# Pasqui1010/DART-Planner

Hardware: AMD Instinct MI355X
Metric: SE(3) rollouts/sec (N=30, batch=8192) + p95 solve ms, at 1/2/4/8 MI355X (higher is better)
Workload: dtype f32

## Files before the change

### dart_planner_amd/capi.py

```python
from __future__ import annotations

import ctypes as C
import math
import os
from typing import Optional

_HERE = os.path.dirname(os.path.abspath(__file__))
DEFAULT_LIBRARY = os.path.join(_HERE, "libse3mpc.so")

SE3MPC_MAX_HORIZON = 64
SE3MPC_MAX_CORRECTIONS = 10
SE3MPC_MAX_SPHERES = 256

STATUS_NAMES = {0: "SE3MPC_OK", -1: "SE3MPC_ERR_NULL", -2: "SE3MPC_ERR_HORIZON", -3: "SE3MPC_ERR_SHAPE",
                -4: "SE3MPC_ERR_PARAM", -5: "SE3MPC_ERR_WORKSPACE", -6: "SE3MPC_ERR_LAUNCH",
                -7: "SE3MPC_ERR_NO_DEVICE"}
TASK_MESSAGES = {1: "CONVERGENCE: NORM OF PROJECTED GRADIENT <= PGTOL",
                 2: "CONVERGENCE: RELATIVE REDUCTION OF F <= FACTR*EPSMCH",
                 3: "STOP: TOTAL NO. OF ITERATIONS REACHED LIMIT",
                 4: "STOP: TOTAL NO. OF F,G EVALUATIONS EXCEEDS LIMIT",
                 5: "ABNORMAL: "}


class Se3mpcLibraryError(RuntimeError):
    """libse3mpc.so is missing or does not export the ABI of include/se3mpc.h."""


class Se3mpcError(RuntimeError):

    def __init__(self, fn: str, status: int, detail: str = ""):
        self.status = status
        super().__init__(f"{fn} -> {STATUS_NAMES.get(status, status)}" + (f": {detail}" if detail else ""))


class Params(C.Structure):
    _fields_ = [("horizon", C.c_int32), ("has_goal", C.c_int32), ("dt", C.c_double), ("mass", C.c_double),
                ("gravity", C.c_double), ("position_weight", C.c_double), ("velocity_weight", C.c_double),
                ("acceleration_weight", C.c_double), ("thrust_weight", C.c_double), ("terminal_factor", C.c_double),
                ("position_bound", C.c_double), ("max_velocity", C.c_double), ("max_acceleration", C.c_double),
                ("max_thrust", C.c_double), ("min_thrust", C.c_double), ("max_tilt_angle", C.c_double),
                ("safety_margin", C.c_double), ("max_iterations", C.c_int32), ("max_corrections", C.c_int32),
                ("max_linesearch", C.c_int32), ("max_fun", C.c_int32), ("pgtol", C.c_double), ("ftol", C.c_double)]

    @classmethod
    def reference_defaults(cls, **overrides) -> "Params":
        p = cls(horizon=6, has_goal=1, dt=1.0 / 400.0, mass=1.5, gravity=9.81, position_weight=100.0,
                velocity_weight=10.0, acceleration_weight=1.0, thrust_weight=0.1, terminal_factor=10.0,
                position_bound=100.0, max_velocity=10.0, max_acceleration=15.0, max_thrust=25.0, min_thrust=2.0,
                max_tilt_angle=math.pi / 4, safety_margin=1.5, max_iterations=15, max_corrections=10,
                max_linesearch=20, max_fun=15000, pgtol=0.05, ftol=0.5)
        names = cls._field_names()
        for k, v in overrides.items():
            if k not in names:
                raise AttributeError(f"se3mpc_params has no field {k!r}")
            setattr(p, k, v)
        return p

    @classmethod
    def _field_names(cls) -> frozenset:
        names = cls.__dict__.get("_names")
        if names is None:
            names = cls._names = frozenset(n for n, _ in cls._fields_)
        return names

    def copy(self, **overrides) -> "Params":
        q = Params()
        C.memmove(C.byref(q), C.byref(self), C.sizeof(Params))
        for k, v in overrides.items():
            setattr(q, k, v)
        return q

    def as_dict(self) -> dict:
        return {n: getattr(self, n) for n, _ in self._fields_}


class SolveInfo(C.Structure):
    _fields_ = [("fun", C.c_double), ("nit", C.c_int32), ("nfev", C.c_int32), ("status", C.c_int32),
                ("task", C.c_int32)]


class VoxelMapDesc(C.Structure):
    _fields_ = [("keys", C.c_void_p), ("prob", C.c_void_p), ("count", C.c_void_p), ("capacity", C.c_int32),
                ("reserved", C.c_int32), ("resolution", C.c_double), ("prior", C.c_double)]


class ControllerParams(C.Structure):
    _fields_ = [("kp_pos", C.c_double * 3), ("ki_pos", C.c_double * 3), ("kd_pos", C.c_double * 3), ("kp_att", C.c_double * 3),
                ("kd_att", C.c_double * 3), ("inertia", C.c_double * 3), ("max_torque_xyz", C.c_double * 3),
                ("max_integral_per_axis", C.c_double * 3), ("max_integral_pos", C.c_double), ("max_tilt_angle", C.c_double),
                ("mass", C.c_double), ("gravity", C.c_double), ("max_thrust", C.c_double), ("min_thrust", C.c_double),
                ("tracking_error_threshold", C.c_double), ("velocity_error_threshold", C.c_double),
                ("back_calculation_gain", C.c_double), ("integral_decay_factor", C.c_double), ("saturation_threshold", C.c_double),
                ("yaw_singularity_threshold", C.c_double), ("default_heading_yaw", C.c_double),
                ("anti_windup_method", C.c_int32), ("yaw_fallback_method", C.c_int32)]
    ANTI_WINDUP = {"clamping": 0, "back_calculation": 1}
    YAW_FALLBACK = {"skip_yaw": 0, "default_heading": 1, "maintain_current": 2}

    @classmethod
    def from_config(cls, cfg) -> "ControllerParams":
        p = cls()
        for name, ctype in cls._fields_:
            if name == "anti_windup_method":
                p.anti_windup_method = cls.ANTI_WINDUP.get(cfg.anti_windup_method, 2)
            elif name == "yaw_fallback_method":
                p.yaw_fallback_method = cls.YAW_FALLBACK.get(cfg.yaw_singularity_fallback_method, 3)
            elif ctype is C.c_double:
                setattr(p, name, float(getattr(cfg, name)))
            else:
                setattr(p, name, (C.c_double * 3)(*[float(v) for v in getattr(cfg, name)]))
        return p


class SimulatorParams(C.Structure):
    _fields_ = [("mass", C.c_double), ("gravity", C.c_double), ("inertia", C.c_double * 3), ("max_thrust", C.c_double),
                ("max_torque", C.c_double)]

    @classmethod
    def reference_defaults(cls, **overrides) -> "SimulatorParams":
        p = cls(mass=1.5, gravity=9.81, inertia=(C.c_double * 3)(0.1, 0.1, 0.2), max_thrust=20.0, max_torque=10.0)
        for k, v in overrides.items():
            setattr(p, k, v)
        return p


class SmootherParams(C.Structure):
    _fields_ = [("transition_time", C.c_double), ("velocity_limit", C.c_double), ("acceleration_limit", C.c_double),
                ("jerk_limit", C.c_double), ("update_dt", C.c_double), ("smoothing_window", C.c_double),
                ("pos_diff_threshold", C.c_double), ("vel_diff_threshold", C.c_double), ("timeout", C.c_double),
                ("decay_rate", C.c_double), ("decay_cap", C.c_double)]

    @classmethod
    def reference_defaults(cls, **overrides) -> "SmootherParams":
        p = cls(transition_time=0.5, velocity_limit=5.0, acceleration_limit=3.0, jerk_limit=10.0, update_dt=0.01, smoothing_window=0.1,
                pos_diff_threshold=0.5, vel_diff_threshold=1.0, timeout=2.0, decay_rate=2.0, decay_cap=5.0)
        for k, v in overrides.items():
            if k not in dict(cls._fields_):
                raise AttributeError(f"se3mpc_smoother_params has no field {k!r}")
            setattr(p, k, float(v))
        return p

    def copy(self, **overrides) -> "SmootherParams":
        return type(self).reference_defaults(**{**{k: getattr(self, k) for k, _ in self._fields_}, **overrides})


CONTROLLER_STATE_WORDS = 12
SMOOTHER_STATE_WORDS = 25

_P = C.c_void_p
_I = C.c_int
_D = C.c_double
_PP = C.POINTER(Params)
_VP = C.POINTER(VoxelMapDesc)

_TYPED_API = {
    "init": (True, [_I, _I, _P, _P, _P, _I, _P, _P]),
    "cost_grad": (True, [_I, _I, _P, _P, _P, _P, _P]),
    "dynamics_residual": (True, [_I, _I, _P, _P, _P, _P, _P]),
    "obstacle_residual": (True, [_I, _I, _P, _P, _I, _P, _P, _P, _P]),
    "physical_constraints": (True, [_I, _I, _P, _P, _P]),
    "extract": (True, [_I, _I, _P, _P, _P, _P, _P, _P]),
    "rollout_cost_grad": (True, [_I, _I, _P, _P, _P, _P, _P, _P, _P, _P, _P, C.c_uint32, _P]),
    "rollout_cost_grad_batched": (True, [_I, _I, _I, _P, _P, _P, _P, _P, _P, _P, C.c_uint32, _P]),
    "rollout_obstacles": (True, [_I, _I, _P, _P, _P, _P, _P, _P, _P, _I, _P, _P, _P, C.c_uint32, _P]),
    "rollout_obstacles_batched": (True, [_I, _I, _I, _P, _P, _P, _P, _P, _P, _P, _I, _P, _P, _P, C.c_uint32, _P]),
    "rollout_iterate": (True, [_I, _I, _I, _I, _D, _P, _P, _P, _P, _P, _P, _P, _P, _P, C.c_uint32, _P]),
    "rollout_iterate_obstacles": (True, [_I, _I, _I, _I, _D, _P, _P, _P, _P, _P, _P, _P, _P, _P, _I, _D, _P, _P, C.c_uint32, _P]),
    "shooting_finish": (True, [_I, _I, _P, _P, _I, C.c_uint32, _P, _P, _I, _D, _P, _P, _P]),
    "projected_step": (True, [_I, _I, _D, _P, _P, _P, _P]),
    "is_plan_valid": (True, [_I, _I, _P, _P, _P, _P]),
    "argmin": (False, [_I, _P, C.c_uint32, _P, _P]),
    "spheres_from_grid": (False, [_P, _P, _I, C.c_double, _I, C.c_double, _P, _I, _P, _P]),
    "transpose": (False, [_I, _I, _P, _I, _P, _I, _P]),
    "population_sums": (False, [_I, _I, _I, _P, _P, _D, _P, _D, _P, _P, _P]),
    "mppi": (True, [_I, _I, _I, _I, _D, _D, C.c_uint64, C.c_uint32, _P, C.c_uint32, _P, _P, _P, _P, _P, _P, _I, _D, _P, _P, _P, _P]),
    "mppi_split": (True, [_I, _I, _I, _I, _D, _D, C.c_uint64, C.c_uint32, _P, C.c_uint32, _P, _P, _P, _P, _P, _P, _I, _D, _P, _P, _P, _I, _P, C.c_size_t,
                          _P]),
    "mppi_samples": (True, [_I, _I, _I, _D, C.c_uint64, C.c_uint32, C.c_uint32, _P, _P, _I, _P, _P, _P]),
    "solve": (True, [_I, _P, _P, _P, _P, _P, _P, _P, _P, _P, _P, _P]),
    "plan_host": (True, [_I, _P, _P, _P, _P, _P, _P, _P, _P, _P, _P, _P, C.c_uint64, C.c_double, _P]),
}
_VOXEL_TYPED_API = {
    "query": [_P, _I, _P, _P],
    "trajectory_safe": [_P, _I, _I, C.c_longlong, _D, _D, _P, _P, _P],
    "local_spheres": [C.POINTER(C.c_double * 3), _D, _D, _I, _D, _P, _I, _P, _P, _P],
}
_VOXEL_PLAIN_API = {
    "se3mpc_voxel_clear": (C.c_int, [_VP, _P]),
    "se3mpc_voxel_insert": (C.c_int, [_VP, _P, _P, _D, _P, _I, _P, _P]),
    "se3mpc_voxel_update_rays": (C.c_int, [_VP, _P, _P, _P, _P, _I, _D, _D, _P, _P, _I, _P, _P, _P, _P]),
    "se3mpc_voxel_update_row_words": (C.c_longlong, [_I, _I]),
    "se3mpc_voxel_trace_rays": (C.c_int, [_VP, _P, _P, _P, _I, _P, _P, _I, _P, _P]),
    "se3mpc_voxel_export": (C.c_int, [_VP, _P, _P, _P, _P, _P]),
    "se3mpc_voxel_local_workspace": (C.c_int, [_I]),
}
_CP = C.POINTER(ControllerParams)
_SP = C.POINTER(SimulatorParams)
_MP = C.POINTER(SmootherParams)
_LL = C.c_longlong
_PLAN = [_I, _P, _LL, _P, _LL, _P, _LL, _P, _LL]
_LOOP_TYPED_API = {
    "control": [_CP, _I, _P, _P, _P, _P, _P, _P, _P, _P, _P, _P, _P, _P, _P, _P, _P, _P, _P],
    "control_fast": [_CP, _D, _D, _I, _D, _P, _P, _P, _P, _P, _P, _P, _P, _P, _P, _P, _P, _P, _P],
    "controller_integral_update": [_CP, _I, _P, _D, _P, _P, _P],
    "controller_attitude_torque": [_CP, _I, _P, _P, _P, _P, _P, C.POINTER(C.c_double * 9), _P, _P, _P, _P],
    "controller_desired_frame": [_CP, _I, _I, _P, _P, _P, _P, _P, _P, _P],
    "control_plan": [_CP, _I, _P, _P, _P, _P, _P, _P, _I, _P, _LL, _P, _LL, _P, _LL, _P, _LL, _P, _P, _P, _P, _P, _P, _P, _P],
    "simulator_step": [_SP, _I, _D, _P, _P, _P, _LL, _P, _P, _P, _P, _P, _P],
    "closed_loop": [_CP, _SP, _I, _I, _D, _I, _P, _LL, _P, _LL, _P, _LL, _P, _LL, _P, _P, _P, _P, _P, _P, _P, _LL, _I,
                    C.POINTER(C.c_double * 3), _I, _P, _P, _P, _P, _P],
    "smoother_update": [_MP, _I, _P] + _PLAN + _PLAN + [_P, _P],
    "smoother_desired": [_MP, _I, _P, _P, _P] + _PLAN + [_P, _P, _P, _P],
    "closed_loop_smoothed": [_MP, _CP, _SP, _I, _I, _D] + _PLAN + [_P, _P, _P, _P, _P, _P, _P, _P, _LL, _I, C.POINTER(C.c_double * 3),
                             _P, _P, _P, _P, _P],
    "monte_carlo": [_PP, _CP, _SP, _I, _I, _I, _D, _P, _P, _LL, _P, _P, _P, _P, _P, _P, _P, _P, _P, _P, _P],
    "mppi_closed_loop": [_PP, _CP, _SP, _I, _I, _I, _D, C.c_uint32, _I, _I, _I, _D, _D, C.c_uint64, C.c_uint32, C.c_uint32, _P, _P, _I, _D, _P, _LL,
                         _P, _P, _P, _P, _P, _P, _P, _P, _P, _P, _P, _P],
}
_PLAIN_API = {
    "se3mpc_controller_default_params": (C.c_int, [_CP]),
    "se3mpc_simulator_default_params": (C.c_int, [_SP]),
    "se3mpc_controller_reset": (C.c_int, [_CP, _I, _P, _P]),
    "se3mpc_smoother_default_params": (C.c_int, [_MP]),
    "se3mpc_smoother_reset": (C.c_int, [_I, _P, _P]),
    "se3mpc_abi_version": (C.c_int, []),
    "se3mpc_last_error": (C.c_char_p, []),
    "se3mpc_device_count": (C.c_int, []),
    "se3mpc_default_params": (C.c_int, [_PP]),
    "se3mpc_check_params": (C.c_int, [_PP]),
    "se3mpc_set_rollout_variant": (C.c_int, [_I]),
    "se3mpc_set_solver_variant": (C.c_int, [_I]),
    "se3mpc_reduce_keys": (C.c_int, [_P, _I, _I, _P, _P]),
    "se3mpc_key_index": (C.c_uint32, [C.c_uint64]),
    "se3mpc_key_cost": (C.c_float, [C.c_uint64]),
    "se3mpc_population_workspace": (C.c_int, [_I, _I]),
    "se3mpc_mppi_split_workspace_bytes": (C.c_size_t, [_I, _I, _I]),
}


def exported_symbols() -> list:
    names = list(_PLAIN_API)
    for base in _TYPED_API:
        names += [f"se3mpc_{base}_f32", f"se3mpc_{base}_f64"]
    for base in _LOOP_TYPED_API:
        names += [f"se3mpc_{base}_f32", f"se3mpc_{base}_f64"]
    names += list(_VOXEL_PLAIN_API)
    for base in _VOXEL_TYPED_API:
        names += [f"se3mpc_voxel_{base}_f32", f"se3mpc_voxel_{base}_f64"]
    return names


class Library:

    def __init__(self, path: Optional[str] = None):
        self.path = path or os.environ.get("SE3MPC_LIBRARY", DEFAULT_LIBRARY)
        if not os.path.exists(self.path):
            raise Se3mpcLibraryError(
                f"{self.path} not found: the HIP extension has not been built.  Run "
                "`python -c 'import __graft_entry__ as g; g.build()'` (or `make -C dart_planner_amd/csrc`). "
                "There is no CPU fallback.")
        try:
            self._dll = C.CDLL(self.path)
        except OSError as e:
            raise Se3mpcLibraryError(f"cannot load {self.path}: {e}") from e
        missing = [s for s in exported_symbols() if not hasattr(self._dll, s)]
        if missing:
            raise Se3mpcLibraryError(f"{self.path} does not export {missing}")
        for name, (res, args) in _PLAIN_API.items():
            fn = getattr(self._dll, name)
            fn.restype, fn.argtypes = res, args
        for base, (has_params, args) in _TYPED_API.items():
            for suf in ("f32", "f64"):
                fn = getattr(self._dll, f"se3mpc_{base}_{suf}")
                fn.restype = C.c_int
                fn.argtypes = ([_PP] if has_params else []) + args
        for base, args in _LOOP_TYPED_API.items():
            for suf in ("f32", "f64"):
                fn = getattr(self._dll, f"se3mpc_{base}_{suf}")
                fn.restype, fn.argtypes = C.c_int, args
        for name, (res, args) in _VOXEL_PLAIN_API.items():
            fn = getattr(self._dll, name)
            fn.restype, fn.argtypes = res, args
        for base, args in _VOXEL_TYPED_API.items():
            for suf in ("f32", "f64"):
                fn = getattr(self._dll, f"se3mpc_voxel_{base}_{suf}")
                fn.restype = C.c_int
                fn.argtypes = [_VP] + args
        if self._dll.se3mpc_abi_version() != 1:
            raise Se3mpcLibraryError(f"{self.path}: ABI version {self._dll.se3mpc_abi_version()} != 1")

    def abi_version(self) -> int:
        return self._dll.se3mpc_abi_version()

    def last_error(self) -> str:
        return (self._dll.se3mpc_last_error() or b"").decode()

    def device_count(self) -> int:
        return self._dll.se3mpc_device_count()

    def default_params(self) -> Params:
        p = Params()
        self._check("se3mpc_default_params", self._dll.se3mpc_default_params(C.byref(p)))
        return p

    def check_params(self, p: Params) -> int:
        return self._dll.se3mpc_check_params(C.byref(p))

    def set_rollout_variant(self, variant: int) -> None:
        self._check("se3mpc_set_rollout_variant", self._dll.se3mpc_set_rollout_variant(variant))

    def set_solver_variant(self, variant: int) -> None:
        self._check("se3mpc_set_solver_variant", self._dll.se3mpc_set_solver_variant(variant))

    def reduce_keys(self, wave_keys: int, per_batch: int, nbatch: int, keys_out: int, stream: int) -> None:
        self._check("se3mpc_reduce_keys", self._dll.se3mpc_reduce_keys(wave_keys, per_batch, nbatch, keys_out, stream))

    def population_workspace(self, rows: int, B: int) -> int:
        return self._dll.se3mpc_population_workspace(rows, B)

    def mppi_split_workspace_bytes(self, horizon: int, nprob: int, splits: int) -> int:
        return self._dll.se3mpc_mppi_split_workspace_bytes(horizon, nprob, splits)

    def key_index(self, key: int) -> int:
        return self._dll.se3mpc_key_index(C.c_uint64(key))

    def key_cost(self, key: int) -> float:
        return self._dll.se3mpc_key_cost(C.c_uint64(key))

    def call(self, base: str, suffix: str, *args, params: Optional[Params] = None) -> None:
        fn = getattr(self._dll, f"se3mpc_{base}_{suffix}")
        has_params = _TYPED_API[base][0]
        if has_params:
            if params is None:
                raise TypeError(f"se3mpc_{base} needs params")
            rc = fn(C.byref(params), *args)
        else:
            rc = fn(*args)
        self._check(f"se3mpc_{base}_{suffix}", rc)

    def call_status(self, base: str, suffix: str, *args, params: Optional[Params] = None) -> int:
        fn = getattr(self._dll, f"se3mpc_{base}_{suffix}")
        if _TYPED_API[base][0]:
            return fn(C.byref(params) if params is not None else None, *args)
        return fn(*args)

    def controller_default_params(self) -> ControllerParams:
        p = ControllerParams()
        self._check("se3mpc_controller_default_params", self._dll.se3mpc_controller_default_params(C.byref(p)))
        return p

    def simulator_default_params(self) -> SimulatorParams:
        p = SimulatorParams()
        self._check("se3mpc_simulator_default_params", self._dll.se3mpc_simulator_default_params(C.byref(p)))
        return p

    def controller_reset(self, cp: ControllerParams, B: int, state: int, stream: int) -> None:
        self._check("se3mpc_controller_reset", self._dll.se3mpc_controller_reset(C.byref(cp), B, state, stream))

    def smoother_default_params(self) -> SmootherParams:
        p = SmootherParams()
        self._check("se3mpc_smoother_default_params", self._dll.se3mpc_smoother_default_params(C.byref(p)))
        return p

    def smoother_reset(self, B: int, state: int, stream: int) -> None:
        self._check("se3mpc_smoother_reset", self._dll.se3mpc_smoother_reset(B, state, stream))

    def loop_call(self, base: str, suffix: str, *args) -> None:
        a = [C.byref(x) if isinstance(x, (ControllerParams, SimulatorParams, SmootherParams, Params)) else x for x in args]
        self._check(f"se3mpc_{base}_{suffix}", getattr(self._dll, f"se3mpc_{base}_{suffix}")(*a))

    def loop_status(self, base: str, suffix: str, *args) -> int:
        a = [C.byref(x) if isinstance(x, (ControllerParams, SimulatorParams, SmootherParams, Params)) else x for x in args]
        return getattr(self._dll, f"se3mpc_{base}_{suffix}")(*a)

    def voxel(self, name: str, desc: VoxelMapDesc, *args) -> None:
        self._check(f"se3mpc_voxel_{name}", getattr(self._dll, f"se3mpc_voxel_{name}")(C.byref(desc), *args))

    def voxel_status(self, name: str, desc: Optional[VoxelMapDesc], *args) -> int:
        return getattr(self._dll, f"se3mpc_voxel_{name}")(C.byref(desc) if desc is not None else None, *args)

    def voxel_local_workspace(self, cells_per_axis: int) -> int:
        return self._dll.se3mpc_voxel_local_workspace(cells_per_axis)

    def voxel_update_row_words(self, M: int, max_len: int) -> int:
        return self._dll.se3mpc_voxel_update_row_words(M, max_len)

    def _check(self, name: str, rc: int) -> None:
        if rc != 0:
            raise Se3mpcError(name, rc, self.last_error() if rc == -6 else "")


_default: Optional[Library] = None


def get_library() -> Library:
    global _default
    if _default is None:
        _default = Library()
    return _default
```

### dart_planner_amd/csrc/reduce_kernels.hip

```cpp
#include "lane_common.hpp"
#include "rollout_device.hpp"

namespace se3mpc {

template <typename R>
__global__ void __launch_bounds__(256)
argmin_kernel(int B, const R* __restrict__ cost, uint32_t index_base, unsigned long long* __restrict__ key) {
  __shared__ unsigned long long wave_min[4];
  unsigned long long best = ~0ull;
  for (int b = blockIdx.x * blockDim.x + threadIdx.x; b < B; b += gridDim.x * blockDim.x) {
    const unsigned long long k = ((unsigned long long)orderable_bits((float)cost[b]) << 32) | (unsigned long long)(index_base + (uint32_t)b);
    best = k < best ? k : best;
  }
  for (int off = 32; off > 0; off >>= 1) {
    const unsigned long long o = __shfl_down(best, off, kWave);
    best = o < best ? o : best;
  }
  const int lane = threadIdx.x & (kWave - 1), wave = threadIdx.x / kWave;
  if (lane == 0) wave_min[wave] = best;
  __syncthreads();
  if (threadIdx.x == 0) {
    unsigned long long m = wave_min[0];
    for (int w = 1; w < (int)(blockDim.x / kWave); ++w) m = wave_min[w] < m ? wave_min[w] : m;
    atomicMin(key, m);
  }
}

template <typename R>
__global__ void __launch_bounds__(256)
population_sums_kernel(int rows, int B, int ld, const R* __restrict__ X, const R* __restrict__ cost, double cost_ref,
                       const unsigned long long* __restrict__ ref_key, double inv_temperature, int per_split,
                       double* __restrict__ part) {
  __shared__ double wave_tot[4];
  const int r = blockIdx.x, split = blockIdx.y;
  const int lo = split * per_split, hi = (lo + per_split < B) ? lo + per_split : B;
  if (ref_key != nullptr) {
    uint32_t u = (uint32_t)(ref_key[0] >> 32);
    u = (u & 0x80000000u) ? (u & 0x7FFFFFFFu) : ~u;
    cost_ref = (double)__uint_as_float(u);
  }
  const R* row = r < rows ? X + (size_t)r * ld : nullptr;
  double acc = 0.0;
  for (int b = lo + threadIdx.x; b < hi; b += blockDim.x) {
    const double w = cost != nullptr ? exp(-((double)cost[b] - cost_ref) * inv_temperature) : 1.0;
    acc += row != nullptr ? w * (double)row[b] : w;
  }
  acc = wave_sum(acc);
  const int lane = threadIdx.x & (kWave - 1), wave = threadIdx.x / kWave;
  if (lane == 0) wave_tot[wave] = acc;
  __syncthreads();
  if (threadIdx.x == 0) part[(size_t)split * (rows + 1) + r] = ((wave_tot[0] + wave_tot[1]) + wave_tot[2]) + wave_tot[3];
}

__global__ void __launch_bounds__(256)
population_fold_kernel(int n, int nsplit, const double* __restrict__ part, double* __restrict__ out) {
  const int r = blockIdx.x * blockDim.x + threadIdx.x;
  if (r >= n) return;
  double acc = 0.0;
  for (int sp = 0; sp < nsplit; ++sp) acc += part[(size_t)sp * n + r];
  out[r] = acc;
}

__global__ void __launch_bounds__(256)
reduce_keys_kernel(const unsigned long long* __restrict__ wave_keys, int per_batch, unsigned long long* __restrict__ keys_out) {
  __shared__ unsigned long long wave_min[4];
  const unsigned long long* src = wave_keys + (size_t)blockIdx.x * per_batch;
  unsigned long long best = ~0ull;
  for (int i = threadIdx.x; i < per_batch; i += blockDim.x) best = src[i] < best ? src[i] : best;
  for (int off = 32; off > 0; off >>= 1) {
    const unsigned long long o = __shfl_down(best, off, kWave);
    best = o < best ? o : best;
  }
  if ((threadIdx.x & (kWave - 1)) == 0) wave_min[threadIdx.x / kWave] = best;
  __syncthreads();
  if (threadIdx.x == 0) {
    unsigned long long m = wave_min[0];
    for (int w = 1; w < 4; ++w) m = wave_min[w] < m ? wave_min[w] : m;
    keys_out[blockIdx.x] = m;
  }
}

template <typename IO>
__global__ void __launch_bounds__(64)
shooting_finish_kernel(DevParams<double> q, int B, int ld, const IO* __restrict__ T, const unsigned long long* __restrict__ wave_keys,
                       int n_slots, uint32_t index_base, const double* __restrict__ state, const double* __restrict__ spheres, int K,
                       double w_obs, double* __restrict__ out, unsigned long long* __restrict__ key_out) {
  __shared__ double sT[3][kWave], sP[3][kWave], sV[3][kWave], sC[3];
  const int lane = threadIdx.x, N = q.N;
  unsigned long long best = ~0ull;
  for (int i = lane; i < n_slots; i += kWave) best = wave_keys[i] < best ? wave_keys[i] : best;
  for (int off = 32; off > 0; off >>= 1) {
    const unsigned long long o = __shfl_down(best, off, kWave);
    best = o < best ? o : best;
  }
  best = __shfl(best, 0, kWave);
  if (lane == 0 && key_out != nullptr) *key_out = best;
  uint32_t idx = (uint32_t)(best & 0xFFFFFFFFull) - index_base;
  if (idx >= (uint32_t)B) idx = 0;
  const bool live = lane < N;
  double t0 = 0.0, t1 = 0.0, t2 = 0.0;
  if (live) {
    t0 = (double)T[(size_t)(3 * lane + 0) * ld + idx]; t1 = (double)T[(size_t)(3 * lane + 1) * ld + idx]; t2 = (double)T[(size_t)(3 * lane + 2) * ld + idx];
  }
  sT[0][lane] = t0; sT[1][lane] = t1; sT[2][lane] = t2;
  __syncthreads();
  if (lane < 3) {
    const int a = lane;
    const AxisConsts<double> c = axis_consts<double>(q, a, q.has_goal ? state[6 + a] : 0.0);
    double p = state[a], v = state[3 + a];
    RolloutSums<double> s = {0, 0, 0, 0, 0};
    for (int k = 0; k < N; ++k) {
      const double tk = sT[a][k];
      const double acc = tk * q.inv_mass - c.grav, dev = tk - c.hov, e = p - c.gl;
      sP[a][k] = p; sV[a][k] = v;
      if (k == N - 1) s.sterm = e * e; else s.sp += e * e;
      s.sv += v * v; s.sa += acc * acc; s.st += dev * dev;
      p = p + v * q.dt + q.half_dt2 * acc;
      v = v + acc * q.dt;
    }
    s.sp += s.sterm;
    sC[a] = axis_cost(q, s);
  }
  __syncthreads();
  const double cost = sC[0] + sC[1] + sC[2];
  const double mag = sqrt(t0 * t0 + t1 * t1 + t2 * t2);
  const bool valid = live && mag > 1e-6;
  double b1[3] = {0, 0, 0}, b2[3] = {0, 0, 0}, b3[3] = {0, 0, 0};
  double roll = 0.0, pitch = 0.0, yaw = 0.0;
  double n1 = 0.0;
  if (valid) {
    b3[0] = t0 / mag; b3[1] = t1 / mag; b3[2] = t2 / mag;
    b1[0] = 0.0; b1[1] = -b3[2]; b1[2] = b3[1];
    n1 = sqrt(b1[1] * b1[1] + b1[2] * b1[2]);
    if (n1 > 1e-6) { b1[1] /= n1; b1[2] /= n1; } else { b1[0] = 1.0; b1[1] = 0.0; b1[2] = 0.0; }
    b2[0] = b3[1] * b1[2] - b3[2] * b1[1];
    b2[1] = b3[2] * b1[0] - b3[0] * b1[2];
    b2[2] = b3[0] * b1[1] - b3[1] * b1[0];
    roll = atan2(b2[2], b3[2]);
    pitch = asin(fmin(fmax(-b1[2], -1.0), 1.0));
    yaw = n1 > 1e-6 ? (b1[1] == 0.0 ? b1[1] : copysign(1.5707963267948966, b1[1])) : 0.0;
  }
  const uint64_t vmask = wave_ballot(valid);
  const uint64_t below = vmask & ((lane == 0) ? 0ull : (~0ull >> (64 - lane)));
  const bool has_prev = valid && below != 0ull;
  const int pk = has_prev ? 63 - __builtin_clzll(below) : lane;
  double q1[3], q2[3], q3[3];
#pragma unroll
  for (int c = 0; c < 3; ++c) { q1[c] = group_gather<kWave>(b1[c], pk); q2[c] = group_gather<kWave>(b2[c], pk); q3[c] = group_gather<kWave>(b3[c], pk); }
  double w0 = 0.0, w1 = 0.0, w2 = 0.0;
  if (has_prev) {
    double d1[3], d2[3], d3[3];
    for (int c = 0; c < 3; ++c) {
      d1[c] = (b1[c] - q1[c]) / q.dt;
      d2[c] = (b2[c] - q2[c]) / q.dt;
      d3[c] = (b3[c] - q3[c]) / q.dt;
    }
    w0 = b3[0] * d2[0] + b3[1] * d2[1] + b3[2] * d2[2];
    w1 = b1[0] * d3[0] + b1[1] * d3[1] + b1[2] * d3[2];
    w2 = b2[0] * d1[0] + b2[1] * d1[1] + b2[2] * d1[2];
  }
  double pen = 0.0;
  if (spheres != nullptr && K > 0) {
    double pl = 0.0;
    if (live) {
      const double px = sP[0][lane], py = sP[1][lane], pz = sP[2][lane];
      for (int j = 0; j < K; ++j) {
        const double dx = px - spheres[4 * j], dy = py - spheres[4 * j + 1], dz = pz - spheres[4 * j + 2], sm = spheres[4 * j + 3] + q.margin;
        const double h = fmax(0.0, -((dx * dx + dy * dy + dz * dz) - sm * sm));
        pl += h * h;
      }
    }
    pen = w_obs * wave_sum(pl);
  }
  if (live) {
    const int k = lane;
    double* o = out;
    o[3 * k] = sP[0][k]; o[3 * k + 1] = sP[1][k]; o[3 * k + 2] = sP[2][k]; o += 3 * N;
    o[3 * k] = sV[0][k]; o[3 * k + 1] = sV[1][k]; o[3 * k + 2] = sV[2][k]; o += 3 * N;
    o[3 * k] = t0; o[3 * k + 1] = t1; o[3 * k + 2] = t2; o += 3 * N;
    o[3 * k] = t0 / q.mass; o[3 * k + 1] = t1 / q.mass; o[3 * k + 2] = t2 / q.mass - q.grav; o += 3 * N;
    o[3 * k] = roll; o[3 * k + 1] = pitch; o[3 * k + 2] = yaw; o += 3 * N;
    o[3 * k] = w0; o[3 * k + 1] = w1; o[3 * k + 2] = w2; o += 3 * N;
    o[k] = mag;
  }
  if (lane == 0) { out[19 * N] = cost; out[19 * N + 1] = pen; out[19 * N + 2] = cost + pen; }
}

template <typename R>
__global__ void __launch_bounds__(256)
spheres_from_grid_kernel(const R* __restrict__ pos, const R* __restrict__ occ, int M, R threshold, int target, R radius,
                         R* __restrict__ spheres, int cap, int32_t* __restrict__ count) {
  __shared__ int wave_total[4];
  const int lane = threadIdx.x & (kWave - 1), wave = threadIdx.x / kWave;
  const int seg = ((M + 3) / 4 + kWave - 1) / kWave * kWave;
  const int lo = wave * seg, hi = (lo + seg < M) ? lo + seg : M;
  int mine = 0;
  for (int i0 = lo; i0 < hi; i0 += kWave) {
    const int i = i0 + lane;
    const bool o = i < hi && occ[i] > threshold;
    mine += __builtin_popcountll(wave_ballot(o));
  }
  if (lane == 0) wave_total[wave] = mine;
  __syncthreads();
  int rank = 0, total = 0;
  for (int w = 0; w < 4; ++w) { if (w < wave) rank += wave_total[w]; total += wave_total[w]; }
  const int step = (target > 0 && total / target > 1) ? total / target : 1;
  for (int i0 = lo; i0 < hi; i0 += kWave) {
    const int i = i0 + lane;
    const bool o = i < hi && occ[i] > threshold;
    const uint64_t m = wave_ballot(o);
    if (o) {
      const int r = rank + __builtin_popcountll(m & ((lane == 0) ? 0ull : (~0ull >> (64 - lane))));
      if (r % step == 0 && r / step < cap) {
        R* s4 = spheres + (size_t)4 * (r / step);
        s4[0] = pos[(size_t)3 * i]; s4[1] = pos[(size_t)3 * i + 1]; s4[2] = pos[(size_t)3 * i + 2]; s4[3] = radius;
      }
    }
    rank += __builtin_popcountll(m);
  }
  if (threadIdx.x == 0) {
    const int k = total == 0 ? 0 : (total + step - 1) / step;
    *count = k < cap ? k : cap;
  }
}

template <typename R>
__global__ void __launch_bounds__(256)
transpose_kernel(int rows, int cols, const R* __restrict__ in, int ld_in, R* __restrict__ out, int ld_out) {
  __shared__ R tile[64][65];
  const int c0 = blockIdx.x * 64, r0 = blockIdx.y * 64;
  const int tx = threadIdx.x & 63, ty = threadIdx.x >> 6;
  for (int i = ty; i < 64; i += 4) {
    const int r = r0 + i, c = c0 + tx;
    if (r < rows && c < cols) tile[i][tx] = in[(size_t)r * ld_in + c];
  }
  __syncthreads();
  for (int i = ty; i < 64; i += 4) {
    const int c = c0 + i, r = r0 + tx;
    if (r < rows && c < cols) out[(size_t)c * ld_out + r] = tile[tx][i];
  }
}

template <typename R, bool ROWS_SMALL>
__global__ void __launch_bounds__(512)
transpose_strip_kernel(int small, int longn, const R* __restrict__ in, int ld_in, R* __restrict__ out, int ld_out, int TW) {
  HIP_DYNAMIC_SHARED(unsigned char, lds_raw)
  R* tile = reinterpret_cast<R*>(lds_raw);
  const int pitch = small | 1;
  const int l0 = blockIdx.x * TW;
  const int nt = (longn - l0 < TW) ? longn - l0 : TW;
  const int lane = threadIdx.x & (kWave - 1), wave = threadIdx.x / kWave, nwave = blockDim.x / kWave;
  constexpr int U = 8;
  if constexpr (ROWS_SMALL) {
    for (int s0 = wave * U; s0 < small; s0 += nwave * U) {
      R v[U];
#pragma unroll
      for (int u = 0; u < U; ++u) v[u] = (s0 + u < small && lane < nt) ? in[(size_t)(s0 + u) * ld_in + l0 + lane] : (R)0;
#pragma unroll
      for (int u = 0; u < U; ++u) if (s0 + u < small && lane < nt) tile[lane * pitch + s0 + u] = v[u];
    }
    __syncthreads();
    for (int t = wave; t < nt; t += nwave)
      for (int sidx = lane; sidx < small; sidx += kWave) out[(size_t)(l0 + t) * ld_out + sidx] = tile[t * pitch + sidx];
  } else {
    for (int t = wave; t < nt; t += nwave) {
      const R* src = in + (size_t)(l0 + t) * ld_in;
      for (int s0 = lane; s0 < small; s0 += kWave * U) {
        R v[U];
#pragma unroll
        for (int u = 0; u < U; ++u) v[u] = (s0 + u * kWave < small) ? src[s0 + u * kWave] : (R)0;
#pragma unroll
        for (int u = 0; u < U; ++u) if (s0 + u * kWave < small) tile[t * pitch + s0 + u * kWave] = v[u];
      }
    }
    __syncthreads();
    for (int sidx = wave; sidx < small; sidx += nwave)
      if (lane < nt) out[(size_t)sidx * ld_out + l0 + lane] = tile[lane * pitch + sidx];
  }
}

template <typename R>
int argmin_impl(int B, const R* cost, uint32_t index_base, uint64_t* key, void* stream) {
  if (B < 0) return SE3MPC_ERR_SHAPE;
  if (!key) return SE3MPC_ERR_NULL;
  hipStream_t s = (hipStream_t)stream;
  if (hipMemsetAsync(key, 0xFF, sizeof(uint64_t), s) != hipSuccess) return launch_status("se3mpc_argmin(memset)");
  if (B == 0) return SE3MPC_OK;
  if (!cost) return SE3MPC_ERR_NULL;
  int grid = grid_for(B, 256);
  if (grid > 1024) grid = 1024;
  hipLaunchKernelGGL(argmin_kernel<R>, dim3(grid), dim3(256), 0, s, B, cost, index_base, (unsigned long long*)key);
  return launch_status("se3mpc_argmin");
}

static int population_splits(int B) {
  int n = B / 65536;
  return n < 1 ? 1 : (n > 16 ? 16 : n);
}

template <typename R>
int population_sums_impl(int rows, int B, int ld, const R* X, const R* cost, double cost_ref, const uint64_t* ref_key,
                         double temperature, double* out, double* workspace, void* stream) {
  if (rows < 0 || B < 0 || ld < B) return SE3MPC_ERR_SHAPE;
  if (!out) return SE3MPC_ERR_NULL;
  if (cost != nullptr && (!(temperature > 0.0) || !std::isfinite(temperature) || !std::isfinite(cost_ref))) return SE3MPC_ERR_PARAM;
  hipStream_t s = (hipStream_t)stream;
  if (B == 0) {
    if (hipMemsetAsync(out, 0, (size_t)(rows + 1) * sizeof(double), s) != hipSuccess) return launch_status("se3mpc_population_sums(memset)");
    return SE3MPC_OK;
  }
  if ((rows > 0 && !X) || !workspace) return SE3MPC_ERR_NULL;
  const int nsplit = population_splits(B);
  const int per_split = (B + nsplit - 1) / nsplit;
  hipLaunchKernelGGL(population_sums_kernel<R>, dim3(rows + 1, nsplit), dim3(256), 0, s, rows, B, ld, X, cost, cost_ref,
                     reinterpret_cast<const unsigned long long*>(ref_key), cost != nullptr ? 1.0 / temperature : 0.0, per_split,
                     workspace);
  int rc = launch_status("se3mpc_population_sums");
  if (rc) return rc;
  hipLaunchKernelGGL(population_fold_kernel, dim3(grid_for(rows + 1, 256)), dim3(256), 0, s, rows + 1, nsplit, workspace, out);
  return launch_status("se3mpc_population_sums(fold)");
}

template <typename R>
int spheres_from_grid_impl(const R* pos, const R* occ, int M, double threshold, int target, double radius, R* spheres, int cap,
                           int32_t* count, void* stream) {
  if (M < 0 || cap < 0 || target < 1) return SE3MPC_ERR_SHAPE;
  if (!count || (M > 0 && (!pos || !occ)) || (cap > 0 && !spheres)) return SE3MPC_ERR_NULL;
  hipLaunchKernelGGL(spheres_from_grid_kernel<R>, dim3(1), dim3(256), 0, (hipStream_t)stream, pos, occ, M, (R)threshold,
                     target, (R)radius, spheres, cap, count);
  return launch_status("se3mpc_spheres_from_grid");
}

template <typename R>
int transpose_impl(int rows, int cols, const R* in, int ld_in, R* out, int ld_out, void* stream) {
  if (rows < 0 || cols < 0 || ld_in < cols || ld_out < rows) return SE3MPC_ERR_SHAPE;
  if (rows == 0 || cols == 0) return SE3MPC_OK;
  if (!in || !out) return SE3MPC_ERR_NULL;
  const int small = rows < cols ? rows : cols, longn = rows < cols ? cols : rows;
// ... 95 lines not shown
```

### dart_planner_amd/csrc/rollout_device.hpp

```cpp
#pragma once

#include <hip/hip_runtime.h>

#include <cstdint>

#include "se3mpc_common.hpp"
#include <se3mpc_wave_ops.hpp>

namespace se3mpc {


template <typename R, bool SHARED_SLOT = false>
__device__ __forceinline__ void rollout_epilogue(bool live, int b, R c, R* __restrict__ cost,
                                                 unsigned long long* __restrict__ wave_key_slot, uint32_t index_base) {
  if (live) cost[b] = c;
  const uint32_t bits = live ? orderable_bits((float)c) : 0xFFFFFFFFu;
  const uint32_t m = wave_min_u32(bits);
  const int src = first_lane(wave_ballot(live && bits == m));
  if (wave_key_slot != nullptr && src >= 0 && lane_id() == src) {
    const unsigned long long k = ((unsigned long long)m << 32) | (unsigned long long)(index_base + (uint32_t)b);
    if constexpr (SHARED_SLOT) atomicMin(wave_key_slot, k);
    else *wave_key_slot = k;
  }
}

template <typename R>
struct RolloutSums {
  R sp, sv, sa, st, sterm;
};

template <typename R>
__device__ __forceinline__ R rollout_total(const DevParams<R>& q, const RolloutSums<R>& s) {
  R c = q.wv * s.sv + q.wa * s.sa + q.wT * s.st;
  if (q.has_goal) c += q.wp * s.sp + q.term * q.wp * s.sterm;
  return c;
}

template <typename R>
struct AxisConsts {
  R gl, grav, hov, two_wp, two_wv, c_aa, c_tt, c_lp, c_lv;
};

template <typename R>
__device__ __forceinline__ AxisConsts<R> axis_consts(const DevParams<R>& q, int a, R gl) {
  AxisConsts<R> c;
  c.gl = gl;
  c.grav = (a == 2) ? q.grav : (R)0;
  c.hov = (a == 2) ? q.hover : (R)0;
  c.two_wp = q.has_goal ? (R)2 * q.wp : (R)0;
  c.two_wv = (R)2 * q.wv;
  c.c_aa = (R)2 * q.wa * q.inv_mass;
  c.c_tt = (R)2 * q.wT;
  c.c_lp = q.half_dt2 * q.inv_mass;
  c.c_lv = q.dt * q.inv_mass;
  return c;
}

template <typename R>
__device__ __forceinline__ R axis_cost(const DevParams<R>& q, const RolloutSums<R>& s) {
  R c = q.wv * s.sv + q.wa * s.sa + q.wT * s.st;
  if (q.has_goal) c += q.wp * (s.sp + q.term * s.sterm);
  return c;
}

template <typename R, int N, bool GRAD, bool STATES, int LDAUX = 0, int STAUX = 0, bool TILE = false, bool EXACT = true, bool MIDSYNC = false>
__device__ __forceinline__ R rollout_axis_reg(const DevParams<R>& q, int a, unsigned voff, unsigned rowb, const R* __restrict__ p0,
                                              const R* __restrict__ v0, const R* __restrict__ goal,
                                              const R* __restrict__ T, R* __restrict__ gradT, R* __restrict__ Pout,
                                              R* __restrict__ Vout, R* __restrict__ ptile = nullptr) {
  const int Nn = EXACT ? N : q.N;
  R t[N], es[N], vs[N];
#pragma unroll
  for (int k = 0; k < N; ++k) {
    if (EXACT || k < Nn) t[k] = lane_ld<LDAUX>(lane_buf(T), voff, (unsigned)(3 * k + a) * rowb);
  }
  const AxisConsts<R> c = axis_consts<R>(q, a, q.has_goal ? lane_ld(lane_buf(goal), voff, (unsigned)(a) * rowb) : (R)0);
  R p = lane_ld(lane_buf(p0), voff, (unsigned)(a) * rowb);
  R v = lane_ld(lane_buf(v0), voff, (unsigned)(a) * rowb);
  RolloutSums<R> s = {0, 0, 0, 0, 0};
#pragma unroll
  for (int k = 0; k < N; ++k) {
    if (EXACT || k < Nn) {
      const R acc = t[k] * q.inv_mass - c.grav;
      const R dev = t[k] - c.hov;
      const R e = p - c.gl;
      es[k] = e; vs[k] = v;
      if (TILE) ptile[k * kWave] = p;
      if (k == Nn - 1) s.sterm = e * e; else s.sp += e * e;
      s.sv += v * v; s.sa += acc * acc; s.st += dev * dev;
      if (STATES) {
        lane_st(lane_buf(Pout), voff, (unsigned)(3 * k + a) * rowb, p);
        lane_st(lane_buf(Vout), voff, (unsigned)(3 * k + a) * rowb, v);
      }
      p = p + v * q.dt + q.half_dt2 * acc;
      v = v + acc * q.dt;
    }
  }
  if (MIDSYNC) __syncthreads();
  s.sp += s.sterm;
  if (GRAD) {
    R lamP = (R)0, lamV = (R)0;
#pragma unroll
    for (int k = N - 1; k >= 0; --k) {
      if (EXACT || k < Nn) {
        const R acc = t[k] * q.inv_mass - c.grav;
        const R dev = t[k] - c.hov;
        if (k == Nn - 1) {
          lane_st<STAUX>(lane_buf(gradT), voff, (unsigned)(3 * k + a) * rowb, c.c_aa * acc + c.c_tt * dev);
          lamP = c.two_wp * ((R)1 + q.term) * es[k];
          lamV = c.two_wv * vs[k];
        } else {
          lane_st<STAUX>(lane_buf(gradT), voff, (unsigned)(3 * k + a) * rowb, c.c_aa * acc + c.c_tt * dev + c.c_lp * lamP + c.c_lv * lamV);
          lamV = c.two_wv * vs[k] + q.dt * lamP + lamV;
          lamP = c.two_wp * es[k] + lamP;
        }
      }
    }
  }
  return axis_cost(q, s);
}

template <typename R, bool GRAD, bool STATES, int STAUX = 0, bool TILE = false, bool MIDSYNC = false>
__device__ __forceinline__ R rollout_axis_rev(const DevParams<R>& q, int a, unsigned voff, unsigned rowb, const R* __restrict__ p0,
                                              const R* __restrict__ v0, const R* __restrict__ goal,
                                              const R* __restrict__ T, R* __restrict__ gradT, R* __restrict__ Pout,
                                              R* __restrict__ Vout, R* __restrict__ ptile = nullptr) {
  const int N = q.N;
  const AxisConsts<R> c = axis_consts<R>(q, a, q.has_goal ? lane_ld(lane_buf(goal), voff, (unsigned)(a) * rowb) : (R)0);
  R p = lane_ld(lane_buf(p0), voff, (unsigned)(a) * rowb);
  R v = lane_ld(lane_buf(v0), voff, (unsigned)(a) * rowb);
  RolloutSums<R> s = {0, 0, 0, 0, 0};
  R tk = (R)0, pl = p, vl = v;
#pragma unroll 6
  for (int k = 0; k < N; ++k) {
    tk = lane_ld(lane_buf(T), voff, (unsigned)(3 * k + a) * rowb);
    const R acc = tk * q.inv_mass - c.grav;
    const R dev = tk - c.hov;
    const R e = p - c.gl;
    if (TILE) ptile[k * kWave] = p;
    if (k == N - 1) s.sterm = e * e; else s.sp += e * e;
    s.sv += v * v; s.sa += acc * acc; s.st += dev * dev;
    if (STATES) {
      lane_st(lane_buf(Pout), voff, (unsigned)(3 * k + a) * rowb, p);
      lane_st(lane_buf(Vout), voff, (unsigned)(3 * k + a) * rowb, v);
    }
    pl = p; vl = v;
    p = p + v * q.dt + q.half_dt2 * acc;
    v = v + acc * q.dt;
  }
  if (MIDSYNC) __syncthreads();
  s.sp += s.sterm;
  if (GRAD) {
    R lamP = c.two_wp * ((R)1 + q.term) * (pl - c.gl);
    R lamV = c.two_wv * vl;
    lane_st<STAUX>(lane_buf(gradT), voff, (unsigned)(3 * (N - 1) + a) * rowb, c.c_aa * (tk * q.inv_mass - c.grav) + c.c_tt * (tk - c.hov));
    R pk = pl, vk = vl;
#pragma unroll 6
    for (int k = N - 2; k >= 0; --k) {
      const R t = lane_ld(lane_buf(T), voff, (unsigned)(3 * k + a) * rowb);
      const R acc = t * q.inv_mass - c.grav;
      const R dev = t - c.hov;
      vk = vk - acc * q.dt;
      pk = pk - vk * q.dt - q.half_dt2 * acc;
      lane_st<STAUX>(lane_buf(gradT), voff, (unsigned)(3 * k + a) * rowb, c.c_aa * acc + c.c_tt * dev + c.c_lp * lamP + c.c_lv * lamV);
      lamV = c.two_wv * vk + q.dt * lamP + lamV;
      lamP = c.two_wp * (pk - c.gl) + lamP;
    }
  }
  return axis_cost(q, s);
}

typedef float obs_f2 __attribute__((vector_size(8)));
#ifndef SE3MPC_OBS_PACKED
#define SE3MPC_OBS_PACKED 1
#endif
template <typename R> constexpr bool kObsPacked = sizeof(R) == 4 && SE3MPC_OBS_PACKED;

}
```

### dart_planner_amd/csrc/rollout_iterate.hip

```cpp
#include "lane_common.hpp"
#include "rollout_device.hpp"

namespace se3mpc {

__device__ __forceinline__ float fma_r(float a, float b, float c) { return __builtin_fmaf(a, b, c); }
__device__ __forceinline__ double fma_r(double a, double b, double c) { return __builtin_fma(a, b, c); }
__device__ __forceinline__ float clamp_r(float x, float lo, float hi) { return __builtin_amdgcn_fmed3f(x, lo, hi); }
__device__ __forceinline__ double clamp_r(double x, double lo, double hi) { return fmin(fmax(x, lo), hi); }
template <typename R>
__device__ __forceinline__ R projected_update(R t, R g, R step, R lo, R hi) {
  return fmin(fmax(fma_r(-step, g, t), lo), hi);
}

template <typename R>
struct ObsCtx {
  R* tile;
  const R* sph;
  R* pen;
  R* pen_first;
  int Kpad;
  bool axis_sweeps;
  int slot, slots;
  R w_obs;
};
// ... 3 lines not shown
                                            obs_f2& qy, obs_f2& qz) {
  const obs_f2 dx = px2 - cx, dy = py2 - cy, dz = pz2 - cz;
  const obs_f2 c = dz * dz + (dy * dy + (dx * dx - r2));
  const obs_f2 h = obs_f2{fmaxf(0.0f, -c[0]), fmaxf(0.0f, -c[1])};
  if constexpr (PEN) pk += h * h;
  qx += h * dx; qy += h * dy; qz += h * dz;
}
template <typename R, bool PEN = true>
__device__ __forceinline__ void sphere_one(R px, R py, R pz, R cx, R cy, R cz, R r2, R& pk, R& qx, R& qy, R& qz) {
  const R dx = px - cx, dy = py - cy, dz = pz - cz;
  const R c = dz * dz + (dy * dy + (dx * dx - r2));
  const R h = fmax((R)0, -c);
  if constexpr (PEN) pk += h * h;
  qx += h * dx; qy += h * dy; qz += h * dz;
}

template <typename R, int TS>
__device__ __forceinline__ R obstacle_penalty_sweep(R* __restrict__ tile, const R* __restrict__ sph, int Nn, int Kpad, int first, int stride, int lane,
                                                    R w_obs) {
  R pen = (R)0;
  const R scale = (R)-4 * w_obs;
  lane &= TS - 1;
  for (int k = first; k < Nn; k += stride) {
    R* tx = tile + ((size_t)0 * Nn + k) * kWave + lane;
    R* ty = tile + ((size_t)1 * Nn + k) * kWave + lane;
    R* tz = tile + ((size_t)2 * Nn + k) * kWave + lane;
    const R px = *tx, py = *ty, pz = *tz;
    if constexpr (kObsPacked<R>) {
      const obs_f2 px2 = {px, px}, py2 = {py, py}, pz2 = {pz, pz}, zero = {0.0f, 0.0f};
      obs_f2 qx = zero, qy = zero, qz = zero, pk = zero;
#pragma unroll 4
      for (int j = 0; j < Kpad; j += 2) {
        const R* s0 = sph + 4 * j;
        sphere_pair(px2, py2, pz2, obs_f2{s0[0], s0[4]}, obs_f2{s0[1], s0[5]}, obs_f2{s0[2], s0[6]}, obs_f2{s0[3], s0[7]}, pk, qx, qy, qz);
      }
      pen += pk[0] + pk[1];
      *tx = scale * (qx[0] + qx[1]); *ty = scale * (qy[0] + qy[1]); *tz = scale * (qz[0] + qz[1]);
    } else {
      R qx = (R)0, qy = (R)0, qz = (R)0, pk = (R)0;
      for (int j = 0; j < Kpad; ++j) {
        const R* s0 = sph + 4 * j;
        sphere_one<R>(px, py, pz, s0[0], s0[1], s0[2], s0[3], pk, qx, qy, qz);
      }
      pen += pk;
      *tx = scale * qx; *ty = scale * qy; *tz = scale * qz;
    }
  }
  return w_obs * pen;
}

template <typename R, int KP>
struct SphereRegs {
  static constexpr int kPairs = kObsPacked<R> ? 4 * KP : 1, kOnes = kObsPacked<R> ? 1 : 8 * KP;
  obs_f2 cx2[kPairs], cy2[kPairs], cz2[kPairs], r22[kPairs];
  R cx[kOnes], cy[kOnes], cz[kOnes], r2[kOnes];
  __device__ __forceinline__ void load(const R* __restrict__ sph) {
    if constexpr (kObsPacked<R>) {
#pragma unroll
      for (int i = 0; i < kPairs; ++i) {
        const R* s0 = sph + 8 * i;
        cx2[i] = obs_f2{s0[0], s0[4]}; cy2[i] = obs_f2{s0[1], s0[5]}; cz2[i] = obs_f2{s0[2], s0[6]}; r22[i] = obs_f2{s0[3], s0[7]};
      }
    } else {
#pragma unroll
      for (int i = 0; i < kOnes; ++i) { cx[i] = sph[4 * i]; cy[i] = sph[4 * i + 1]; cz[i] = sph[4 * i + 2]; r2[i] = sph[4 * i + 3]; }
    }
  }
};

template <typename R, int KP, int U, int TS, bool PEN>
__device__ __forceinline__ R obstacle_penalty_sweep_regs(R* __restrict__ tile, const SphereRegs<R, KP>& sr, int Nn, int first, int stride, int lane,
                                                         R w_obs) {
  R pen = (R)0;
  const R scale = (R)-4 * w_obs;
  lane &= TS - 1;
#pragma unroll 1
  for (int k0 = first; k0 < Nn; k0 += U * stride) {
    R px[U], py[U], pz[U];
    R* tx[U];
#pragma unroll
    for (int u = 0; u < U; ++u) {
      const int k = k0 + u * stride;
      tx[u] = tile + (size_t)(k < Nn ? k : k0) * kWave + lane;
      px[u] = tx[u][0]; py[u] = tx[u][(size_t)Nn * kWave]; pz[u] = tx[u][(size_t)2 * Nn * kWave];
    }
    if constexpr (kObsPacked<R>) {
      const obs_f2 zero = {0.0f, 0.0f};
      obs_f2 px2[U], py2[U], pz2[U], qx[U], qy[U], qz[U], pk[U];
#pragma unroll
      for (int u = 0; u < U; ++u) { px2[u] = obs_f2{px[u], px[u]}; py2[u] = obs_f2{py[u], py[u]}; pz2[u] = obs_f2{pz[u], pz[u]}; qx[u] = qy[u] = qz[u] = pk[u] = zero; }
#pragma unroll
      for (int i = 0; i < SphereRegs<R, KP>::kPairs; ++i) {
#pragma unroll
        for (int u = 0; u < U; ++u) sphere_pair<PEN>(px2[u], py2[u], pz2[u], sr.cx2[i], sr.cy2[i], sr.cz2[i], sr.r22[i], pk[u], qx[u], qy[u], qz[u]);
      }
#pragma unroll
      for (int u = 0; u < U; ++u) {
        if (k0 + u * stride < Nn) {
          pen += pk[u][0] + pk[u][1];
          tx[u][0] = scale * (qx[u][0] + qx[u][1]); tx[u][(size_t)Nn * kWave] = scale * (qy[u][0] + qy[u][1]);
          tx[u][(size_t)2 * Nn * kWave] = scale * (qz[u][0] + qz[u][1]);
        }
      }
    } else {
      R qx[U], qy[U], qz[U], pk[U];
#pragma unroll
      for (int u = 0; u < U; ++u) qx[u] = qy[u] = qz[u] = pk[u] = (R)0;
#pragma unroll
      for (int i = 0; i < SphereRegs<R, KP>::kOnes; ++i) {
#pragma unroll
        for (int u = 0; u < U; ++u) sphere_one<R, PEN>(px[u], py[u], pz[u], sr.cx[i], sr.cy[i], sr.cz[i], sr.r2[i], pk[u], qx[u], qy[u], qz[u]);
      }
#pragma unroll
      for (int u = 0; u < U; ++u) {
        if (k0 + u * stride < Nn) {
          pen += pk[u];
          tx[u][0] = scale * qx[u]; tx[u][(size_t)Nn * kWave] = scale * qy[u]; tx[u][(size_t)2 * Nn * kWave] = scale * qz[u];
        }
      }
    }
  }
  return w_obs * pen;
}

template <typename R, int TS = kWave>
__device__ __forceinline__ void obstacle_exchange(const ObsCtx<R>& o, int Nn, int w, int lane, bool first) {
  __syncthreads();
  R pen = (R)0;
  if (o.axis_sweeps || w >= 3) pen = obstacle_penalty_sweep<R, TS>(o.tile, o.sph, Nn, o.Kpad, o.slot, o.slots, lane, o.w_obs);
  o.pen[w * kWave + lane] = pen;
  if (first) o.pen_first[w * kWave + lane] = pen;
  __syncthreads();
}

#ifndef SE3MPC_OBS_STEPS_IN_FLIGHT
#define SE3MPC_OBS_STEPS_IN_FLIGHT 2
#endif
template <typename R, int KP, int TS>
__device__ __forceinline__ void helper_passes_regs(const ObsCtx<R>& o, int Nn, int w, int lane, int passes) {
  SphereRegs<R, KP> sr;
  sr.load(o.sph);
#pragma unroll 1
  for (int ps = 0; ps < passes; ++ps) {
    __syncthreads();
    R pen = (R)0;
    if (ps == 0 || ps == passes - 1) pen = obstacle_penalty_sweep_regs<R, KP, SE3MPC_OBS_STEPS_IN_FLIGHT, TS, true>(o.tile, sr, Nn, o.slot, o.slots, lane, o.w_obs);
    else (void)obstacle_penalty_sweep_regs<R, KP, SE3MPC_OBS_STEPS_IN_FLIGHT, TS, false>(o.tile, sr, Nn, o.slot, o.slots, lane, o.w_obs);
    o.pen[w * kWave + lane] = pen;
    if (ps == 0) o.pen_first[w * kWave + lane] = pen;
    __syncthreads();
  }
}

template <typename R, int N, bool EXACT, int LDAUX, int STAUX, bool OBS = false, int TS = kWave>
__device__ __forceinline__ R iterate_axis_reg(const DevParams<R>& q, int a, unsigned voff, unsigned rowb, const R* __restrict__ p0,
                                              const R* __restrict__ v0, const R* __restrict__ goal, const R* __restrict__ Tin,
                                              R* __restrict__ Tout, R* __restrict__ gradT, int iters, R step, bool live, bool want_first,
                                              R& cost_first, const ObsCtx<R>* obs = nullptr) {
  const int Nn = EXACT ? N : q.N;
  R t[N], es[N], vs[N];
#pragma unroll
  for (int k = 0; k < N; ++k) {
    if (EXACT || k < Nn) t[k] = lane_ld<LDAUX>(lane_buf(Tin), voff, (unsigned)(3 * k + a) * rowb);
  }
  const AxisConsts<R> c = axis_consts<R>(q, a, q.has_goal ? lane_ld(lane_buf(goal), voff, (unsigned)(a) * rowb) : (R)0);
  const R pinit = lane_ld(lane_buf(p0), voff, (unsigned)(a) * rowb);
  const R vinit = lane_ld(lane_buf(v0), voff, (unsigned)(a) * rowb);
  const R lo = (a == 2) ? q.tz_lo : -q.txy, hi = (a == 2) ? q.tz_hi : q.txy;
  const int lane_ = (int)(threadIdx.x & (kWave - 1));
  R* my_tile = nullptr;
  if constexpr (OBS) my_tile = obs->tile + (size_t)a * Nn * kWave + lane_;
  auto forward_cost = [&]() -> R {
    R p = pinit, v = vinit;
    RolloutSums<R> s = {0, 0, 0, 0, 0};
#pragma unroll
    for (int k = 0; k < N; ++k) {
      if (EXACT || k < Nn) {
        const R acc = t[k] * q.inv_mass - c.grav;
        const R dev = t[k] - c.hov;
        const R e = p - c.gl;
        es[k] = e; vs[k] = v;
        if constexpr (OBS) my_tile[(size_t)k * kWave] = p;
        if (k == Nn - 1) s.sterm = e * e; else s.sp += e * e;
        s.sv += v * v; s.sa += acc * acc; s.st += dev * dev;
        p = p + v * q.dt + q.half_dt2 * acc;
        v = v + acc * q.dt;
      }
    }
    s.sp += s.sterm;
    return axis_cost(q, s);
  };
  cost_first = (R)0;
  bool first_exchange = true;
  if (want_first && iters > 0) {
    cost_first = forward_cost();
    if constexpr (OBS) { obstacle_exchange<R, TS>(*obs, Nn, a, lane_, first_exchange); first_exchange = false; }
  }
  const R gA = c.c_aa * q.inv_mass + c.c_tt, gB = c.c_aa * c.grav + c.c_tt * c.hov;
  const R u1 = (R)1 - step * gA, u0 = step * gB, uP = -step * c.c_lp, uV = -step * c.c_lv;
  const R lamP_term = c.two_wp * ((R)1 + q.term);
#pragma unroll 1
  for (int it = 0; it < iters; ++it) {
    R e = pinit - c.gl, v = vinit;
#pragma unroll
    for (int k = 0; k < N; ++k) {
      if (EXACT || k < Nn) {
        const R acc = fma_r(t[k], q.inv_mass, -c.grav);
        es[k] = e; vs[k] = v;
        if constexpr (OBS) my_tile[(size_t)k * kWave] = e + c.gl;
        e = fma_r(q.half_dt2, acc, fma_r(v, q.dt, e));
        v = fma_r(acc, q.dt, v);
      }
    }
    if constexpr (OBS) { obstacle_exchange<R, TS>(*obs, Nn, a, lane_, first_exchange); first_exchange = false; }
    R lamP = (R)0, lamV = (R)0;
#pragma unroll
    for (int k = N - 1; k >= 0; --k) {
      if (EXACT || k < Nn) {
        R qk = (R)0;
        if constexpr (OBS) qk = my_tile[(size_t)k * kWave];
        if (k == Nn - 1) {
          t[k] = clamp_r(fma_r(t[k], u1, u0), lo, hi);
          if constexpr (OBS) lamP = fma_r(lamP_term, es[k], qk); else lamP = lamP_term * es[k];
          lamV = c.two_wv * vs[k];
        } else {
          t[k] = clamp_r(fma_r(t[k], u1, fma_r(lamP, uP, fma_r(lamV, uV, u0))), lo, hi);
          lamV = fma_r(c.two_wv, vs[k], fma_r(q.dt, lamP, lamV));
          if constexpr (OBS) lamP = fma_r(c.two_wp, es[k], lamP + qk); else lamP = fma_r(c.two_wp, es[k], lamP);
        }
      }
    }
  }
  const R cost = forward_cost();
  if (!(want_first && iters > 0)) cost_first = cost;
  if constexpr (OBS) obstacle_exchange<R, TS>(*obs, Nn, a, lane_, first_exchange);
  if (gradT != nullptr) {
    R lamP = (R)0, lamV = (R)0;
#pragma unroll
    for (int k = N - 1; k >= 0; --k) {
      if (EXACT || k < Nn) {
        const R acc = t[k] * q.inv_mass - c.grav;
        const R dev = t[k] - c.hov;
        R qk = (R)0;
        if constexpr (OBS) qk = my_tile[(size_t)k * kWave];
        R g;
        if (k == Nn - 1) {
          g = c.c_aa * acc + c.c_tt * dev;
          lamP = c.two_wp * ((R)1 + q.term) * es[k];
          if constexpr (OBS) lamP += qk;
          lamV = c.two_wv * vs[k];
        } else {
          g = c.c_aa * acc + c.c_tt * dev + c.c_lp * lamP + c.c_lv * lamV;
          lamV = c.two_wv * vs[k] + q.dt * lamP + lamV;
          if constexpr (OBS) lamP = c.two_wp * es[k] + (lamP + qk); else lamP = c.two_wp * es[k] + lamP;
        }
        es[k] = g;
      }
    }
  }
  if (live) {
    if (gradT != nullptr) {
#pragma unroll
      for (int k = 0; k < N; ++k) {
        if (EXACT || k < Nn) lane_st<STAUX>(lane_buf(gradT), voff, (unsigned)(3 * k + a) * rowb, es[k]);
      }
    }
#pragma unroll
    for (int k = 0; k < N; ++k) {
      if (EXACT || k < Nn) lane_st<STAUX>(lane_buf(Tout), voff, (unsigned)(3 * k + a) * rowb, t[k]);
    }
  }
  return cost;
}

template <typename R, bool OBS = false, int TS = kWave>
__device__ __forceinline__ R iterate_axis_mem(const DevParams<R>& q, int a, unsigned voff, unsigned rowb, const R* __restrict__ p0,
                                              const R* __restrict__ v0, const R* __restrict__ goal, const R* __restrict__ Tin,
                                              R* __restrict__ Tout, R* __restrict__ gradT, int iters, R step, bool live, bool want_first,
                                              R& cost_first, const ObsCtx<R>* obs = nullptr) {
  (void)want_first;
  const int N = q.N;
  const int lane_ = (int)(threadIdx.x & (kWave - 1));
  if constexpr (!OBS) {
    if (!live) { cost_first = (R)0; return (R)0; }
  }
  R* my_tile = nullptr;
  if constexpr (OBS) my_tile = obs->tile + (size_t)a * N * kWave + lane_;
  const AxisConsts<R> c = axis_consts<R>(q, a, q.has_goal ? lane_ld(lane_buf(goal), voff, (unsigned)(a) * rowb) : (R)0);
  const R pinit = lane_ld(lane_buf(p0), voff, (unsigned)(a) * rowb);
  const R vinit = lane_ld(lane_buf(v0), voff, (unsigned)(a) * rowb);
  const R lo = (a == 2) ? q.tz_lo : -q.txy, hi = (a == 2) ? q.tz_hi : q.txy;
  if (Tin != Tout && live) {
    for (int k = 0; k < N; ++k) lane_st(lane_buf(Tout), voff, (unsigned)(3 * k + a) * rowb, lane_ld(lane_buf(Tin), voff, (unsigned)(3 * k + a) * rowb));
  }
  R cost = (R)0;
#pragma unroll 1
  for (int it = 0; it <= iters; ++it) {
    const bool last = it == iters;
    R p = pinit, v = vinit, pl = pinit, vl = vinit, tk = (R)0;
    RolloutSums<R> s = {0, 0, 0, 0, 0};
#pragma unroll 6
    for (int k = 0; k < N; ++k) {
      tk = (!OBS || live) ? lane_ld(lane_buf(Tout), voff, (unsigned)(3 * k + a) * rowb) : (R)0;
      const R acc = tk * q.inv_mass - c.grav;
      const R dev = tk - c.hov;
      const R e = p - c.gl;
      if (k == N - 1) s.sterm = e * e; else s.sp += e * e;
      s.sv += v * v; s.sa += acc * acc; s.st += dev * dev;
      if constexpr (OBS) my_tile[(size_t)k * kWave] = p;
      pl = p; vl = v;
      p = p + v * q.dt + q.half_dt2 * acc;
      v = v + acc * q.dt;
    }
    s.sp += s.sterm;
    cost = axis_cost(q, s);
    if (it == 0) cost_first = cost;
    if constexpr (OBS) obstacle_exchange<R, TS>(*obs, N, a, lane_, it == 0);
    R lamP = c.two_wp * ((R)1 + q.term) * (pl - c.gl);
    if constexpr (OBS) lamP += my_tile[(size_t)(N - 1) * kWave];
    R lamV = c.two_wv * vl;
    {
      const R g = c.c_aa * (tk * q.inv_mass - c.grav) + c.c_tt * (tk - c.hov);
      if (!OBS || live) {
        if (last) { if (gradT != nullptr) lane_st(lane_buf(gradT), voff, (unsigned)(3 * (N - 1) + a) * rowb, g); }
        else lane_st(lane_buf(Tout), voff, (unsigned)(3 * (N - 1) + a) * rowb, projected_update(tk, g, step, lo, hi));
      }
    }
    R pk = pl, vk = vl;
#pragma unroll 6
    for (int k = N - 2; k >= 0; --k) {
      const R tt = (!OBS || live) ? lane_ld(lane_buf(Tout), voff, (unsigned)(3 * k + a) * rowb) : (R)0;
      const R acc = tt * q.inv_mass - c.grav;
      const R dev = tt - c.hov;
      vk = vk - acc * q.dt;
      pk = pk - vk * q.dt - q.half_dt2 * acc;
      const R g = c.c_aa * acc + c.c_tt * dev + c.c_lp * lamP + c.c_lv * lamV;
      if (!OBS || live) {
        if (last) { if (gradT != nullptr) lane_st(lane_buf(gradT), voff, (unsigned)(3 * k + a) * rowb, g); }
        else lane_st(lane_buf(Tout), voff, (unsigned)(3 * k + a) * rowb, projected_update(tt, g, step, lo, hi));
      }
      lamV = c.two_wv * vk + q.dt * lamP + lamV;
      if constexpr (OBS) lamP = c.two_wp * (pk - c.gl) + (lamP + my_tile[(size_t)k * kWave]); else lamP = c.two_wp * (pk - c.gl) + lamP;
    }
  }
  return cost;
}

template <typename R, int N, bool REG, int FLAGS>
__global__ void __launch_bounds__(192)
rollout_iterate_kernel(DevParams<R> q, int B, int ld, int iters, R step, const R* __restrict__ p0, const R* __restrict__ v0,
                       const R* __restrict__ goal, const R* __restrict__ Tin, R* __restrict__ Tout, R* __restrict__ cost_first,
                       R* __restrict__ cost, R* __restrict__ gradT, unsigned long long* __restrict__ key, uint32_t index_base) {
  {
    const size_t bi = blockIdx.y, ss = (size_t)3 * ld, st = (size_t)3 * q.N * ld;
    p0 += bi * ss; v0 += bi * ss; Tin += bi * st; Tout += bi * st; cost += bi * (size_t)ld;
    if (goal != nullptr) goal += bi * ss;
    if (gradT != nullptr) gradT += bi * st;
    if (cost_first != nullptr) cost_first += bi * (size_t)ld;
    if (key != nullptr) key += bi * (size_t)gridDim.x;
  }
  int blk = blockIdx.x;
  if ((FLAGS & 4) && (gridDim.x & 7) == 0) blk = (blk & 7) * (gridDim.x >> 3) + (blk >> 3);
  const int lane = threadIdx.x & (kWave - 1);
  const int b0 = blk * kWave + lane;
  const bool live = b0 < B;
  const int b = live ? b0 : B - 1;
  const unsigned voff = (unsigned)b * (unsigned)sizeof(R), rowb = (unsigned)ld * (unsigned)sizeof(R);
  __shared__ R part[2][3][kWave];
  const int a = wave_uniform((int)(threadIdx.x / kWave));
  R c0 = (R)0, c;
  if constexpr (REG) c = iterate_axis_reg<R, N, !(FLAGS & 8), (FLAGS & 1) ? 2 : 0, (FLAGS & 2) ? 2 : 0>(q, a, voff, rowb, p0, v0, goal, Tin, Tout, gradT, iters, step, live, cost_first != nullptr, c0);
  else c = iterate_axis_mem<R>(q, a, voff, rowb, p0, v0, goal, Tin, Tout, gradT, iters, step, live, cost_first != nullptr, c0);
  part[0][a][lane] = c; part[1][a][lane] = c0;
  __syncthreads();
  const R total = part[0][0][lane] + part[0][1][lane] + part[0][2][lane];
  if (a == 0 && live && cost_first != nullptr) cost_first[b] = part[1][0][lane] + part[1][1][lane] + part[1][2][lane];
  rollout_epilogue<R>(live && a == 0, b, total, cost, (a == 0 && key != nullptr) ? key + blk : nullptr, index_base);
}

#ifndef SE3MPC_OBS_WIDE_W
#define SE3MPC_OBS_WIDE_W 7
#endif
#ifndef SE3MPC_OBS_WIDE_TS
#define SE3MPC_OBS_WIDE_TS 32
#endif
constexpr int kObsWideW = SE3MPC_OBS_WIDE_W, kObsWideTS = SE3MPC_OBS_WIDE_TS;
template <typename R, int N, bool REG, int FLAGS, int W, int TS>
__global__ void __launch_bounds__(64 * W)
rollout_iterate_obstacles_kernel(DevParams<R> q, int B, int ld, int iters, R step, const R* __restrict__ p0, const R* __restrict__ v0,
                                 const R* __restrict__ goal, const R* __restrict__ Tin, R* __restrict__ Tout, R* __restrict__ cost_first,
                                 R* __restrict__ cost, R* __restrict__ gradT, const R* __restrict__ spheres, int K, R w_obs,
                                 R* __restrict__ penalty, unsigned long long* __restrict__ key, uint32_t index_base) {
  HIP_DYNAMIC_SHARED(unsigned char, lds_raw)
  constexpr int SUBS = kWave / TS;
  {
    const size_t bi = blockIdx.y, ss = (size_t)3 * ld, st = (size_t)3 * q.N * ld;
    p0 += bi * ss; v0 += bi * ss; Tin += bi * st; Tout += bi * st; cost += bi * (size_t)ld;
    if (goal != nullptr) goal += bi * ss;
    if (gradT != nullptr) gradT += bi * st;
    if (cost_first != nullptr) cost_first += bi * (size_t)ld;
    if (penalty != nullptr) penalty += bi * (size_t)ld;
    if (key != nullptr) key += bi * (size_t)((B + kWave - 1) / kWave);
  }
  const int Kpad = (K + 7) / 8 * 8;
  R* tile = reinterpret_cast<R*>(lds_raw);
  R* sph = tile + (size_t)3 * q.N * kWave;
  R* pcost = sph + (size_t)4 * Kpad;
  R* ppen = pcost + 6 * kWave;
  for (int i = threadIdx.x; i < Kpad; i += 64 * W) {
    if (i < K) {
      const R sm = spheres[4 * i + 3] + q.margin;
      sph[4 * i + 0] = spheres[4 * i + 0]; sph[4 * i + 1] = spheres[4 * i + 1]; sph[4 * i + 2] = spheres[4 * i + 2]; sph[4 * i + 3] = sm * sm;
    } else {
      sph[4 * i + 0] = (R)0; sph[4 * i + 1] = (R)0; sph[4 * i + 2] = (R)0; sph[4 * i + 3] = (R)-INFINITY;
    }
  }
  int blk = blockIdx.x;
  if ((FLAGS & 4) && (gridDim.x & 7) == 0) blk = (blk & 7) * (gridDim.x >> 3) + (blk >> 3);
  const int lane = threadIdx.x & (kWave - 1);
  const int tl = lane & (TS - 1), sub = lane / TS;
  const int b0 = blk * TS + tl;
  const bool live = b0 < B && sub == 0;
  const int b = b0 < B ? b0 : B - 1;
  const unsigned voff = (unsigned)b * (unsigned)sizeof(R), rowb = (unsigned)ld * (unsigned)sizeof(R);
  const int a = wave_uniform((int)(threadIdx.x / kWave));
  ObsCtx<R> o;
  o.tile = tile; o.sph = sph; o.pen = ppen; o.pen_first = ppen + W * kWave; o.Kpad = Kpad; o.w_obs = w_obs;
  o.axis_sweeps = W <= 3 || Kpad == 0 || Kpad / 8 > (sizeof(R) == 4 ? 4 : 2);
  if (o.axis_sweeps) { o.slot = a * SUBS + sub; o.slots = W * SUBS; }
  else { o.slot = (a - 3) * SUBS + sub; o.slots = (W - 3) * SUBS; }
  if constexpr (W > 3) __syncthreads();
  if (a < 3) {
    R c0 = (R)0, c;
    if constexpr (REG) c = iterate_axis_reg<R, N, !(FLAGS & 8), (FLAGS & 1) ? 2 : 0, (FLAGS & 2) ? 2 : 0, true, TS>(q, a, voff, rowb, p0, v0, goal, Tin, Tout, gradT, iters, step, live, cost_first != nullptr, c0, &o);
    else c = iterate_axis_mem<R, true, TS>(q, a, voff, rowb, p0, v0, goal, Tin, Tout, gradT, iters, step, live, cost_first != nullptr, c0, &o);
    pcost[a * kWave + lane] = c; pcost[(3 + a) * kWave + lane] = c0;
  } else {
    const int passes = iters + 1 + ((REG && cost_first != nullptr && iters > 0) ? 1 : 0);
    const int kp = Kpad / 8;
    if (o.axis_sweeps) {
      for (int ps = 0; ps < passes; ++ps) obstacle_exchange<R, TS>(o, q.N, a, lane, ps == 0);
    } else if (kp == 1) helper_passes_regs<R, 1, TS>(o, q.N, a, lane, passes);
    else if (kp == 2) helper_passes_regs<R, 2, TS>(o, q.N, a, lane, passes);
    else if constexpr (sizeof(R) == 4) {
      if (kp == 3) helper_passes_regs<R, 3, TS>(o, q.N, a, lane, passes);
      else helper_passes_regs<R, 4, TS>(o, q.N, a, lane, passes);
    }
  }
  __syncthreads();
  R total = pcost[0 * kWave + lane] + pcost[1 * kWave + lane] + pcost[2 * kWave + lane];
  R pen = (R)0, pen0 = (R)0;
#pragma unroll
  for (int w = 0; w < W; ++w) {
#pragma unroll
    for (int h = 0; h < SUBS; ++h) { pen += ppen[w * kWave + h * TS + tl]; pen0 += ppen[(W + w) * kWave + h * TS + tl]; }
  }
  total += pen;
  if (a == 0 && live) {
    if (cost_first != nullptr) cost_first[b] = pcost[3 * kWave + lane] + pcost[4 * kWave + lane] + pcost[5 * kWave + lane] + pen0;
    if (penalty != nullptr) penalty[b] = pen;
  }
  if constexpr (SUBS == 1) {
    rollout_epilogue<R>(live && a == 0, b, total, cost, (a == 0 && key != nullptr) ? key + blk : nullptr, index_base);
  } else {
    rollout_epilogue<R, true>(live && a == 0, b, total, cost, (a == 0 && key != nullptr) ? key + blk / SUBS : nullptr, index_base);
  }
}

template <typename R>
__global__ void __launch_bounds__(64)
projected_step_kernel(DevParams<R> q, int B, int ld, R step, const R* __restrict__ T, const R* __restrict__ g, R* __restrict__ Tout) {
  const LaneIdx li = lane_index<R>(B);
  if (!li.live) return;
  const unsigned voff = li.voff, rowb = (unsigned)ld * (unsigned)sizeof(R);
  const int rows = 3 * q.N;
#pragma unroll 6
  for (int r = 0; r < rows; ++r) {
    const int a = r % 3;
    const R lo = (a == 2) ? q.tz_lo : -q.txy, hi = (a == 2) ? q.tz_hi : q.txy;
    const R t = lane_ld<2>(lane_buf(T), voff, (unsigned)r * rowb), gr = lane_ld<2>(lane_buf(g), voff, (unsigned)r * rowb);
    lane_st<2>(lane_buf(Tout), voff, (unsigned)r * rowb, projected_update(t, gr, step, lo, hi));
  }
}

template <typename R>
int rollout_iterate_impl(const se3mpc_params* p, int B, int ld, int nbatch, int iters, double step, const R* p0, const R* v0, const R* goal,
                         const R* Tin, R* Tout, R* cost_first, R* cost, R* gradT, uint64_t* key64, uint32_t index_base, void* stream) {
  if (nbatch < 1 || nbatch > 65535 || iters < 0 || iters > 1000000) return SE3MPC_ERR_SHAPE;
  int rc = check_lane_args(p, B, ld, p ? 3LL * p->horizon : 0, sizeof(R));
  if (rc) return rc;
  if (!std::isfinite(step)) return SE3MPC_ERR_PARAM;
  if (B == 0) return SE3MPC_OK;
  if (!p0 || !v0 || !Tin || !Tout || !cost || (p->has_goal && !goal)) return SE3MPC_ERR_NULL;
  unsigned long long* key = reinterpret_cast<unsigned long long*>(key64);
  const DevParams<R> q = make_dev_params<R>(*p);
  const int N = p->horizon, nblk = grid_for(B, kWave);
  hipStream_t s = (hipStream_t)stream;
  dispatch_horizon<R, true>(N, kSweepAuto, [&](auto sweep) {
    using S = decltype(sweep);
    hipLaunchKernelGGL((rollout_iterate_kernel<R, S::NN, S::REG, S::FLAGS>), dim3(nblk, nbatch), dim3(192), 0, s, q, B, ld, iters, (R)step, p0, v0,
                       goal, Tin, Tout, cost_first, cost, gradT, key, index_base);
  });
  return launch_status("se3mpc_rollout_iterate");
}

template <typename R>
int rollout_iterate_obstacles_impl(const se3mpc_params* p, int B, int ld, int nbatch, int iters, double step, const R* p0, const R* v0,
                                   const R* goal, const R* Tin, R* Tout, R* cost_first, R* cost, R* gradT, const R* spheres, int K,
                                   double obstacle_weight, R* penalty, uint64_t* key64, uint32_t index_base, void* stream) {
  if (nbatch < 1 || nbatch > 65535 || iters < 0 || iters > 1000000 || K < 0 || K > SE3MPC_MAX_SPHERES) return SE3MPC_ERR_SHAPE;
  int rc = check_lane_args(p, B, ld, p ? 3LL * p->horizon : 0, sizeof(R));
  if (rc) return rc;
  if (!std::isfinite(step) || !std::isfinite(obstacle_weight) || obstacle_weight < 0.0) return SE3MPC_ERR_PARAM;
  if (B == 0) return SE3MPC_OK;
  if (!p0 || !v0 || !Tin || !Tout || !cost || (p->has_goal && !goal) || (K > 0 && !spheres)) return SE3MPC_ERR_NULL;
  unsigned long long* key = reinterpret_cast<unsigned long long*>(key64);
  const DevParams<R> q = make_dev_params<R>(*p);
  const int N = p->horizon, nblk = grid_for(B, kWave);
  hipStream_t s = (hipStream_t)stream;
  const int forced_w = (g_lane_tuning.rollout_variant >> 7) & 3;
  const bool wide = forced_w != 1;
  const int Kpad = (K + 7) / 8 * 8;
  if (wide && key != nullptr && kObsWideTS < kWave) {
    if (hipMemsetAsync(key, 0xFF, (size_t)nbatch * nblk * sizeof(unsigned long long), s) != hipSuccess) return SE3MPC_ERR_LAUNCH;
  }
  dispatch_horizon<R, true>(N, kSweepAuto, [&](auto sweep) {
    using S = decltype(sweep);
    auto launch = [&](auto w, auto ts) {
      constexpr int WW = decltype(w)::value, TT = decltype(ts)::value;
      const size_t lds = ((size_t)3 * N * kWave + (size_t)4 * Kpad + (size_t)(6 + 2 * WW) * kWave) * sizeof(R);
      if (lds > 64 * 1024)
        (void)hipFuncSetAttribute(reinterpret_cast<const void*>(&rollout_iterate_obstacles_kernel<R, S::NN, S::REG, S::FLAGS, WW, TT>),
                                  hipFuncAttributeMaxDynamicSharedMemorySize, (int)lds);
      hipLaunchKernelGGL((rollout_iterate_obstacles_kernel<R, S::NN, S::REG, S::FLAGS, WW, TT>), dim3(grid_for(B, TT), nbatch), dim3(64 * WW),
                         lds, s, q, B, ld, iters, (R)step, p0, v0, goal, Tin, Tout, cost_first, cost, gradT, spheres, K,
                         (R)obstacle_weight, penalty, key, index_base);
    };
    if (wide) launch(std::integral_constant<int, kObsWideW>{}, std::integral_constant<int, kObsWideTS>{});
    else launch(std::integral_constant<int, 3>{}, std::integral_constant<int, kWave>{});
  });
  return launch_status("se3mpc_rollout_iterate_obstacles");
}

template <typename R>
int projected_step_impl(const se3mpc_params* p, int B, int ld, double step, const R* T, const R* g, R* Tout, void* stream) {
  int rc = check_lane_args(p, B, ld, p ? 3LL * p->horizon : 0, sizeof(R));
  if (rc) return rc;
  if (!std::isfinite(step)) return SE3MPC_ERR_PARAM;
  if (B == 0) return SE3MPC_OK;
  if (!T || !g || !Tout) return SE3MPC_ERR_NULL;
  hipLaunchKernelGGL(projected_step_kernel<R>, dim3(grid_for(B, kLaneBlock)), dim3(kLaneBlock), 0, (hipStream_t)stream, make_dev_params<R>(*p), B,
                     ld, (R)step, T, g, Tout);
  return launch_status("se3mpc_projected_step");
}

}

using namespace se3mpc;

extern "C" int se3mpc_rollout_iterate_f32(const se3mpc_params* p, int B, int ld, int nbatch, int iters, double step, const float* p0, const float* v0,
                                          const float* goal, const float* T_in, float* T_out, float* cost_first, float* cost, float* gradT,
                                          uint64_t* wave_keys, uint32_t index_base, void* stream) {
  return rollout_iterate_impl<float>(p, B, ld, nbatch, iters, step, p0, v0, goal, T_in, T_out, cost_first, cost, gradT, wave_keys, index_base,
                                     stream);
}
extern "C" int se3mpc_rollout_iterate_f64(const se3mpc_params* p, int B, int ld, int nbatch, int iters, double step, const double* p0,
                                          const double* v0, const double* goal, const double* T_in, double* T_out, double* cost_first, double* cost,
                                          double* gradT, uint64_t* wave_keys, uint32_t index_base, void* stream) {
  return rollout_iterate_impl<double>(p, B, ld, nbatch, iters, step, p0, v0, goal, T_in, T_out, cost_first, cost, gradT, wave_keys, index_base,
                                      stream);
}
extern "C" int se3mpc_rollout_iterate_obstacles_f32(const se3mpc_params* p, int B, int ld, int nbatch, int iters, double step, const float* p0,
                                                    const float* v0, const float* goal, const float* T_in, float* T_out, float* cost_first,
                                                    float* cost, float* gradT, const float* spheres, int K, double obstacle_weight, float* penalty,
                                                    uint64_t* wave_keys, uint32_t index_base, void* stream) {
  return rollout_iterate_obstacles_impl<float>(p, B, ld, nbatch, iters, step, p0, v0, goal, T_in, T_out, cost_first, cost, gradT, spheres, K,
                                               obstacle_weight, penalty, wave_keys, index_base, stream);
}
extern "C" int se3mpc_rollout_iterate_obstacles_f64(const se3mpc_params* p, int B, int ld, int nbatch, int iters, double step, const double* p0,
                                                    const double* v0, const double* goal, const double* T_in, double* T_out, double* cost_first,
                                                    double* cost, double* gradT, const double* spheres, int K, double obstacle_weight,
                                                    double* penalty, uint64_t* wave_keys, uint32_t index_base, void* stream) {
  return rollout_iterate_obstacles_impl<double>(p, B, ld, nbatch, iters, step, p0, v0, goal, T_in, T_out, cost_first, cost, gradT, spheres, K,
                                                obstacle_weight, penalty, wave_keys, index_base, stream);
}
extern "C" int se3mpc_projected_step_f32(const se3mpc_params* p, int B, int ld, double step, const float* T, const float* gradT, float* T_out,
                                         void* stream) {
  return projected_step_impl<float>(p, B, ld, step, T, gradT, T_out, stream);
}
extern "C" int se3mpc_projected_step_f64(const se3mpc_params* p, int B, int ld, double step, const double* T, const double* gradT, double* T_out,
                                         void* stream) {
  return projected_step_impl<double>(p, B, ld, step, T, gradT, T_out, stream);
}
```

### dart_planner_amd/ops.py

```python
from __future__ import annotations

from typing import Optional, Tuple

import ctypes as _C

import numpy as np

from .capi import (CONTROLLER_STATE_WORDS, SMOOTHER_STATE_WORDS, ControllerParams, Library, Params, SimulatorParams, SmootherParams, SolveInfo,
                   get_library, SE3MPC_MAX_SPHERES)

INFO_DTYPE = np.dtype([("fun", "<f8"), ("nit", "<i4"), ("nfev", "<i4"), ("status", "<i4"), ("task", "<i4")])
assert INFO_DTYPE.itemsize == 24


class TorchBackend:
    graph_capable = True

    def __init__(self, device=None):
        import torch
        self.torch = torch
        if not torch.cuda.is_available():
            raise RuntimeError("dart_planner_amd needs a HIP device (torch.cuda.is_available() is False); "
                               "there is no CPU fallback")
        self.device = torch.device(device if device is not None else f"cuda:{torch.cuda.current_device()}")
# ... 48 lines not shown
        self.be.check(a, name)
        if a.ndim != 2 or a.shape[0] != rows:
            raise ValueError(f"{name}: expected shape ({rows}, ld), got {tuple(a.shape)}")
        return a

    def _same(self, ref, *others):
        suf = self.be.suffix(ref)
        for o in others:
            if o is not None and (self.be.suffix(o) != suf or o.shape[-1] != ref.shape[-1]):
                raise ValueError("all lane-layout operands must share dtype and leading dimension")
        return suf

    def _spheres(self, spheres, suf) -> int:
        self.be.check(spheres, "spheres")
        if spheres.ndim != 2 or spheres.shape[1] != 4 or spheres.shape[0] > SE3MPC_MAX_SPHERES or self.be.suffix(spheres) != suf:
            raise ValueError(f"spheres: expected (K<={SE3MPC_MAX_SPHERES}, 4) {suf}, got {tuple(spheres.shape)}")
        return spheres.shape[0]

    @staticmethod
    def _B(ld: int, B: Optional[int]) -> int:
        B = ld if B is None else int(B)
        if B < 0 or B > ld:
            raise ValueError(f"B={B} outside [0, ld={ld}]")
        return B

    def init(self, params: Params, p0, v0, goal, project: bool = False, B: Optional[int] = None):
        N = params.horizon
        self._lane(p0, 3, "p0"); self._lane(v0, 3, "v0")
        if params.has_goal:
            self._lane(goal, 3, "goal")
        suf = self._same(p0, v0, goal if params.has_goal else None)
        ld = p0.shape[1]
        X0 = self.be.empty((9 * N, ld), suf)
        self.lib.call("init", suf, self._B(ld, B), ld, self.be.ptr(p0), self.be.ptr(v0),
                      self.be.ptr(goal if params.has_goal else None), int(bool(project)), self.be.ptr(X0),
                      self.be.stream(), params=params)
        return X0

    def cost_grad(self, params: Params, X, goal, want_grad: bool = True, B: Optional[int] = None):
        N = params.horizon
        self._lane(X, 9 * N, "X")
        if params.has_goal:
            self._lane(goal, 3, "goal")
        suf = self._same(X, goal if params.has_goal else None)
        ld = X.shape[1]
        f = self.be.empty((ld,), suf)
        g = self.be.empty((9 * N, ld), suf) if want_grad else None
        self.lib.call("cost_grad", suf, self._B(ld, B), ld, self.be.ptr(X),
                      self.be.ptr(goal if params.has_goal else None), self.be.ptr(f), self.be.ptr(g),
                      self.be.stream(), params=params)
        return f, g

    def dynamics_residual(self, params: Params, X, p0, v0, B: Optional[int] = None):
        N = params.horizon
        self._lane(X, 9 * N, "X"); self._lane(p0, 3, "p0"); self._lane(v0, 3, "v0")
        suf = self._same(X, p0, v0)
        ld = X.shape[1]
        R = self.be.empty((6 * N, ld), suf)
        self.lib.call("dynamics_residual", suf, self._B(ld, B), ld, self.be.ptr(X), self.be.ptr(p0), self.be.ptr(v0),
                      self.be.ptr(R), self.be.stream(), params=params)
        return R

    def obstacle_residual(self, params: Params, X, spheres, materialize: bool = True, reduce: bool = True,
                          B: Optional[int] = None):
        N = params.horizon
        self._lane(X, 9 * N, "X")
        self.be.check(spheres, "spheres")
        if spheres.ndim != 2 or spheres.shape[1] != 4 or spheres.shape[0] > SE3MPC_MAX_SPHERES:
            raise ValueError(f"spheres: expected (K<={SE3MPC_MAX_SPHERES}, 4), got {tuple(spheres.shape)}")
        suf = self.be.suffix(X)
        if self.be.suffix(spheres) != suf:
            raise ValueError("spheres dtype must match X")
        K, ld = spheres.shape[0], X.shape[1]
        Cm = self.be.empty((N * K, ld), suf) if materialize else None
        cmin = self.be.empty((ld,), suf) if reduce else None
        viol = self.be.empty((ld,), suf) if reduce else None
        self.lib.call("obstacle_residual", suf, self._B(ld, B), ld, self.be.ptr(X), self.be.ptr(spheres), K,
                      self.be.ptr(Cm), self.be.ptr(cmin), self.be.ptr(viol), self.be.stream(), params=params)
        return Cm, cmin, viol

    def physical_constraints(self, params: Params, X, B: Optional[int] = None):
        N = params.horizon
        self._lane(X, 9 * N, "X")
        suf, ld = self.be.suffix(X), X.shape[1]
        Cm = self.be.empty((4 * N, ld), suf)
        self.lib.call("physical_constraints", suf, self._B(ld, B), ld, self.be.ptr(X), self.be.ptr(Cm),
                      self.be.stream(), params=params)
        return Cm

    def extract(self, params: Params, T, B: Optional[int] = None):
        N = params.horizon
        self._lane(T, 3 * N, "T")
        suf, ld = self.be.suffix(T), T.shape[1]
        acc, att, rates = (self.be.empty((3 * N, ld), suf) for _ in range(3))
        thrust = self.be.empty((N, ld), suf)
        self.lib.call("extract", suf, self._B(ld, B), ld, self.be.ptr(T), self.be.ptr(acc), self.be.ptr(att),
                      self.be.ptr(rates), self.be.ptr(thrust), self.be.stream(), params=params)
        return acc, att, rates, thrust

    def rollout_cost_grad(self, params: Params, p0, v0, goal, T, want_grad: bool = True, want_states: bool = False,
                          B: Optional[int] = None, out=None, key=None, index_base: int = 0, wave_keys=None):
        N = params.horizon
        self._lane(p0, 3, "p0"); self._lane(v0, 3, "v0"); self._lane(T, 3 * N, "T")
        if params.has_goal:
            self._lane(goal, 3, "goal")
        suf = self._same(T, p0, v0, goal if params.has_goal else None)
        ld = T.shape[1]
        if out is not None:
            cost, gradT = out
        else:
            cost = self.be.empty((ld,), suf)
            gradT = self.be.empty((3 * N, ld), suf) if want_grad else None
        P = self.be.empty((3 * N, ld), suf) if want_states else None
        V = self.be.empty((3 * N, ld), suf) if want_states else None
        nB = self._B(ld, B)
        if key is not None and wave_keys is None:
            wave_keys = self.be.empty(((nB + 63) // 64,), "i64")
        self.lib.call("rollout_cost_grad", suf, nB, ld, self.be.ptr(p0), self.be.ptr(v0),
                      self.be.ptr(goal if params.has_goal else None), self.be.ptr(T), self.be.ptr(cost),
                      self.be.ptr(gradT), self.be.ptr(P), self.be.ptr(V), self.be.ptr(wave_keys), int(index_base),
                      self.be.stream(), params=params)
        if key is not None and nB > 0:
            self.lib.reduce_keys(self.be.ptr(wave_keys), (nB + 63) // 64, 1, self.be.ptr(key), self.be.stream())
        return cost, gradT, P, V

    def reduce_keys(self, wave_keys, keys_out):
        nb, per = wave_keys.shape
        self.lib.reduce_keys(self.be.ptr(wave_keys), per, nb, self.be.ptr(keys_out), self.be.stream())
        return keys_out

    def shooting_finish(self, params: Params, T, wave_keys, state, out, key_out=None, spheres=None, obstacle_weight: float = 0.0, B: Optional[int] = None,
                        index_base: int = 0):
        N = params.horizon
        self._lane(T, 3 * N, "T")
        suf = self.be.suffix(T)
        for nm, a, n in (("state", state, 9), ("out", out, 19 * N + 3), ("key_out", key_out, 1)):
            if a is None and nm == "key_out":
                continue
            if not (self.be.is_host_mapped(a) or (self.be.check(a, nm) is a)):
                raise TypeError(f"{nm}: expected a device tensor or a pinned host tensor")
            if int(np.prod(a.shape)) < n or str(a.dtype).rsplit(".", 1)[-1] != ("int64" if nm == "key_out" else "float64"):
                raise ValueError(f"{nm}: expected at least {n} {'int64' if nm == 'key_out' else 'float64'} values")
        K = 0
        if spheres is not None:
            self.be.check(spheres, "spheres")
            if spheres.ndim != 2 or spheres.shape[1] != 4 or spheres.shape[0] > SE3MPC_MAX_SPHERES or str(spheres.dtype).rsplit(".", 1)[-1] != "float64":
                raise ValueError(f"spheres: expected float64 (K<={SE3MPC_MAX_SPHERES}, 4), got {tuple(spheres.shape)} {spheres.dtype}")
            K = spheres.shape[0]
        self.be.check(wave_keys, "wave_keys")
        ld = T.shape[1]
        self.lib.call("shooting_finish", suf, self._B(ld, B), ld, self.be.ptr(T), self.be.ptr(wave_keys), int(np.prod(wave_keys.shape)), int(index_base),
                      self.be.ptr(state), self.be.ptr(spheres if K else None), K, float(obstacle_weight), self.be.ptr(out), self.be.ptr(key_out),
                      self.be.stream(), params=params)
        return out

    def rollout_cost_grad_batched(self, params: Params, p0, v0, goal, T, cost, gradT, wave_keys=None, index_base: int = 0):
        N = params.horizon
        nb, _, ld = T.shape
        for a, shp, nm in ((p0, (nb, 3, ld), "p0"), (v0, (nb, 3, ld), "v0"), (T, (nb, 3 * N, ld), "T"),
                           (cost, (nb, ld), "cost"), (gradT, (nb, 3 * N, ld), "gradT")):
            self.be.check(a, nm)
            if tuple(a.shape) != shp:
                raise ValueError(f"{nm}: expected {shp}, got {tuple(a.shape)}")
        if params.has_goal:
            self.be.check(goal, "goal")
        suf = self.be.suffix(T)
        self.lib.call("rollout_cost_grad_batched", suf, ld, ld, nb, self.be.ptr(p0), self.be.ptr(v0),
                      self.be.ptr(goal if params.has_goal else None), self.be.ptr(T), self.be.ptr(cost),
                      self.be.ptr(gradT), self.be.ptr(wave_keys), int(index_base), self.be.stream(), params=params)
        return cost, gradT

    def rollout_obstacles(self, params: Params, p0, v0, goal, T, spheres, want_grad: bool = True, B: Optional[int] = None,
                          wave_keys=None, index_base: int = 0, out=None):
        N = params.horizon
        self._lane(p0, 3, "p0"); self._lane(v0, 3, "v0"); self._lane(T, 3 * N, "T")
        if params.has_goal:
            self._lane(goal, 3, "goal")
        suf = self._same(T, p0, v0, goal if params.has_goal else None)
        self._spheres(spheres, suf)
        ld = T.shape[1]
        if out is not None:
            cost, gradT, cmin, viol = out
        else:
            cost = self.be.empty((ld,), suf)
            gradT = self.be.empty((3 * N, ld), suf) if want_grad else None
            cmin, viol = self.be.empty((ld,), suf), self.be.empty((ld,), suf)
        self.lib.call("rollout_obstacles", suf, self._B(ld, B), ld, self.be.ptr(p0), self.be.ptr(v0),
                      self.be.ptr(goal if params.has_goal else None), self.be.ptr(T), self.be.ptr(cost), self.be.ptr(gradT),
                      self.be.ptr(spheres), spheres.shape[0], self.be.ptr(cmin), self.be.ptr(viol), self.be.ptr(wave_keys),
                      int(index_base), self.be.stream(), params=params)
        return cost, gradT, cmin, viol

    def rollout_obstacles_batched(self, params: Params, p0, v0, goal, T, spheres, cost, gradT, cmin, viol, wave_keys=None,
                                  index_base: int = 0):
        N = params.horizon
        nb, _, ld = T.shape
        for a, shp, nm in ((p0, (nb, 3, ld), "p0"), (v0, (nb, 3, ld), "v0"), (T, (nb, 3 * N, ld), "T"), (cost, (nb, ld), "cost"),
                           (gradT, (nb, 3 * N, ld), "gradT"), (cmin, (nb, ld), "cmin"), (viol, (nb, ld), "viol")):
            if a is None and nm in ("gradT", "cmin", "viol"):
                continue
            self.be.check(a, nm)
            if tuple(a.shape) != shp:
                raise ValueError(f"{nm}: expected {shp}, got {tuple(a.shape)}")
        if params.has_goal:
            self.be.check(goal, "goal")
        suf = self.be.suffix(T)
        self._spheres(spheres, suf)
        self.lib.call("rollout_obstacles_batched", suf, ld, ld, nb, self.be.ptr(p0), self.be.ptr(v0),
                      self.be.ptr(goal if params.has_goal else None), self.be.ptr(T), self.be.ptr(cost), self.be.ptr(gradT),
                      self.be.ptr(spheres), spheres.shape[0], self.be.ptr(cmin), self.be.ptr(viol), self.be.ptr(wave_keys),
                      int(index_base), self.be.stream(), params=params)
        return cost, gradT, cmin, viol

    def rollout_iterate(self, params: Params, p0, v0, goal, T, iters: int, step: float, T_out=None, want_grad: bool = True,
                        want_first_cost: bool = False, B: Optional[int] = None, out=None, wave_keys=None, index_base: int = 0,
                        spheres=None, obstacle_weight: float = 1000.0, want_penalty: bool = True):
        N = params.horizon
        batched = T.ndim == 3
        nb = T.shape[0] if batched else 1
        ld = T.shape[-1]
        lead = (nb,) if batched else ()
        for a, rows, nm in ((p0, 3, "p0"), (v0, 3, "v0"), (T, 3 * N, "T")) + (((goal, 3, "goal"),) if params.has_goal else ()):
            self.be.check(a, nm)
            if tuple(a.shape) != lead + (rows, ld):
                raise ValueError(f"{nm}: expected {lead + (rows, ld)}, got {tuple(a.shape)}")
        suf = self.be.suffix(T)
        if out is not None:
            T_out, cost, gradT = out
        else:
            T_out = T_out if T_out is not None else self.be.empty(lead + (3 * N, ld), suf)
            cost = self.be.empty(lead + (ld,), suf)
            gradT = self.be.empty(lead + (3 * N, ld), suf) if want_grad else None
        cost_first = self.be.empty(lead + (ld,), suf) if want_first_cost else None
        nB = self._B(ld, B)
        if spheres is not None:
            self._spheres(spheres, suf)
            penalty = self.be.empty(lead + (ld,), suf) if want_penalty else None
            self.lib.call("rollout_iterate_obstacles", suf, nB, ld, nb, int(iters), float(step), self.be.ptr(p0), self.be.ptr(v0),
                          self.be.ptr(goal if params.has_goal else None), self.be.ptr(T), self.be.ptr(T_out), self.be.ptr(cost_first),
                          self.be.ptr(cost), self.be.ptr(gradT), self.be.ptr(spheres if spheres.shape[0] else None), spheres.shape[0],
                          float(obstacle_weight), self.be.ptr(penalty), self.be.ptr(wave_keys), int(index_base), self.be.stream(),
                          params=params)
            return dict(T=T_out, cost=cost, gradT=gradT, cost_first=cost_first, penalty=penalty)
        self.lib.call("rollout_iterate", suf, nB, ld, nb, int(iters), float(step), self.be.ptr(p0), self.be.ptr(v0),
                      self.be.ptr(goal if params.has_goal else None), self.be.ptr(T), self.be.ptr(T_out), self.be.ptr(cost_first),
                      self.be.ptr(cost), self.be.ptr(gradT), self.be.ptr(wave_keys), int(index_base), self.be.stream(), params=params)
        return dict(T=T_out, cost=cost, gradT=gradT, cost_first=cost_first)

    def projected_step(self, params: Params, T, gradT, step: float, out=None, B: Optional[int] = None):
        N = params.horizon
        self._lane(T, 3 * N, "T"); self._lane(gradT, 3 * N, "gradT")
        suf = self._same(T, gradT)
        ld = T.shape[1]
        T_out = out if out is not None else self.be.empty((3 * N, ld), suf)
        self.lib.call("projected_step", suf, self._B(ld, B), ld, float(step), self.be.ptr(T), self.be.ptr(gradT), self.be.ptr(T_out),
                      self.be.stream(), params=params)
        return T_out

    def is_plan_valid(self, params: Params, P, V=None, B: Optional[int] = None):
        N = params.horizon
        self._lane(P, 3 * N, "P")
        if V is not None:
            self._lane(V, 3 * N, "V")
        suf = self._same(P, V)
        ld = P.shape[1]
        valid = self.be.empty((ld,), "i32")
        self.lib.call("is_plan_valid", suf, self._B(ld, B), ld, self.be.ptr(P), self.be.ptr(V), self.be.ptr(valid),
                      self.be.stream(), params=params)
        return valid

    def argmin(self, cost, index_base: int = 0, out=None):
        self.be.check(cost, "cost")
        suf = self.be.suffix(cost)
        key = out if out is not None else self.be.empty((1,), "i64")
        self.lib.call("argmin", suf, int(cost.shape[0]), self.be.ptr(cost), int(index_base), self.be.ptr(key),
                      self.be.stream())
        return key

    def decode_key(self, key) -> Tuple[int, float]:
        k = int(self.be.to_host(key).reshape(-1)[0]) & 0xFFFFFFFFFFFFFFFF
        return self.lib.key_index(k), self.lib.key_cost(k)

    def population_sums(self, X, cost=None, temperature: float = 1.0, cost_ref: float = 0.0, ref_key=None, B: Optional[int] = None):
        self.be.check(X, "X")
        if X.ndim != 2:
            raise ValueError("X: expected (rows, ld)")
        rows, ld = X.shape
        B = self._B(ld, B)
        suf = self.be.suffix(X)
        if cost is not None and (self.be.suffix(self.be.check(cost, "cost")) != suf or cost.shape[-1] < B):
            raise ValueError("cost: same dtype as X and at least B entries")
        out = self.be.empty((rows + 1,), "f64")
        work = self.be.empty((self.lib.population_workspace(rows, B),), "f64")
        self.lib.call("population_sums", suf, rows, B, ld, self.be.ptr(X), self.be.ptr(cost), float(cost_ref), self.be.ptr(ref_key),
                      float(temperature), self.be.ptr(out), self.be.ptr(work), self.be.stream())
        return out

    def _mppi_operands(self, params: Params, U, p0=None, v0=None, goal=None):
        N = params.horizon
        self._lane(U, 3 * N, "U")
        if p0 is not None:
            self._lane(p0, 3, "p0"); self._lane(v0, 3, "v0")
            if params.has_goal:
                self._lane(goal, 3, "goal")
        return self._same(U, p0, v0, goal if params.has_goal else None), U.shape[1]

# ... 471 lines not shown
```

### dart_planner_amd/planning/se3_mpc_planner.py

```python
from __future__ import annotations

import logging
import math
import ctypes
import time
from dataclasses import dataclass, fields
from typing import Any, Dict, List, Optional, Tuple

import numpy as np

from ..capi import Params, TASK_MESSAGES
from ..common.types import DroneState, Trajectory
from ..common.units import ensure_units, to_float
from .base_planner import BasePlanner, PlannerFactory

_log = logging.getLogger(__name__)


@dataclass(frozen=True)
class SE3MPCConfig:
    prediction_horizon: int = 6
    dt: float = 0.125
    max_velocity: float = 10.0
    max_acceleration: float = 15.0
# ... 195 lines not shown
            io = self._io = dict(key=key,
                                 h_in=torch.empty((3, B, 3), dtype=dt, pin_memory=pin),
                                 h_out=torch.empty((nbytes,), dtype=torch.uint8, pin_memory=pin))
            if mapped:
                io["h_x0"] = torch.empty((B, 9 * N), dtype=dt, pin_memory=pin)
                io["h_x0_np"] = io["h_x0"].numpy()
            else:
                io["d_in"] = torch.empty((3, B, 3), dtype=dt, device=dev)
                io["d_out"] = ops.be.empty((nbytes,), "u8")
            io["h_in_np"] = io["h_in"].numpy()
            io["h_out_np"] = io["h_out"].numpy()
            if mapped:
                esz = 4 if suf == "f32" else 8
                o_x, o_acc, o_att, o_rates, o_thr, o_info, _ = ops._packed_offsets(B, N, esz)
                pin, base, stepb = io["h_in"].data_ptr(), io["h_out"].data_ptr(), B * 3 * esz
                io["ptr_in"] = (pin, pin + stepb, pin + 2 * stepb)
                io["ptr_out"] = (base + o_x, base + o_info, base + o_acc, base + o_att, base + o_rates, base + o_thr)
                io["ptr_x0"] = io["h_x0"].data_ptr()
                lanes = 64 if B == 1 else (8 if N <= 8 else 16 if N <= 16 else 32 if N <= 32 else 64)
                io["one_wave"] = B * lanes <= 64
                io["h_done"] = torch.zeros((8,), dtype=torch.int64, pin_memory=dev.type == "cuda")
                io["ptr_done"] = io["h_done"].data_ptr()
                io["ticket"] = 0
                io["plan_fn"] = getattr(ops.lib._dll, f"se3mpc_plan_host_{suf}")
                io["plan_stream"] = torch.cuda.Stream(dev) if (io["one_wave"] and dev.type == "cuda") else None
                io["plan_stream_handle"] = None if io["plan_stream"] is None else io["plan_stream"].cuda_stream
        if mapped and io["one_wave"]:
            cur, stream_handle = None, io["plan_stream_handle"]
        else:
            cur = torch.cuda.current_stream(dev) if dev.type == "cuda" else None
            stream_handle = None if cur is None else cur.cuda_stream
        hin = io["h_in_np"]
        hin[0] = p0; hin[1] = v0
        hin[2] = goal if goal is not None else 0.0
        if mapped:
            hx0 = None
            if x0 is not None:
                io["h_x0_np"][...] = x0
                hx0 = io["h_x0"]
            pin = io["ptr_in"]
            if io["one_wave"]:
                io["ticket"] = ticket = io["ticket"] + 1
                rc = io["plan_fn"](ctypes.byref(prm), B, pin[0], pin[1], pin[2] if prm.has_goal else 0, io["ptr_x0"] if hx0 is not None else 0,
                                   *io["ptr_out"], io["ptr_done"], ticket, 2000.0, stream_handle)
                if rc != 0:
                    ops.lib._check(f"se3mpc_plan_host_{suf}", rc)
                cur = None
            else:
                ops.lib.call("solve", suf, B, pin[0], pin[1], pin[2] if prm.has_goal else 0, io["ptr_x0"] if hx0 is not None else 0, *io["ptr_out"],
                             stream_handle, params=prm)
        else:
            io["d_in"].copy_(io["h_in"], non_blocking=True)
            dx0 = None if x0 is None else torch.from_numpy(np.ascontiguousarray(x0)).to(device=dev, dtype=dt)
            ops.solve_packed(prm, io["d_in"], x0=dx0, out=io["d_out"])
            io["h_out"].copy_(io["d_out"], non_blocking=True)
        if cur is not None:
            cur.synchronize()
        res = ops.unpack_solution(io["h_out_np"], B, N, suf)
        x = res["x"]
        res.update(positions=x[:, :3 * N].reshape(B, N, 3), velocities=x[:, 3 * N:6 * N].reshape(B, N, 3),
                   thrust_vectors=x[:, 6 * N:].reshape(B, N, 3))
        return res

    def plan_batch(self, positions, velocities, goals, x0=None, precision: Optional[str] = None) -> Dict[str, np.ndarray]:
        p0 = np.asarray(to_float(positions), float).reshape(-1, 3)
        v0 = np.asarray(to_float(velocities), float).reshape(-1, 3)
        g = np.asarray(to_float(goals), float).reshape(-1, 3)
        if not (p0.shape == v0.shape == g.shape):
            raise ValueError("positions, velocities and goals must all be (B, 3)")
        return self._solve_batch(p0, v0, g, x0, precision or "f32")

    def plan_with_restarts(self, current_state: DroneState, goal_position, n_restarts: int = 256, sigma: float = 1.0,
                           seed: int = 0, precision: Optional[str] = None, mapper=None, safety_margin: float = 1.0,
                           occupancy_threshold: float = 0.6) -> Trajectory:
        current_state, _, _ = self.sense(current_state, goal_position)
        N, R = self.se3_config.prediction_horizon, int(n_restarts)
        p0 = np.tile(np.asarray(to_float(current_state.position), float), (R, 1))
        v0 = np.tile(np.asarray(to_float(current_state.velocity), float), (R, 1))
        g = np.tile(self.goal_position, (R, 1))
        x0 = np.tile(self._cold_start(p0[0], v0[0], self.goal_position), (R, 1))
        rng = np.random.default_rng(seed)
        x0[1:, 6 * N:] += rng.normal(0.0, sigma, (R - 1, 3 * N))
        res = self._solve_batch(p0, v0, g, x0, precision or self.precision)
        fun = np.array(res["info"]["fun"], dtype=float)
        self.last_result = dict(fun_cold_start=float(fun[0]))
        if mapper is not None:
            safe, _ = mapper.trajectories_safe(res["positions"], safety_margin, occupancy_threshold)
            self.last_result["n_safe"] = int(safe.sum())
            if safe.any():
                fun = np.where(safe, fun, np.inf)
        best = int(np.argmin(fun))
        self.last_result.update(best_restart=best, fun=float(res["info"]["fun"][best]))
        sol = {k: res[k][best] for k in ("positions", "velocities", "thrust_vectors", "accelerations", "attitudes",
                                         "body_rates", "thrusts")}
        return self._create_trajectory_from_solution(sol, time.time())

    def _obstacle_table(self, obstacles) -> Optional[np.ndarray]:
        if obstacles is False:
            return None
        if obstacles is None or obstacles is True:
            if not self.obstacles:
                return None
            return np.array([[*np.asarray(to_float(c), float).reshape(3), float(r)] for c, r in self.obstacles], dtype=float)
        sph = np.asarray(obstacles, float).reshape(-1, 4)
        return sph if len(sph) else None

    def plan_shooting(self, current_state: DroneState, goal_position, n_samples: int = 8192, iters: int = 16, step: float = 0.9,
                      sigma: float = 2.0, seed: int = 0, precision: str = "f32", obstacles=None,
                      obstacle_weight: Optional[float] = None) -> Trajectory:
        import torch
        import torch.distributed as dist
        from ..distributed import sharded_shooting_plan
        current_state, _, _ = self.sense(current_state, goal_position)
        ops = self._get_ops()
        prm = self._params()
        N = self.se3_config.prediction_horizon
        p0 = np.asarray(to_float(current_state.position), float)
        v0 = np.asarray(to_float(current_state.velocity), float)
        sph = self._obstacle_table(obstacles)
        w_obs = float(self.se3_config.obstacle_weight if obstacle_weight is None else obstacle_weight)
        single = not (dist.is_available() and dist.is_initialized() and dist.get_world_size() > 1)
        if single and getattr(ops.be, "graph_capable", False):
            return self._plan_shooting_captured(ops, prm, p0, v0, int(n_samples), int(iters), float(step), float(sigma), int(seed), precision, sph, w_obs)
        best = sharded_shooting_plan(ops, prm, p0, v0, self.goal_position, n_samples, iters, step, sigma, seed, precision, spheres=sph,
                                     obstacle_weight=w_obs)
        dev = ops.be.device
        col = lambda a: torch.from_numpy(np.ascontiguousarray(np.asarray(a, float).reshape(-1, 1))).to(dev)
        T = col(best["T"].reshape(-1))
        cost, _, P, V = ops.rollout_cost_grad(prm, col(p0), col(v0), col(self.goal_position), T, want_grad=False, want_states=True)
        acc, att, rates, thr = ops.extract(prm, T)
        h = lambda a, shape: ops.be.to_host(a)[:, 0].reshape(shape).astype(float)
        self.last_result = dict(cost=float(ops.be.to_host(cost)[0]), sample=int(best["sample"]), owner=int(best["owner"]), n_samples=int(n_samples),
                                iters=int(iters), T=best["T"])
        if sph is not None:
            o = ops.rollout_iterate(prm, col(p0), col(v0), col(self.goal_position), T, 0, 0.0, want_grad=False, spheres=col(sph.reshape(-1)).reshape(-1, 4).contiguous(),
                                    obstacle_weight=w_obs)
            self.last_result.update(penalty=float(ops.be.to_host(o["penalty"])[0]), cost_with_penalty=float(ops.be.to_host(o["cost"])[0]))
        sol = {"positions": h(P, (N, 3)), "velocities": h(V, (N, 3)), "thrust_vectors": best["T"], "accelerations": h(acc, (N, 3)),
               "attitudes": h(att, (N, 3)), "body_rates": h(rates, (N, 3)), "thrusts": h(thr, (N,))}
        return self._create_trajectory_from_solution(sol, time.time())

    def _plan_shooting_captured(self, ops, prm, p0, v0, n_samples, iters, step, sigma, seed, precision, sph=None, w_obs=1000.0) -> Trajectory:
        import torch
        from ..distributed import shooting_samples
        N = prm.horizon
        K = 0 if sph is None else len(sph)
        key = (N, n_samples, iters, step, sigma, seed, precision, bytes(prm), K, w_obs)
        g = self._shooting_graphs.get(key) if hasattr(self, "_shooting_graphs") else None
        if g is None:
            if not hasattr(self, "_shooting_graphs"):
                self._shooting_graphs = {}
            dev = ops.be.device
            dt = torch.float32 if precision == "f32" else torch.float64
            io = dict(h_in=torch.zeros(9, dtype=torch.float64).pin_memory(), d_in=torch.zeros(9, dtype=torch.float64, device=dev),
                      h_out=torch.zeros(19 * N + 3, dtype=torch.float64).pin_memory(), h_key=torch.zeros(1, dtype=torch.int64).pin_memory(),
                      samples=shooting_samples(prm, n_samples, sigma, seed, dev, dt), wk=torch.zeros(((n_samples + 63) // 64,), dtype=torch.int64, device=dev))
            if K:
                io.update(h_sph=torch.zeros((K, 4), dtype=torch.float64).pin_memory(), d_sph=torch.zeros((K, 4), dtype=torch.float64, device=dev))

            io["wide"] = torch.empty((3, 3, n_samples), dtype=dt, device=dev)
            io["h_in_np"], io["h_out_np"], io["h_key_np"] = io["h_in"].numpy(), io["h_out"].numpy(), io["h_key"].numpy()
            if K:
                io["h_sph_np"] = io["h_sph"].numpy()

            def body():
                io["d_in"].copy_(io["h_in"], non_blocking=True)
                wide = io["wide"]
                wide.copy_(io["d_in"].view(3, 3, 1).expand(3, 3, n_samples))
                sph_d = None
                if K:
                    io["d_sph"].copy_(io["h_sph"], non_blocking=True)
                    sph_d = io["d_sph"].to(dt)
                out = ops.rollout_iterate(prm, wide[0], wide[1], wide[2], io["samples"], iters, step, want_grad=False, wave_keys=io["wk"], index_base=0,
                                          spheres=sph_d, obstacle_weight=w_obs, want_penalty=False)
                ops.shooting_finish(prm, out["T"], io["wk"], io["d_in"], io["h_out"], key_out=io["h_key"], spheres=io["d_sph"] if K else None,
                                    obstacle_weight=w_obs)

            side = torch.cuda.Stream(device=dev)
            side.wait_stream(torch.cuda.current_stream(dev))
            with torch.cuda.stream(side):
                body()
            torch.cuda.current_stream(dev).wait_stream(side)
            torch.cuda.synchronize(dev)
            graph = torch.cuda.CUDAGraph()
            with torch.cuda.graph(graph, capture_error_mode="thread_local"):
                body()
            if len(self._shooting_graphs) >= 4:
                self._shooting_graphs.pop(next(iter(self._shooting_graphs)))
            g = self._shooting_graphs[key] = (graph, io)
        graph, io = g
        hin = io["h_in_np"]
        hin[0:3] = p0; hin[3:6] = v0; hin[6:9] = self.goal_position
        if K:
            io["h_sph_np"][...] = sph
        graph.replay()
        torch.cuda.current_stream(ops.be.device).synchronize()
        r = io["h_out_np"]
        kh = int(io["h_key_np"][0]) & 0xFFFFFFFFFFFFFFFF
        blk = lambda i: r[3 * N * i:3 * N * (i + 1)].reshape(N, 3).copy()
        self.last_result = dict(cost=float(r[19 * N]), sample=int(ops.lib.key_index(kh)), owner=0, n_samples=n_samples, iters=iters, T=blk(2))
        if K:
            self.last_result.update(penalty=float(r[19 * N + 1]), cost_with_penalty=float(r[19 * N + 2]))
        sol = {"positions": blk(0), "velocities": blk(1), "thrust_vectors": blk(2), "accelerations": blk(3), "attitudes": blk(4),
               "body_rates": blk(5), "thrusts": r[18 * N:19 * N].copy()}
        return self._create_trajectory_from_solution(sol, time.time())

    MPPI_SAMPLES = 1024
    MPPI_ITERS = 8
    MPPI_SIGMA = 4.0
    MPPI_TEMPERATURE = 100.0

    def _mppi_nominal(self, N: int, warm_start: bool):
        st = getattr(self, "_mppi_state", None)
        hover = np.tile([0.0, 0.0, self.hover_thrust], (N, 1))
        if not warm_start or st is None or st["U"].shape[0] != N or not np.array_equal(st["goal"], self.goal_position):
            return hover, 0
        U = np.empty((N, 3))
        U[:N - 1] = st["U"][1:]
        U[N - 1] = hover[0]
        return U, 1

    MPPI_SPLIT_SAMPLES = 256
    MPPI_SPLIT_WORKGROUPS = 1024

    @classmethod
    def _mppi_splits(cls, splits, n_samples: int, n_problems: int = 1) -> Optional[int]:
        if splits is None:
            return None
        if splits == "auto":
            g = max(1, min(int(n_samples) // cls.MPPI_SPLIT_SAMPLES, cls.MPPI_SPLIT_WORKGROUPS // max(int(n_problems), 1)))
            while g > 1 and int(n_samples) % (64 * g):
                g -= 1
            return g if g > 1 else None
        if isinstance(splits, (bool, str)) or int(splits) != splits:
            raise ValueError(f"splits: expected None, \"auto\" or an integer, got {splits!r}")
        return int(splits)

    @staticmethod
    def _mppi_op(ops, splits, *a, workspace=None, **kw):
        if splits is None:
            return ops.mppi(*a, **kw)
        return ops.mppi_split(*a, splits=splits, workspace=workspace, **kw)

    def plan_mppi(self, current_state: DroneState, goal_position, n_samples: int = MPPI_SAMPLES, iters: int = MPPI_ITERS,
                  sigma: float = MPPI_SIGMA, temperature: float = MPPI_TEMPERATURE, seed: int = 0, precision: str = "f32", obstacles=None,
                  obstacle_weight: Optional[float] = None, warm_start: bool = True, splits=None) -> Trajectory:
        current_state, _, _ = self.sense(current_state, goal_position)
        ops = self._get_ops()
        prm = self._params()
        N = self.se3_config.prediction_horizon
        p0 = np.asarray(to_float(current_state.position), float)
        v0 = np.asarray(to_float(current_state.velocity), float)
        sph = self._obstacle_table(obstacles)
        w_obs = float(self.se3_config.obstacle_weight if obstacle_weight is None else obstacle_weight)
        U0, shift = self._mppi_nominal(N, warm_start)
        it_base = getattr(self, "_mppi_iter_base", 0)
        splits = self._mppi_splits(splits, n_samples)
        args = (ops, prm, p0, v0, U0, int(n_samples), int(iters), float(sigma), float(temperature), int(seed), precision, sph, w_obs, it_base, splits)
        if getattr(ops.be, "graph_capable", False):
            r, trace = self._plan_mppi_captured(*args)
        else:
            r, trace = self._plan_mppi_eager(*args)
        self._mppi_iter_base = (it_base + int(iters)) & 0xFFFFFFFF
        blk = lambda i: r[3 * N * i:3 * N * (i + 1)].reshape(N, 3).copy()
        self._mppi_state = dict(U=blk(2), goal=np.array(self.goal_position, dtype=float))
        self.last_result = dict(cost=float(r[19 * N]), penalty=float(r[19 * N + 1]), cost_with_penalty=float(r[19 * N + 2]), trace=trace,
                                shift=shift, iter_base=it_base, n_samples=int(n_samples), iters=int(iters), U=blk(2), splits=splits)
        sol = {"positions": blk(0), "velocities": blk(1), "thrust_vectors": blk(2), "accelerations": blk(3), "attitudes": blk(4),
               "body_rates": blk(5), "thrusts": r[18 * N:19 * N].copy()}
        return self._create_trajectory_from_solution(sol, time.time())

    def _plan_mppi_eager(self, ops, prm, p0, v0, U0, n_samples, iters, sigma, temperature, seed, precision, sph, w_obs, it_base, splits=None):
        N = prm.horizon
        be = ops.be
        suf = "f32" if precision == "f32" else "f64"
        col = lambda a, kind: be.from_host(np.ascontiguousarray(np.asarray(a, float).reshape(-1, 1).astype(np.float32 if kind == "f32" else np.float64)))
        state = be.from_host(np.concatenate([p0, v0, self.goal_position]).astype(np.float64))
        sph_r = None if sph is None else be.from_host(np.ascontiguousarray(sph.astype(np.float32 if suf == "f32" else np.float64)))
        out = self._mppi_op(ops, splits, prm, col(p0, suf), col(v0, suf), col(self.goal_position, suf), col(U0, suf), n_samples, iters, sigma,
                            temperature, seed=seed, iter_base=it_base, spheres=sph_r, obstacle_weight=w_obs)
        res = be.empty((19 * N + 3,), "f64")
        sph_d = None if sph is None else be.from_host(np.ascontiguousarray(sph.astype(np.float64)))
        ops.shooting_finish(prm, out["U"], out["keys"], state, res, spheres=sph_d, obstacle_weight=w_obs)
        return np.asarray(be.to_host(res), dtype=float).copy(), np.asarray(be.to_host(out["trace"]), dtype=float)[:, 0].copy()

    def _plan_mppi_captured(self, ops, prm, p0, v0, U0, n_samples, iters, sigma, temperature, seed, precision, sph, w_obs, it_base, splits=None):
        import torch
        N = prm.horizon
        K = 0 if sph is None else len(sph)
        key = (N, n_samples, iters, sigma, temperature, seed, precision, bytes(prm), K, w_obs, splits)
        graphs = self.__dict__.setdefault("_mppi_graphs", {})
        g = graphs.get(key)
        if g is None:
            dev = ops.be.device
            dt = torch.float32 if precision == "f32" else torch.float64
            pin = lambda n, t=torch.float64: torch.zeros(n, dtype=t).pin_memory()
            io = dict(h_in=pin(9 + 3 * N), d_in=torch.zeros(9 + 3 * N, dtype=torch.float64, device=dev), h_it=pin(1, torch.int32),
                      d_it=torch.zeros(1, dtype=torch.int32, device=dev), h_out=pin(19 * N + 3), h_trace=pin(max(iters, 1), dt),
                      d_U=torch.empty((3 * N, 1), dtype=dt, device=dev), d_cost=torch.empty(1, dtype=dt, device=dev),
                      d_trace=torch.empty((max(iters, 1), 1), dtype=dt, device=dev), d_keys=torch.empty(1, dtype=torch.int64, device=dev),
                      d_s=torch.empty((3, 3, 1), dtype=dt, device=dev), d_U0=torch.empty((3 * N, 1), dtype=dt, device=dev))
            if K:
                io.update(h_sph=pin((K, 4)), d_sph=torch.zeros((K, 4), dtype=torch.float64, device=dev), d_sph_r=torch.empty((K, 4), dtype=dt, device=dev))
            io["d_ws"] = None if splits is None else ops.mppi_split_workspace(prm, 1, splits)
            io["h_in_np"], io["h_it_np"], io["h_out_np"], io["h_trace_np"] = (io[k].numpy() for k in ("h_in", "h_it", "h_out", "h_trace"))
            if K:
                io["h_sph_np"] = io["h_sph"].numpy()

            def body():
                io["d_in"].copy_(io["h_in"], non_blocking=True)
                io["d_it"].copy_(io["h_it"], non_blocking=True)
                io["d_s"].copy_(io["d_in"][:9].view(3, 3, 1))
                io["d_U0"].copy_(io["d_in"][9:].view(3 * N, 1))
                if K:
                    io["d_sph"].copy_(io["h_sph"], non_blocking=True)
                    io["d_sph_r"].copy_(io["d_sph"])
                self._mppi_op(ops, splits, prm, io["d_s"][0], io["d_s"][1], io["d_s"][2], io["d_U0"], n_samples, iters, sigma, temperature, seed=seed,
                              iter_base=0, iter_offset=io["d_it"], spheres=io["d_sph_r"] if K else None, obstacle_weight=w_obs,
                              out=(io["d_U"], io["d_cost"], io["d_trace"], io["d_keys"]), workspace=io["d_ws"])
                ops.shooting_finish(prm, io["d_U"], io["d_keys"], io["d_in"], io["h_out"], spheres=io["d_sph"] if K else None, obstacle_weight=w_obs)
                io["h_trace"].copy_(io["d_trace"].view(-1), non_blocking=True)

            side = torch.cuda.Stream(device=dev)
            side.wait_stream(torch.cuda.current_stream(dev))
            with torch.cuda.stream(side):
                body()
            torch.cuda.current_stream(dev).wait_stream(side)
            torch.cuda.synchronize(dev)
            graph = torch.cuda.CUDAGraph()
            with torch.cuda.graph(graph, capture_error_mode="thread_local"):
                body()
            if len(graphs) >= 4:
                graphs.pop(next(iter(graphs)))
            g = graphs[key] = (graph, io)
        graph, io = g
        hin = io["h_in_np"]
        hin[0:3] = p0; hin[3:6] = v0; hin[6:9] = self.goal_position; hin[9:] = U0.reshape(-1)
        io["h_it_np"][0] = np.array(it_base, dtype=np.uint32).view(np.int32)
        if K:
            io["h_sph_np"][...] = sph
        graph.replay()
        torch.cuda.current_stream(ops.be.device).synchronize()
        return io["h_out_np"].copy(), io["h_trace_np"][:iters].astype(float)

    def plan_batch_mppi(self, positions, velocities, goals, n_samples: int = MPPI_SAMPLES, iters: int = MPPI_ITERS, sigma: float = MPPI_SIGMA,
                        temperature: float = MPPI_TEMPERATURE, seed: int = 0, precision: Optional[str] = None, obstacles=None,
                        obstacle_weight: Optional[float] = None, nominal=None, iter_base: int = 0, splits=None) -> Dict[str, np.ndarray]:
# ... 226 lines not shown
```

### include/se3mpc.h

```cpp
#ifndef SE3MPC_H
#define SE3MPC_H

#include <stddef.h>
#include <stdint.h>

#ifdef __cplusplus
extern "C" {
#endif

#define SE3MPC_ABI_VERSION 1
#define SE3MPC_MAX_HORIZON 64
#define SE3MPC_MAX_CORRECTIONS 10
#define SE3MPC_MAX_SPHERES 256

enum se3mpc_status {
  SE3MPC_OK = 0,
  SE3MPC_ERR_NULL = -1,
  SE3MPC_ERR_HORIZON = -2,
  SE3MPC_ERR_SHAPE = -3,
  SE3MPC_ERR_PARAM = -4,
  SE3MPC_ERR_WORKSPACE = -5,
  SE3MPC_ERR_LAUNCH = -6,
  SE3MPC_ERR_NO_DEVICE = -7
};

typedef struct se3mpc_params {
  int32_t horizon;
  int32_t has_goal;
  double dt;
  double mass;
  double gravity;
  double position_weight;
  double velocity_weight;
  double acceleration_weight;
  double thrust_weight;
  double terminal_factor;
  double position_bound;
  double max_velocity;
  double max_acceleration;
  double max_thrust;
  double min_thrust;
  double max_tilt_angle;
  double safety_margin;
  int32_t max_iterations;
  int32_t max_corrections;
  int32_t max_linesearch;
  int32_t max_fun;
  double pgtol;
  double ftol;
} se3mpc_params;

typedef struct se3mpc_solve_info {
  double fun;
  int32_t nit;
  int32_t nfev;
  int32_t status;
  int32_t task;
} se3mpc_solve_info;

enum se3mpc_task {
  SE3MPC_TASK_CONV_PGTOL = 1,
  SE3MPC_TASK_CONV_FTOL = 2,
  SE3MPC_TASK_STOP_MAXITER = 3,
  SE3MPC_TASK_STOP_MAXFUN = 4,
  SE3MPC_TASK_ABNORMAL = 5,
  SE3MPC_TASK_OVERFLOW = 6
};

int se3mpc_abi_version(void);
const char* se3mpc_last_error(void);
int se3mpc_device_count(void);
int se3mpc_default_params(se3mpc_params* out);
int se3mpc_check_params(const se3mpc_params* p);


int se3mpc_init_f32(const se3mpc_params* p, int B, int ld, const float* p0, const float* v0,
                    const float* goal, int project, float* X0, void* stream);
int se3mpc_init_f64(const se3mpc_params* p, int B, int ld, const double* p0, const double* v0,
                    const double* goal, int project, double* X0, void* stream);

int se3mpc_cost_grad_f32(const se3mpc_params* p, int B, int ld, const float* X, const float* goal,
                         float* f, float* g, void* stream);
int se3mpc_cost_grad_f64(const se3mpc_params* p, int B, int ld, const double* X, const double* goal,
                         double* f, double* g, void* stream);

int se3mpc_dynamics_residual_f32(const se3mpc_params* p, int B, int ld, const float* X, const float* p0,
                                 const float* v0, float* R, void* stream);
int se3mpc_dynamics_residual_f64(const se3mpc_params* p, int B, int ld, const double* X, const double* p0,
                                 const double* v0, double* R, void* stream);

int se3mpc_obstacle_residual_f32(const se3mpc_params* p, int B, int ld, const float* X, const float* spheres,
                                 int K, float* C, float* cmin, float* viol, void* stream);
int se3mpc_obstacle_residual_f64(const se3mpc_params* p, int B, int ld, const double* X, const double* spheres,
                                 int K, double* C, double* cmin, double* viol, void* stream);

int se3mpc_physical_constraints_f32(const se3mpc_params* p, int B, int ld, const float* X, float* C, void* stream);
int se3mpc_physical_constraints_f64(const se3mpc_params* p, int B, int ld, const double* X, double* C, void* stream);

int se3mpc_extract_f32(const se3mpc_params* p, int B, int ld, const float* T, float* acc, float* att,
                       float* rates, float* thrust, void* stream);
int se3mpc_extract_f64(const se3mpc_params* p, int B, int ld, const double* T, double* acc, double* att,
                       double* rates, double* thrust, void* stream);

int se3mpc_rollout_cost_grad_f32(const se3mpc_params* p, int B, int ld, const float* p0, const float* v0,
                                 const float* goal, const float* T, float* cost, float* gradT, float* P,
                                 float* V, uint64_t* wave_keys, uint32_t index_base, void* stream);
int se3mpc_rollout_cost_grad_f64(const se3mpc_params* p, int B, int ld, const double* p0, const double* v0,
                                 const double* goal, const double* T, double* cost, double* gradT, double* P,
                                 double* V, uint64_t* wave_keys, uint32_t index_base, void* stream);

int se3mpc_rollout_cost_grad_batched_f32(const se3mpc_params* p, int B, int ld, int nbatch, const float* p0,
                                         const float* v0, const float* goal, const float* T, float* cost,
                                         float* gradT, uint64_t* wave_keys, uint32_t index_base, void* stream);
int se3mpc_rollout_cost_grad_batched_f64(const se3mpc_params* p, int B, int ld, int nbatch, const double* p0,
                                         const double* v0, const double* goal, const double* T, double* cost,
                                         double* gradT, uint64_t* wave_keys, uint32_t index_base, void* stream);

int se3mpc_rollout_obstacles_f32(const se3mpc_params* p, int B, int ld, const float* p0, const float* v0,
                                 const float* goal, const float* T, float* cost, float* gradT, const float* spheres,
                                 int K, float* cmin, float* viol, uint64_t* wave_keys, uint32_t index_base, void* stream);
int se3mpc_rollout_obstacles_f64(const se3mpc_params* p, int B, int ld, const double* p0, const double* v0,
                                 const double* goal, const double* T, double* cost, double* gradT, const double* spheres,
                                 int K, double* cmin, double* viol, uint64_t* wave_keys, uint32_t index_base, void* stream);

int se3mpc_rollout_obstacles_batched_f32(const se3mpc_params* p, int B, int ld, int nbatch, const float* p0,
                                         const float* v0, const float* goal, const float* T, float* cost, float* gradT,
                                         const float* spheres, int K, float* cmin, float* viol, uint64_t* wave_keys,
                                         uint32_t index_base, void* stream);
int se3mpc_rollout_obstacles_batched_f64(const se3mpc_params* p, int B, int ld, int nbatch, const double* p0,
                                         const double* v0, const double* goal, const double* T, double* cost, double* gradT,
                                         const double* spheres, int K, double* cmin, double* viol, uint64_t* wave_keys,
                                         uint32_t index_base, void* stream);

int se3mpc_rollout_iterate_f32(const se3mpc_params* p, int B, int ld, int nbatch, int iters, double step, const float* p0,
                               const float* v0, const float* goal, const float* T_in, float* T_out, float* cost_first, float* cost,
                               float* gradT, uint64_t* wave_keys, uint32_t index_base, void* stream);
int se3mpc_rollout_iterate_f64(const se3mpc_params* p, int B, int ld, int nbatch, int iters, double step, const double* p0,
                               const double* v0, const double* goal, const double* T_in, double* T_out, double* cost_first, double* cost,
                               double* gradT, uint64_t* wave_keys, uint32_t index_base, void* stream);
int se3mpc_rollout_iterate_obstacles_f32(const se3mpc_params* p, int B, int ld, int nbatch, int iters, double step, const float* p0,
                                         const float* v0, const float* goal, const float* T_in, float* T_out, float* cost_first,
                                         float* cost, float* gradT, const float* spheres, int K, double obstacle_weight,
                                         float* penalty, uint64_t* wave_keys, uint32_t index_base, void* stream);
int se3mpc_rollout_iterate_obstacles_f64(const se3mpc_params* p, int B, int ld, int nbatch, int iters, double step, const double* p0,
                                         const double* v0, const double* goal, const double* T_in, double* T_out, double* cost_first,
                                         double* cost, double* gradT, const double* spheres, int K, double obstacle_weight,
                                         double* penalty, uint64_t* wave_keys, uint32_t index_base, void* stream);
int se3mpc_projected_step_f32(const se3mpc_params* p, int B, int ld, double step, const float* T, const float* gradT, float* T_out,
                              void* stream);
int se3mpc_projected_step_f64(const se3mpc_params* p, int B, int ld, double step, const double* T, const double* gradT, double* T_out,
                              void* stream);

int se3mpc_shooting_finish_f32(const se3mpc_params* p, int B, int ld, const float* T, const uint64_t* wave_keys, int n_slots,
                               uint32_t index_base, const double* state, const double* spheres, int K, double obstacle_weight, double* out,
                               uint64_t* key_out, void* stream);
int se3mpc_shooting_finish_f64(const se3mpc_params* p, int B, int ld, const double* T, const uint64_t* wave_keys, int n_slots,
                               uint32_t index_base, const double* state, const double* spheres, int K, double obstacle_weight, double* out,
                               uint64_t* key_out, void* stream);

int se3mpc_reduce_keys(const uint64_t* wave_keys, int per_batch, int nbatch, uint64_t* keys_out, void* stream);

int se3mpc_set_rollout_variant(int variant);

int se3mpc_is_plan_valid_f32(const se3mpc_params* p, int B, int ld, const float* P, const float* V,
                             int32_t* valid, void* stream);
int se3mpc_is_plan_valid_f64(const se3mpc_params* p, int B, int ld, const double* P, const double* V,
                             int32_t* valid, void* stream);

int se3mpc_argmin_f32(int B, const float* cost, uint32_t index_base, uint64_t* key, void* stream);
int se3mpc_argmin_f64(int B, const double* cost, uint32_t index_base, uint64_t* key, void* stream);
uint32_t se3mpc_key_index(uint64_t key);
float se3mpc_key_cost(uint64_t key);

int se3mpc_population_workspace(int rows, int B);
int se3mpc_population_sums_f32(int rows, int B, int ld, const float* X, const float* cost, double cost_ref,
                               const uint64_t* ref_key, double temperature, double* out, double* workspace, void* stream);
int se3mpc_population_sums_f64(int rows, int B, int ld, const double* X, const double* cost, double cost_ref,
                               const uint64_t* ref_key, double temperature, double* out, double* workspace, void* stream);

int se3mpc_mppi_f32(const se3mpc_params* p, int nprob, int ld, int S, int iters, double sigma, double temperature, uint64_t seed,
                    uint32_t iter_base, const uint32_t* iter_offset, uint32_t index_base, const float* p0, const float* v0, const float* goal,
                    const float* U_in, float* U_out, const float* spheres, int K, double obstacle_weight, float* cost, float* trace,
                    uint64_t* keys, void* stream);
int se3mpc_mppi_f64(const se3mpc_params* p, int nprob, int ld, int S, int iters, double sigma, double temperature, uint64_t seed,
                    uint32_t iter_base, const uint32_t* iter_offset, uint32_t index_base, const double* p0, const double* v0, const double* goal,
                    const double* U_in, double* U_out, const double* spheres, int K, double obstacle_weight, double* cost, double* trace,
                    uint64_t* keys, void* stream);
size_t se3mpc_mppi_split_workspace_bytes(int horizon, int nprob, int splits);
int se3mpc_mppi_split_f32(const se3mpc_params* p, int nprob, int ld, int S, int iters, double sigma, double temperature, uint64_t seed,
                          uint32_t iter_base, const uint32_t* iter_offset, uint32_t index_base, const float* p0, const float* v0,
                          const float* goal, const float* U_in, float* U_out, const float* spheres, int K, double obstacle_weight, float* cost,
                          float* trace, uint64_t* keys, int splits, void* workspace, size_t workspace_bytes, void* stream);
int se3mpc_mppi_split_f64(const se3mpc_params* p, int nprob, int ld, int S, int iters, double sigma, double temperature, uint64_t seed,
                          uint32_t iter_base, const uint32_t* iter_offset, uint32_t index_base, const double* p0, const double* v0,
                          const double* goal, const double* U_in, double* U_out, const double* spheres, int K, double obstacle_weight,
                          double* cost, double* trace, uint64_t* keys, int splits, void* workspace, size_t workspace_bytes, void* stream);
int se3mpc_mppi_samples_f32(const se3mpc_params* p, int nprob, int ld, int S, double sigma, uint64_t seed, uint32_t iter_base,
                            uint32_t index_base, const float* U_in, float* T_out, int ld_out, float* noise, uint32_t* raw, void* stream);
int se3mpc_mppi_samples_f64(const se3mpc_params* p, int nprob, int ld, int S, double sigma, uint64_t seed, uint32_t iter_base,
                            uint32_t index_base, const double* U_in, double* T_out, int ld_out, double* noise, uint32_t* raw, void* stream);

int se3mpc_spheres_from_grid_f32(const float* positions, const float* occupancy, int M, double threshold, int target,
                                 double radius, float* spheres, int cap, int32_t* count, void* stream);
int se3mpc_spheres_from_grid_f64(const double* positions, const double* occupancy, int M, double threshold, int target,
                                 double radius, double* spheres, int cap, int32_t* count, void* stream);

int se3mpc_transpose_f32(int rows, int cols, const float* in, int ld_in, float* out, int ld_out, void* stream);
int se3mpc_transpose_f64(int rows, int cols, const double* in, int ld_in, double* out, int ld_out, void* stream);

#define SE3MPC_VOXEL_EMPTY 0xFFFFFFFFFFFFFFFFull
#define SE3MPC_VOXEL_MAX_CELLS 1024

typedef struct se3mpc_voxel_map {
  uint64_t* keys;
  double* prob;
  int32_t* count;
  int32_t capacity;
  int32_t reserved;
  double resolution;
  double prior;
} se3mpc_voxel_map;

int se3mpc_voxel_clear(const se3mpc_voxel_map* m, void* stream);
int se3mpc_voxel_insert(const se3mpc_voxel_map* m, const int32_t* ijk, const double* prob, double value,
                        const int32_t* count_in, int M, int32_t* failed, void* stream);
#define SE3MPC_VOXEL_MAX_RAYS 1024
int se3mpc_voxel_update_rays(const se3mpc_voxel_map* m, const double* origin, const double* direction,
                             const double* distance, const int32_t* hit, int M, double like_hit, double like_miss,
                             uint64_t* ray_keys, int32_t* ray_len, int max_len, int32_t* slot_rows, uint64_t* row_bits,
                             int32_t* stats, void* stream);
long long se3mpc_voxel_update_row_words(int M, int max_len);
int se3mpc_voxel_trace_rays(const se3mpc_voxel_map* m, const double* origin, const double* direction,
                            const double* distance, int M, uint64_t* ray_keys, int32_t* ray_len, int max_len,
                            int32_t* stats, void* stream);
int se3mpc_voxel_export(const se3mpc_voxel_map* m, int32_t* ijk_out, double* prob_out, int32_t* count_out,
                        int32_t* n_out, void* stream);
int se3mpc_voxel_query_f32(const se3mpc_voxel_map* m, const float* positions, int M, double* occupancy, void* stream);
int se3mpc_voxel_query_f64(const se3mpc_voxel_map* m, const double* positions, int M, double* occupancy, void* stream);
int se3mpc_voxel_trajectory_safe_f32(const se3mpc_voxel_map* m, const float* P, int B, int N, long long stride,
                                     double margin, double threshold, int32_t* safe, int32_t* first, void* stream);
int se3mpc_voxel_trajectory_safe_f64(const se3mpc_voxel_map* m, const double* P, int B, int N, long long stride,
                                     double margin, double threshold, int32_t* safe, int32_t* first, void* stream);
int se3mpc_voxel_local_workspace(int cells_per_axis);
int se3mpc_voxel_local_spheres_f32(const se3mpc_voxel_map* m, const double* centre, double size, double threshold,
                                   int target, double radius, float* spheres, int cap, int32_t* count,
                                   int32_t* workspace, void* stream);
int se3mpc_voxel_local_spheres_f64(const se3mpc_voxel_map* m, const double* centre, double size, double threshold,
                                   int target, double radius, double* spheres, int cap, int32_t* count,
                                   int32_t* workspace, void* stream);


typedef struct se3mpc_controller_params {
  double kp_pos[3], ki_pos[3], kd_pos[3];
  double kp_att[3], kd_att[3];
  double inertia[3];
  double max_torque_xyz[3];
  double max_integral_per_axis[3];
  double max_integral_pos;
  double max_tilt_angle;
  double mass, gravity;
  double max_thrust, min_thrust;
  double tracking_error_threshold, velocity_error_threshold;
  double back_calculation_gain;
  double integral_decay_factor;
  double saturation_threshold;
  double yaw_singularity_threshold;
  double default_heading_yaw;
  int32_t anti_windup_method;
  int32_t yaw_fallback_method;
} se3mpc_controller_params;

typedef struct se3mpc_simulator_params {
  double mass, gravity, inertia[3], max_thrust, max_torque;
} se3mpc_simulator_params;

#define SE3MPC_CONTROLLER_STATE_WORDS 12

int se3mpc_controller_default_params(se3mpc_controller_params* out);
int se3mpc_simulator_default_params(se3mpc_simulator_params* out);
int se3mpc_controller_reset(const se3mpc_controller_params* cp, int B, double* state, void* stream);

int se3mpc_control_f32(const se3mpc_controller_params* cp, int B, const double* time, const float* pos, const float* vel,
                       const float* att, const float* omega, const float* dpos, const float* dvel, const float* dacc,
                       const float* yaw, const float* yaw_rate, double* state, float* thrust, float* torque, float* body_thrust,
                       float* body_rates, int32_t* flags, void* stream);
int se3mpc_control_f64(const se3mpc_controller_params* cp, int B, const double* time, const double* pos, const double* vel,
                       const double* att, const double* omega, const double* dpos, const double* dvel, const double* dacc,
                       const double* yaw, const double* yaw_rate, double* state, double* thrust, double* torque, double* body_thrust,
                       double* body_rates, int32_t* flags, void* stream);

int se3mpc_control_fast_f32(const se3mpc_controller_params* cp, double vehicle_mass, double vehicle_gravity, int B, double dt,
                            const float* pos, const float* vel, const float* att, const float* omega, const float* dpos,
                            const float* dvel, const float* dacc, const float* yaw, const float* yaw_rate, double* state, float* thrust,
                            float* torque, int32_t* flags, void* stream);
int se3mpc_control_fast_f64(const se3mpc_controller_params* cp, double vehicle_mass, double vehicle_gravity, int B, double dt,
                            const double* pos, const double* vel, const double* att, const double* omega, const double* dpos,
                            const double* dvel, const double* dacc, const double* yaw, const double* yaw_rate, double* state,
                            double* thrust, double* torque, int32_t* flags, void* stream);

int se3mpc_controller_integral_update_f32(const se3mpc_controller_params* cp, int B, const float* vel_error, double dt,
                                          const int32_t* saturation, double* state, void* stream);
int se3mpc_controller_integral_update_f64(const se3mpc_controller_params* cp, int B, const double* vel_error, double dt,
                                          const int32_t* saturation, double* state, void* stream);
int se3mpc_controller_attitude_torque_f32(const se3mpc_controller_params* cp, int B, const float* att, const float* omega,
                                          const float* b3_des, const float* yaw, const float* yaw_rate, const double* inertia,
                                          double* state, float* torque, int32_t* flags, void* stream);
int se3mpc_controller_attitude_torque_f64(const se3mpc_controller_params* cp, int B, const double* att, const double* omega,
                                          const double* b3_des, const double* yaw, const double* yaw_rate, const double* inertia,
                                          double* state, double* torque, int32_t* flags, void* stream);
int se3mpc_controller_desired_frame_f32(const se3mpc_controller_params* cp, int B, int method, const float* yaw_vector,
                                        const float* b3_des, const float* current_yaw, float* frame, float* cos_angle,
// ... 130 lines not shown
```

Before: 8.045 billion.

## Fuse shooting iterate and finish into single kernel with last-block tail

Adds a shooting_plan entry point that runs the rollout iterations, stores only each wave's best candidate thrust column, and uses an atomic counter so the last workgroup runs the finish step. Broadcast state and spheres now come from one packed buffer read from shared state rather than an expanded wide copy. This removes the state broadcast copy, a separate finish launch, the sphere dtype conversion and the full T_out write. The cost is a threadfence/atomic tail and a serial final wave, and it only applies to the planner's graph-captured shooting path.

```diff
diff --git a/dart_planner_amd/capi.py b/dart_planner_amd/capi.py
--- a/dart_planner_amd/capi.py
+++ b/dart_planner_amd/capi.py
@@ -166,6 +166,8 @@
     "rollout_iterate": (True, [_I, _I, _I, _I, _D, _P, _P, _P, _P, _P, _P, _P, _P, _P, C.c_uint32, _P]),
     "rollout_iterate_obstacles": (True, [_I, _I, _I, _I, _D, _P, _P, _P, _P, _P, _P, _P, _P, _P, _I, _D, _P, _P, C.c_uint32, _P]),
     "shooting_finish": (True, [_I, _I, _P, _P, _I, C.c_uint32, _P, _P, _I, _D, _P, _P, _P]),
+    "shooting_plan": (True, [_I, _I, _I, _D, _P, _P, _P, _P, _P, _P, _P, _P]),
+    "shooting_plan_obstacles": (True, [_I, _I, _I, _D, _P, _P, _P, _I, _D, _P, _P, _P, _P, _P, _P]),
     "projected_step": (True, [_I, _I, _D, _P, _P, _P, _P]),
     "is_plan_valid": (True, [_I, _I, _P, _P, _P, _P]),
     "argmin": (False, [_I, _P, C.c_uint32, _P, _P]),
@@ -233,6 +235,7 @@
     "se3mpc_key_index": (C.c_uint32, [C.c_uint64]),
     "se3mpc_key_cost": (C.c_float, [C.c_uint64]),
     "se3mpc_population_workspace": (C.c_int, [_I, _I]),
+    "se3mpc_shooting_plan_columns": (C.c_int, [_I, _I, _I, _I]),
     "se3mpc_mppi_split_workspace_bytes": (C.c_size_t, [_I, _I, _I]),
 }
 
@@ -314,6 +317,12 @@
     def reduce_keys(self, wave_keys: int, per_batch: int, nbatch: int, keys_out: int, stream: int) -> None:
         self._check("se3mpc_reduce_keys", self._dll.se3mpc_reduce_keys(wave_keys, per_batch, nbatch, keys_out, stream))
 
+    def shooting_plan_columns(self, horizon: int, B: int, ld: int, elem_bytes: int) -> int:
+        n = self._dll.se3mpc_shooting_plan_columns(horizon, B, ld, elem_bytes)
+        if n < 0:
+            self._check("se3mpc_shooting_plan_columns", n)
+        return n
+
     def population_workspace(self, rows: int, B: int) -> int:
         return self._dll.se3mpc_population_workspace(rows, B)
 
diff --git a/dart_planner_amd/csrc/reduce_kernels.hip b/dart_planner_amd/csrc/reduce_kernels.hip
--- a/dart_planner_amd/csrc/reduce_kernels.hip
+++ b/dart_planner_amd/csrc/reduce_kernels.hip
@@ -85,105 +85,7 @@
 shooting_finish_kernel(DevParams<double> q, int B, int ld, const IO* __restrict__ T, const unsigned long long* __restrict__ wave_keys,
                        int n_slots, uint32_t index_base, const double* __restrict__ state, const double* __restrict__ spheres, int K,
                        double w_obs, double* __restrict__ out, unsigned long long* __restrict__ key_out) {
-  __shared__ double sT[3][kWave], sP[3][kWave], sV[3][kWave], sC[3];
-  const int lane = threadIdx.x, N = q.N;
-  unsigned long long best = ~0ull;
-  for (int i = lane; i < n_slots; i += kWave) best = wave_keys[i] < best ? wave_keys[i] : best;
-  for (int off = 32; off > 0; off >>= 1) {
-    const unsigned long long o = __shfl_down(best, off, kWave);
-    best = o < best ? o : best;
-  }
-  best = __shfl(best, 0, kWave);
-  if (lane == 0 && key_out != nullptr) *key_out = best;
-  uint32_t idx = (uint32_t)(best & 0xFFFFFFFFull) - index_base;
-  if (idx >= (uint32_t)B) idx = 0;
-  const bool live = lane < N;
-  double t0 = 0.0, t1 = 0.0, t2 = 0.0;
-  if (live) {
-    t0 = (double)T[(size_t)(3 * lane + 0) * ld + idx]; t1 = (double)T[(size_t)(3 * lane + 1) * ld + idx]; t2 = (double)T[(size_t)(3 * lane + 2) * ld + idx];
-  }
-  sT[0][lane] = t0; sT[1][lane] = t1; sT[2][lane] = t2;
-  __syncthreads();
-  if (lane < 3) {
-    const int a = lane;
-    const AxisConsts<double> c = axis_consts<double>(q, a, q.has_goal ? state[6 + a] : 0.0);
-    double p = state[a], v = state[3 + a];
-    RolloutSums<double> s = {0, 0, 0, 0, 0};
-    for (int k = 0; k < N; ++k) {
-      const double tk = sT[a][k];
-      const double acc = tk * q.inv_mass - c.grav, dev = tk - c.hov, e = p - c.gl;
-      sP[a][k] = p; sV[a][k] = v;
-      if (k == N - 1) s.sterm = e * e; else s.sp += e * e;
-      s.sv += v * v; s.sa += acc * acc; s.st += dev * dev;
-      p = p + v * q.dt + q.half_dt2 * acc;
-      v = v + acc * q.dt;
-    }
-    s.sp += s.sterm;
-    sC[a] = axis_cost(q, s);
-  }
-  __syncthreads();
-  const double cost = sC[0] + sC[1] + sC[2];
-  const double mag = sqrt(t0 * t0 + t1 * t1 + t2 * t2);
-  const bool valid = live && mag > 1e-6;
-  double b1[3] = {0, 0, 0}, b2[3] = {0, 0, 0}, b3[3] = {0, 0, 0};
-  double roll = 0.0, pitch = 0.0, yaw = 0.0;
-  double n1 = 0.0;
-  if (valid) {
-    b3[0] = t0 / mag; b3[1] = t1 / mag; b3[2] = t2 / mag;
-    b1[0] = 0.0; b1[1] = -b3[2]; b1[2] = b3[1];
-    n1 = sqrt(b1[1] * b1[1] + b1[2] * b1[2]);
-    if (n1 > 1e-6) { b1[1] /= n1; b1[2] /= n1; } else { b1[0] = 1.0; b1[1] = 0.0; b1[2] = 0.0; }
-    b2[0] = b3[1] * b1[2] - b3[2] * b1[1];
-    b2[1] = b3[2] * b1[0] - b3[0] * b1[2];
-    b2[2] = b3[0] * b1[1] - b3[1] * b1[0];
-    roll = atan2(b2[2], b3[2]);
-    pitch = asin(fmin(fmax(-b1[2], -1.0), 1.0));
-    yaw = n1 > 1e-6 ? (b1[1] == 0.0 ? b1[1] : copysign(1.5707963267948966, b1[1])) : 0.0;
-  }
-  const uint64_t vmask = wave_ballot(valid);
-  const uint64_t below = vmask & ((lane == 0) ? 0ull : (~0ull >> (64 - lane)));
-  const bool has_prev = valid && below != 0ull;
-  const int pk = has_prev ? 63 - __builtin_clzll(below) : lane;
-  double q1[3], q2[3], q3[3];
-#pragma unroll
-  for (int c = 0; c < 3; ++c) { q1[c] = group_gather<kWave>(b1[c], pk); q2[c] = group_gather<kWave>(b2[c], pk); q3[c] = group_gather<kWave>(b3[c], pk); }
-  double w0 = 0.0, w1 = 0.0, w2 = 0.0;
-  if (has_prev) {
-    double d1[3], d2[3], d3[3];
-    for (int c = 0; c < 3; ++c) {
-      d1[c] = (b1[c] - q1[c]) / q.dt;
-      d2[c] = (b2[c] - q2[c]) / q.dt;
-      d3[c] = (b3[c] - q3[c]) / q.dt;
-    }
-    w0 = b3[0] * d2[0] + b3[1] * d2[1] + b3[2] * d2[2];
-    w1 = b1[0] * d3[0] + b1[1] * d3[1] + b1[2] * d3[2];
-    w2 = b2[0] * d1[0] + b2[1] * d1[1] + b2[2] * d1[2];
-  }
-  double pen = 0.0;
-  if (spheres != nullptr && K > 0) {
-    double pl = 0.0;
-    if (live) {
-      const double px = sP[0][lane], py = sP[1][lane], pz = sP[2][lane];
-      for (int j = 0; j < K; ++j) {
-        const double dx = px - spheres[4 * j], dy = py - spheres[4 * j + 1], dz = pz - spheres[4 * j + 2], sm = spheres[4 * j + 3] + q.margin;
-        const double h = fmax(0.0, -((dx * dx + dy * dy + dz * dz) - sm * sm));
-        pl += h * h;
-      }
-    }
-    pen = w_obs * wave_sum(pl);
-  }
-  if (live) {
-    const int k = lane;
-    double* o = out;
-    o[3 * k] = sP[0][k]; o[3 * k + 1] = sP[1][k]; o[3 * k + 2] = sP[2][k]; o += 3 * N;
-    o[3 * k] = sV[0][k]; o[3 * k + 1] = sV[1][k]; o[3 * k + 2] = sV[2][k]; o += 3 * N;
-    o[3 * k] = t0; o[3 * k + 1] = t1; o[3 * k + 2] = t2; o += 3 * N;
-    o[3 * k] = t0 / q.mass; o[3 * k + 1] = t1 / q.mass; o[3 * k + 2] = t2 / q.mass - q.grav; o += 3 * N;
-    o[3 * k] = roll; o[3 * k + 1] = pitch; o[3 * k + 2] = yaw; o += 3 * N;
-    o[3 * k] = w0; o[3 * k + 1] = w1; o[3 * k + 2] = w2; o += 3 * N;
-    o[k] = mag;
-  }
-  if (lane == 0) { out[19 * N] = cost; out[19 * N + 1] = pen; out[19 * N + 2] = cost + pen; }
+  shooting_finish_wave<IO>(q, B, ld, T, 1, wave_keys, n_slots, index_base, state, spheres, K, w_obs, out, key_out);
 }
 
 template <typename R>
diff --git a/dart_planner_amd/csrc/rollout_device.hpp b/dart_planner_amd/csrc/rollout_device.hpp
--- a/dart_planner_amd/csrc/rollout_device.hpp
+++ b/dart_planner_amd/csrc/rollout_device.hpp
@@ -170,6 +170,113 @@
   return axis_cost(q, s);
 }
 
+template <typename IO>
+__device__ __forceinline__ void shooting_finish_wave(const DevParams<double>& q, int B, int ld, const IO* T, int col_div,
+                                                     const unsigned long long* wave_keys, int n_slots, uint32_t index_base,
+                                                     const double* __restrict__ state, const double* __restrict__ spheres, int K, double w_obs,
+                                                     double* __restrict__ out, unsigned long long* __restrict__ key_out) {
+  __shared__ double sT[3][kWave], sP[3][kWave], sV[3][kWave], sC[3];
+  const int lane = lane_id(), N = q.N;
+  unsigned long long best = ~0ull;
+  for (int i = lane; i < n_slots; i += kWave) best = wave_keys[i] < best ? wave_keys[i] : best;
+  for (int off = 32; off > 0; off >>= 1) {
+    const unsigned long long o = __shfl_down(best, off, kWave);
+    best = o < best ? o : best;
+  }
+  best = __shfl(best, 0, kWave);
+  if (lane == 0 && key_out != nullptr) *key_out = best;
+  uint32_t idx = (uint32_t)(best & 0xFFFFFFFFull) - index_base;
+  if (idx >= (uint32_t)B) idx = 0;
+  const size_t col = idx / (uint32_t)col_div;
+  const bool live = lane < N;
+  double t0 = 0.0, t1 = 0.0, t2 = 0.0;
+  if (live) {
+    t0 = (double)T[(size_t)(3 * lane + 0) * ld + col]; t1 = (double)T[(size_t)(3 * lane + 1) * ld + col]; t2 = (double)T[(size_t)(3 * lane + 2) * ld + col];
+  }
+  sT[0][lane] = t0; sT[1][lane] = t1; sT[2][lane] = t2;
+  group_sync<kWave>();
+  if (lane < 3) {
+    const int a = lane;
+    const AxisConsts<double> c = axis_consts<double>(q, a, q.has_goal ? state[6 + a] : 0.0);
+    double p = state[a], v = state[3 + a];
+    RolloutSums<double> s = {0, 0, 0, 0, 0};
+    for (int k = 0; k < N; ++k) {
+      const double tk = sT[a][k];
+      const double acc = tk * q.inv_mass - c.grav, dev = tk - c.hov, e = p - c.gl;
+      sP[a][k] = p; sV[a][k] = v;
+      if (k == N - 1) s.sterm = e * e; else s.sp += e * e;
+      s.sv += v * v; s.sa += acc * acc; s.st += dev * dev;
+      p = p + v * q.dt + q.half_dt2 * acc;
+      v = v + acc * q.dt;
+    }
+    s.sp += s.sterm;
+    sC[a] = axis_cost(q, s);
+  }
+  group_sync<kWave>();
+  const double cost = sC[0] + sC[1] + sC[2];
+  const double mag = sqrt(t0 * t0 + t1 * t1 + t2 * t2);
+  const bool valid = live && mag > 1e-6;
+  double b1[3] = {0, 0, 0}, b2[3] = {0, 0, 0}, b3[3] = {0, 0, 0};
+  double roll = 0.0, pitch = 0.0, yaw = 0.0;
+  double n1 = 0.0;
+  if (valid) {
+    b3[0] = t0 / mag; b3[1] = t1 / mag; b3[2] = t2 / mag;
+    b1[0] = 0.0; b1[1] = -b3[2]; b1[2] = b3[1];
+    n1 = sqrt(b1[1] * b1[1] + b1[2] * b1[2]);
+    if (n1 > 1e-6) { b1[1] /= n1; b1[2] /= n1; } else { b1[0] = 1.0; b1[1] = 0.0; b1[2] = 0.0; }
+    b2[0] = b3[1] * b1[2] - b3[2] * b1[1];
+    b2[1] = b3[2] * b1[0] - b3[0] * b1[2];
+    b2[2] = b3[0] * b1[1] - b3[1] * b1[0];
+    roll = atan2(b2[2], b3[2]);
+    pitch = asin(fmin(fmax(-b1[2], -1.0), 1.0));
+    yaw = n1 > 1e-6 ? (b1[1] == 0.0 ? b1[1] : copysign(1.5707963267948966, b1[1])) : 0.0;
+  }
+  const uint64_t vmask = wave_ballot(valid);
+  const uint64_t below = vmask & ((lane == 0) ? 0ull : (~0ull >> (64 - lane)));
+  const bool has_prev = valid && below != 0ull;
+  const int pk = has_prev ? 63 - __builtin_clzll(below) : lane;
+  double q1[3], q2[3], q3[3];
+#pragma unroll
+  for (int c = 0; c < 3; ++c) { q1[c] = group_gather<kWave>(b1[c], pk); q2[c] = group_gather<kWave>(b2[c], pk); q3[c] = group_gather<kWave>(b3[c], pk); }
+  double w0 = 0.0, w1 = 0.0, w2 = 0.0;
+  if (has_prev) {
+    double d1[3], d2[3], d3[3];
+    for (int c = 0; c < 3; ++c) {
+      d1[c] = (b1[c] - q1[c]) / q.dt;
+      d2[c] = (b2[c] - q2[c]) / q.dt;
+      d3[c] = (b3[c] - q3[c]) / q.dt;
+    }
+    w0 = b3[0] * d2[0] + b3[1] * d2[1] + b3[2] * d2[2];
+    w1 = b1[0] * d3[0] + b1[1] * d3[1] + b1[2] * d3[2];
+    w2 = b2[0] * d1[0] + b2[1] * d1[1] + b2[2] * d1[2];
+  }
+  double pen = 0.0;
+  if (spheres != nullptr && K > 0) {
+    double pl = 0.0;
+    if (live) {
+      const double px = sP[0][lane], py = sP[1][lane], pz = sP[2][lane];
+      for (int j = 0; j < K; ++j) {
+        const double dx = px - spheres[4 * j], dy = py - spheres[4 * j + 1], dz = pz - spheres[4 * j + 2], sm = spheres[4 * j + 3] + q.margin;
+        const double h = fmax(0.0, -((dx * dx + dy * dy + dz * dz) - sm * sm));
+        pl += h * h;
+      }
+    }
+    pen = w_obs * wave_sum(pl);
+  }
+  if (live) {
+    const int k = lane;
+    double* o = out;
+    o[3 * k] = sP[0][k]; o[3 * k + 1] = sP[1][k]; o[3 * k + 2] = sP[2][k]; o += 3 * N;
+    o[3 * k] = sV[0][k]; o[3 * k + 1] = sV[1][k]; o[3 * k + 2] = sV[2][k]; o += 3 * N;
+    o[3 * k] = t0; o[3 * k + 1] = t1; o[3 * k + 2] = t2; o += 3 * N;
+    o[3 * k] = t0 / q.mass; o[3 * k + 1] = t1 / q.mass; o[3 * k + 2] = t2 / q.mass - q.grav; o += 3 * N;
+    o[3 * k] = roll; o[3 * k + 1] = pitch; o[3 * k + 2] = yaw; o += 3 * N;
+    o[3 * k] = w0; o[3 * k + 1] = w1; o[3 * k + 2] = w2; o += 3 * N;
+    o[k] = mag;
+  }
+  if (lane == 0) { out[19 * N] = cost; out[19 * N + 1] = pen; out[19 * N + 2] = cost + pen; }
+}
+
 typedef float obs_f2 __attribute__((vector_size(8)));
 #ifndef SE3MPC_OBS_PACKED
 #define SE3MPC_OBS_PACKED 1
diff --git a/dart_planner_amd/csrc/rollout_iterate.hip b/dart_planner_amd/csrc/rollout_iterate.hip
--- a/dart_planner_amd/csrc/rollout_iterate.hip
+++ b/dart_planner_amd/csrc/rollout_iterate.hip
@@ -179,20 +179,60 @@
   }
 }
 
-template <typename R, int N, bool EXACT, int LDAUX, int STAUX, bool OBS = false, int TS = kWave>
+template <typename R>
+struct PlanOperands {
+  DevParams<double> q64;
+  const double* state;
+  R* cand;
+  int cand_ld;
+  unsigned long long* keys;
+  int* counter;
+  const double* spheres;
+  int K;
+  double w_obs;
+  double* out;
+  unsigned long long* key_out;
+};
+struct NoPlan {};
+template <typename R, bool PLAN> using PlanArg = std::conditional_t<PLAN, PlanOperands<R>, NoPlan>;
+struct NoPick {
+  template <typename R> __device__ __forceinline__ int operator()(R, R) const { return -1; }
+};
+template <bool PLAN, typename R>
+__device__ __forceinline__ R state_ld(const R* __restrict__ lanes, const double* __restrict__ shared9, int i, int a, unsigned voff, unsigned rowb) {
+  if constexpr (PLAN) return (R)shared9[3 * i + a];
+  else return lane_ld(lane_buf(lanes), voff, (unsigned)(a) * rowb);
+}
+
+template <typename R>
+__device__ __forceinline__ void plan_tail(const PlanOperands<R>& po, int B, int nwg, int col_div) {
+  __threadfence();
+  __syncthreads();
+  if (threadIdx.x >= kWave) return;
+  int prev = 0;
+  if (threadIdx.x == 0) prev = atomicAdd(po.counter, 1);
+  if (wave_bcast(prev, 0) != nwg - 1) return;
+  __threadfence();
+  shooting_finish_wave<R>(po.q64, B, po.cand_ld, po.cand, col_div, po.keys, nwg, 0u, po.state, po.K > 0 ? po.spheres : nullptr, po.K, po.w_obs, po.out,
+                          po.key_out);
+  if (threadIdx.x == 0) *po.counter = 0;
+}
+
+template <typename R, int N, bool EXACT, int LDAUX, int STAUX, bool OBS = false, int TS = kWave, bool PLAN = false, typename PICK = NoPick>
 __device__ __forceinline__ R iterate_axis_reg(const DevParams<R>& q, int a, unsigned voff, unsigned rowb, const R* __restrict__ p0,
                                               const R* __restrict__ v0, const R* __restrict__ goal, const R* __restrict__ Tin,
                                               R* __restrict__ Tout, R* __restrict__ gradT, int iters, R step, bool live, bool want_first,
-                                              R& cost_first, const ObsCtx<R>* obs = nullptr) {
+                                              R& cost_first, const ObsCtx<R>* obs = nullptr, const double* __restrict__ state = nullptr,
+                                              const PICK& pick = PICK(), R* cand_col = nullptr, int cand_ld = 0) {
   const int Nn = EXACT ? N : q.N;
   R t[N], es[N], vs[N];
 #pragma unroll
   for (int k = 0; k < N; ++k) {
     if (EXACT || k < Nn) t[k] = lane_ld<LDAUX>(lane_buf(Tin), voff, (unsigned)(3 * k + a) * rowb);
   }
-  const AxisConsts<R> c = axis_consts<R>(q, a, q.has_goal ? lane_ld(lane_buf(goal), voff, (unsigned)(a) * rowb) : (R)0);
-  const R pinit = lane_ld(lane_buf(p0), voff, (unsigned)(a) * rowb);
-  const R vinit = lane_ld(lane_buf(v0), voff, (unsigned)(a) * rowb);
+  const AxisConsts<R> c = axis_consts<R>(q, a, q.has_goal ? state_ld<PLAN>(goal, state, 2, a, voff, rowb) : (R)0);
+  const R pinit = state_ld<PLAN>(p0, state, 0, a, voff, rowb);
+  const R vinit = state_ld<PLAN>(v0, state, 1, a, voff, rowb);
   const R lo = (a == 2) ? q.tz_lo : -q.txy, hi = (a == 2) ? q.tz_hi : q.txy;
   const int lane_ = (int)(threadIdx.x & (kWave - 1));
   R* my_tile = nullptr;
@@ -285,7 +325,15 @@
       }
     }
   }
-  if (live) {
+  if constexpr (PLAN) {
+    const int src = pick(cost, cost_first);
+    if (lane_ == src) {
+#pragma unroll
+      for (int k = 0; k < N; ++k) {
+        if (EXACT || k < Nn) cand_col[(size_t)(3 * k + a) * cand_ld] = t[k];
+      }
+    }
+  } else if (live) {
     if (gradT != nullptr) {
 #pragma unroll
       for (int k = 0; k < N; ++k) {
@@ -300,11 +348,11 @@
   return cost;
 }
 
-template <typename R, bool OBS = false, int TS = kWave>
+template <typename R, bool OBS = false, int TS = kWave, bool PLAN = false>
 __device__ __forceinline__ R iterate_axis_mem(const DevParams<R>& q, int a, unsigned voff, unsigned rowb, const R* __restrict__ p0,
                                               const R* __restrict__ v0, const R* __restrict__ goal, const R* __restrict__ Tin,
                                               R* __restrict__ Tout, R* __restrict__ gradT, int iters, R step, bool live, bool want_first,
-                                              R& cost_first, const ObsCtx<R>* obs = nullptr) {
+                                              R& cost_first, const ObsCtx<R>* obs = nullptr, const double* __restrict__ state = nullptr) {
   (void)want_first;
   const int N = q.N;
   const int lane_ = (int)(threadIdx.x & (kWave - 1));
@@ -313,9 +361,9 @@
   }
   R* my_tile = nullptr;
   if constexpr (OBS) my_tile = obs->tile + (size_t)a * N * kWave + lane_;
-  const AxisConsts<R> c = axis_consts<R>(q, a, q.has_goal ? lane_ld(lane_buf(goal), voff, (unsigned)(a) * rowb) : (R)0);
-  const R pinit = lane_ld(lane_buf(p0), voff, (unsigned)(a) * rowb);
-  const R vinit = lane_ld(lane_buf(v0), voff, (unsigned)(a) * rowb);
+  const AxisConsts<R> c = axis_consts<R>(q, a, q.has_goal ? state_ld<PLAN>(goal, state, 2, a, voff, rowb) : (R)0);
+  const R pinit = state_ld<PLAN>(p0, state, 0, a, voff, rowb);
+  const R vinit = state_ld<PLAN>(v0, state, 1, a, voff, rowb);
   const R lo = (a == 2) ? q.tz_lo : -q.txy, hi = (a == 2) ? q.tz_hi : q.txy;
   if (Tin != Tout && live) {
     for (int k = 0; k < N; ++k) lane_st(lane_buf(Tout), voff, (unsigned)(3 * k + a) * rowb, lane_ld(lane_buf(Tin), voff, (unsigned)(3 * k + a) * rowb));
@@ -373,12 +421,13 @@
   return cost;
 }
 
-template <typename R, int N, bool REG, int FLAGS>
+template <typename R, int N, bool REG, int FLAGS, bool PLAN = false>
 __global__ void __launch_bounds__(192)
 rollout_iterate_kernel(DevParams<R> q, int B, int ld, int iters, R step, const R* __restrict__ p0, const R* __restrict__ v0,
                        const R* __restrict__ goal, const R* __restrict__ Tin, R* __restrict__ Tout, R* __restrict__ cost_first,
-                       R* __restrict__ cost, R* __restrict__ gradT, unsigned long long* __restrict__ key, uint32_t index_base) {
-  {
+                       R* __restrict__ cost, R* __restrict__ gradT, unsigned long long* __restrict__ key, uint32_t index_base,
+                       PlanArg<R, PLAN> po) {
+  if constexpr (!PLAN) {
     const size_t bi = blockIdx.y, ss = (size_t)3 * ld, st = (size_t)3 * q.N * ld;
     p0 += bi * ss; v0 += bi * ss; Tin += bi * st; Tout += bi * st; cost += bi * (size_t)ld;
     if (goal != nullptr) goal += bi * ss;
@@ -396,6 +445,27 @@
   __shared__ R part[2][3][kWave];
   const int a = wave_uniform((int)(threadIdx.x / kWave));
   R c0 = (R)0, c;
+  if constexpr (PLAN) {
+    auto pick = [&](R ca, R) -> int {
+      part[0][a][lane] = ca;
+      __syncthreads();
+      const R total = part[0][0][lane] + part[0][1][lane] + part[0][2][lane];
+      const uint32_t bits = live ? orderable_bits((float)total) : 0xFFFFFFFFu;
+      const uint32_t m = wave_min_u32(bits);
+      const int src = first_lane(wave_ballot(live && bits == m));
+      if (a == 0 && lane == src) po.keys[blk] = ((unsigned long long)m << 32) | (unsigned long long)(uint32_t)b;
+      return src;
+    };
+    if constexpr (REG) {
+      (void)iterate_axis_reg<R, N, !(FLAGS & 8), (FLAGS & 1) ? 2 : 0, 0, false, kWave, true>(q, a, voff, rowb, p0, v0, goal, Tin, Tout, gradT, iters, step, live, false,
+                                                                                             c0, nullptr, po.state, pick, po.cand + blk, po.cand_ld);
+    } else {
+      c = iterate_axis_mem<R, false, kWave, true>(q, a, voff, rowb, p0, v0, goal, Tin, Tout, gradT, iters, step, live, false, c0, nullptr, po.state);
+      (void)pick(c, c0);
+    }
+    plan_tail<R>(po, B, (int)gridDim.x, REG ? kWave : 1);
+    return;
+  }
   if constexpr (REG) c = iterate_axis_reg<R, N, !(FLAGS & 8), (FLAGS & 1) ? 2 : 0, (FLAGS & 2) ? 2 : 0>(q, a, voff, rowb, p0, v0, goal, Tin, Tout, gradT, iters, step, live, cost_first != nullptr, c0);
   else c = iterate_axis_mem<R>(q, a, voff, rowb, p0, v0, goal, Tin, Tout, gradT, iters, step, live, cost_first != nullptr, c0);
   part[0][a][lane] = c; part[1][a][lane] = c0;
@@ -412,15 +482,15 @@
 #define SE3MPC_OBS_WIDE_TS 32
 #endif
 constexpr int kObsWideW = SE3MPC_OBS_WIDE_W, kObsWideTS = SE3MPC_OBS_WIDE_TS;
-template <typename R, int N, bool REG, int FLAGS, int W, int TS>
+template <typename R, int N, bool REG, int FLAGS, int W, int TS, bool PLAN = false>
 __global__ void __launch_bounds__(64 * W)
 rollout_iterate_obstacles_kernel(DevParams<R> q, int B, int ld, int iters, R step, const R* __restrict__ p0, const R* __restrict__ v0,
                                  const R* __restrict__ goal, const R* __restrict__ Tin, R* __restrict__ Tout, R* __restrict__ cost_first,
                                  R* __restrict__ cost, R* __restrict__ gradT, const R* __restrict__ spheres, int K, R w_obs,
-                                 R* __restrict__ penalty, unsigned long long* __restrict__ key, uint32_t index_base) {
+                                 R* __restrict__ penalty, unsigned long long* __restrict__ key, uint32_t index_base, PlanArg<R, PLAN> po) {
   HIP_DYNAMIC_SHARED(unsigned char, lds_raw)
   constexpr int SUBS = kWave / TS;
-  {
+  if constexpr (!PLAN) {
     const size_t bi = blockIdx.y, ss = (size_t)3 * ld, st = (size_t)3 * q.N * ld;
     p0 += bi * ss; v0 += bi * ss; Tin += bi * st; Tout += bi * st; cost += bi * (size_t)ld;
     if (goal != nullptr) goal += bi * ss;
@@ -436,8 +506,11 @@
   R* ppen = pcost + 6 * kWave;
   for (int i = threadIdx.x; i < Kpad; i += 64 * W) {
     if (i < K) {
-      const R sm = spheres[4 * i + 3] + q.margin;
-      sph[4 * i + 0] = spheres[4 * i + 0]; sph[4 * i + 1] = spheres[4 * i + 1]; sph[4 * i + 2] = spheres[4 * i + 2]; sph[4 * i + 3] = sm * sm;
+      R s4[4];
+      if constexpr (PLAN) { for (int j = 0; j < 4; ++j) s4[j] = (R)po.spheres[4 * i + j]; }
+      else { for (int j = 0; j < 4; ++j) s4[j] = spheres[4 * i + j]; }
+      const R sm = s4[3] + q.margin;
+      sph[4 * i + 0] = s4[0]; sph[4 * i + 1] = s4[1]; sph[4 * i + 2] = s4[2]; sph[4 * i + 3] = sm * sm;
     } else {
       sph[4 * i + 0] = (R)0; sph[4 * i + 1] = (R)0; sph[4 * i + 2] = (R)0; sph[4 * i + 3] = (R)-INFINITY;
     }
@@ -457,7 +530,38 @@
   if (o.axis_sweeps) { o.slot = a * SUBS + sub; o.slots = W * SUBS; }
   else { o.slot = (a - 3) * SUBS + sub; o.slots = (W - 3) * SUBS; }
   if constexpr (W > 3) __syncthreads();
-  if (a < 3) {
+  auto pick = [&](R ca, R) -> int {
+    if (a < 3) pcost[a * kWave + lane] = ca;
+    __syncthreads();
+    R total = pcost[0 * kWave + lane] + pcost[1 * kWave + lane] + pcost[2 * kWave + lane];
+    R pen = (R)0;
+#pragma unroll
+    for (int w = 0; w < W; ++w) {
+#pragma unroll
+      for (int h = 0; h < SUBS; ++h) pen += ppen[w * kWave + h * TS + tl];
+    }
+    total += pen;
+    const uint32_t bits = live ? orderable_bits((float)total) : 0xFFFFFFFFu;
+    const uint32_t m = wave_min_u32(bits);
+    const int src = first_lane(wave_ballot(live && bits == m));
+    if constexpr (PLAN) {
+      if (a == 0 && lane == src) po.keys[blk] = ((unsigned long long)m << 32) | (unsigned long long)(uint32_t)b;
+    }
+    return src;
+  };
+  (void)pick;
+  if (PLAN && a < 3) {
+    if constexpr (PLAN) {
+      R c0 = (R)0;
+      if constexpr (REG) {
+        (void)iterate_axis_reg<R, N, !(FLAGS & 8), (FLAGS & 1) ? 2 : 0, 0, true, TS, true>(q, a, voff, rowb, p0, v0, goal, Tin, Tout, gradT, iters, step, live, false, c0,
+                                                                                            &o, po.state, pick, po.cand + blk, po.cand_ld);
+      } else {
+        const R c = iterate_axis_mem<R, true, TS, true>(q, a, voff, rowb, p0, v0, goal, Tin, Tout, gradT, iters, step, live, false, c0, &o, po.state);
+        (void)pick(c, c0);
+      }
+    }
+  } else if (a < 3) {
     R c0 = (R)0, c;
     if constexpr (REG) c = iterate_axis_reg<R, N, !(FLAGS & 8), (FLAGS & 1) ? 2 : 0, (FLAGS & 2) ? 2 : 0, true, TS>(q, a, voff, rowb, p0, v0, goal, Tin, Tout, gradT, iters, step, live, cost_first != nullptr, c0, &o);
     else c = iterate_axis_mem<R, true, TS>(q, a, voff, rowb, p0, v0, goal, Tin, Tout, gradT, iters, step, live, cost_first != nullptr, c0, &o);
@@ -473,6 +577,11 @@
       if (kp == 3) helper_passes_regs<R, 3, TS>(o, q.N, a, lane, passes);
       else helper_passes_regs<R, 4, TS>(o, q.N, a, lane, passes);
     }
+    if constexpr (PLAN) (void)pick((R)0, (R)0);
+  }
+  if constexpr (PLAN) {
+    plan_tail<R>(po, B, (int)gridDim.x, REG ? TS : 1);
+    return;
   }
   __syncthreads();
   R total = pcost[0 * kWave + lane] + pcost[1 * kWave + lane] + pcost[2 * kWave + lane];
@@ -526,7 +635,7 @@
   dispatch_horizon<R, true>(N, kSweepAuto, [&](auto sweep) {
     using S = decltype(sweep);
     hipLaunchKernelGGL((rollout_iterate_kernel<R, S::NN, S::REG, S::FLAGS>), dim3(nblk, nbatch), dim3(192), 0, s, q, B, ld, iters, (R)step, p0, v0,
-                       goal, Tin, Tout, cost_first, cost, gradT, key, index_base);
+                       goal, Tin, Tout, cost_first, cost, gradT, key, index_base, NoPlan{});
   });
   return launch_status("se3mpc_rollout_iterate");
 }
@@ -561,12 +670,70 @@
                                   hipFuncAttributeMaxDynamicSharedMemorySize, (int)lds);
       hipLaunchKernelGGL((rollout_iterate_obstacles_kernel<R, S::NN, S::REG, S::FLAGS, WW, TT>), dim3(grid_for(B, TT), nbatch), dim3(64 * WW),
                          lds, s, q, B, ld, iters, (R)step, p0, v0, goal, Tin, Tout, cost_first, cost, gradT, spheres, K,
-                         (R)obstacle_weight, penalty, key, index_base);
+                         (R)obstacle_weight, penalty, key, index_base, NoPlan{});
     };
     if (wide) launch(std::integral_constant<int, kObsWideW>{}, std::integral_constant<int, kObsWideTS>{});
     else launch(std::integral_constant<int, 3>{}, std::integral_constant<int, kWave>{});
   });
   return launch_status("se3mpc_rollout_iterate_obstacles");
+}
+
+template <typename R>
+int plan_candidate_columns(int N, int B, int ld) {
+  int cols = 2 * grid_for(B, kWave);
+  dispatch_horizon<R, true>(N, kSweepAuto, [&](auto sweep) {
+    if (!decltype(sweep)::REG) cols = ld;
+  });
+  return cols;
+}
+
+template <typename R>
+int shooting_plan_impl(const se3mpc_params* p, int B, int ld, int iters, double step, const double* state, const R* samples, bool obstacles,
+                       const double* spheres, int K, double obstacle_weight, R* cand, uint64_t* wave_keys, int32_t* counter, double* out,
+                       uint64_t* key_out, void* stream) {
+  if (iters < 0 || iters > 1000000 || K < 0 || K > SE3MPC_MAX_SPHERES) return SE3MPC_ERR_SHAPE;
+  int rc = check_lane_args(p, B, ld, p ? 3LL * p->horizon : 0, sizeof(R));
+  if (rc) return rc;
+  if (B < 1) return SE3MPC_ERR_SHAPE;
+  if (!std::isfinite(step) || !std::isfinite(obstacle_weight) || obstacle_weight < 0.0) return SE3MPC_ERR_PARAM;
+  if (!state || !samples || !cand || !wave_keys || !counter || !out || (K > 0 && !spheres)) return SE3MPC_ERR_NULL;
+  const int N = p->horizon;
+  const DevParams<R> q = make_dev_params<R>(*p);
+  PlanOperands<R> po;
+  po.q64 = make_dev_params<double>(*p);
+  po.state = state; po.cand = cand; po.cand_ld = plan_candidate_columns<R>(N, B, ld);
+  po.keys = reinterpret_cast<unsigned long long*>(wave_keys); po.counter = counter;
+  po.spheres = K > 0 ? spheres : nullptr; po.K = K; po.w_obs = obstacle_weight;
+  po.out = out; po.key_out = reinterpret_cast<unsigned long long*>(key_out);
+  hipStream_t s = (hipStream_t)stream;
+  const R* nul = nullptr;
+  R* nulw = nullptr;
+  if (!obstacles) {
+    dispatch_horizon<R, true>(N, kSweepAuto, [&](auto sweep) {
+      using S = decltype(sweep);
+      hipLaunchKernelGGL((rollout_iterate_kernel<R, S::NN, S::REG, S::FLAGS, true>), dim3(grid_for(B, kWave)), dim3(192), 0, s, q, B, ld, iters, (R)step,
+                         nul, nul, nul, samples, S::REG ? nulw : cand, nulw, nulw, nulw, (unsigned long long*)nullptr, 0u, po);
+    });
+    return launch_status("se3mpc_shooting_plan");
+  }
+  const bool wide = ((g_lane_tuning.rollout_variant >> 7) & 3) != 1;
+  const int Kpad = (K + 7) / 8 * 8;
+  dispatch_horizon<R, true>(N, kSweepAuto, [&](auto sweep) {
+    using S = decltype(sweep);
+    auto launch = [&](auto w, auto ts) {
+      constexpr int WW = decltype(w)::value, TT = decltype(ts)::value;
+      const size_t lds = ((size_t)3 * N * kWave + (size_t)4 * Kpad + (size_t)(6 + 2 * WW) * kWave) * sizeof(R);
+      if (lds + 8 * 1024 > 64 * 1024)
+        (void)hipFuncSetAttribute(reinterpret_cast<const void*>(&rollout_iterate_obstacles_kernel<R, S::NN, S::REG, S::FLAGS, WW, TT, true>),
+                                  hipFuncAttributeMaxDynamicSharedMemorySize, (int)lds);
+      hipLaunchKernelGGL((rollout_iterate_obstacles_kernel<R, S::NN, S::REG, S::FLAGS, WW, TT, true>), dim3(grid_for(B, TT)), dim3(64 * WW), lds, s, q, B,
+                         ld, iters, (R)step, nul, nul, nul, samples, S::REG ? nulw : cand, nulw, nulw, nulw, nul, K, (R)obstacle_weight, nulw,
+                         (unsigned long long*)nullptr, 0u, po);
+    };
+    if (wide) launch(std::integral_constant<int, kObsWideW>{}, std::integral_constant<int, kObsWideTS>{});
+    else launch(std::integral_constant<int, 3>{}, std::integral_constant<int, kWave>{});
+  });
+  return launch_status("se3mpc_shooting_plan_obstacles");
 }
 
 template <typename R>
@@ -611,6 +778,30 @@
   return rollout_iterate_obstacles_impl<double>(p, B, ld, nbatch, iters, step, p0, v0, goal, T_in, T_out, cost_first, cost, gradT, spheres, K,
                                                 obstacle_weight, penalty, wave_keys, index_base, stream);
 }
+extern "C" int se3mpc_shooting_plan_columns(int horizon, int B, int ld, int elem_bytes) {
+  if (horizon < 1 || horizon > SE3MPC_MAX_HORIZON || B < 0 || ld < B || (elem_bytes != 4 && elem_bytes != 8)) return SE3MPC_ERR_SHAPE;
+  return elem_bytes == 4 ? plan_candidate_columns<float>(horizon, B, ld) : plan_candidate_columns<double>(horizon, B, ld);
+}
+extern "C" int se3mpc_shooting_plan_f32(const se3mpc_params* p, int B, int ld, int iters, double step, const double* state, const float* samples_T,
+                                        float* candidates, uint64_t* wave_keys, int32_t* counter, double* out, uint64_t* key_out, void* stream) {
+  return shooting_plan_impl<float>(p, B, ld, iters, step, state, samples_T, false, nullptr, 0, 0.0, candidates, wave_keys, counter, out, key_out, stream);
+}
+extern "C" int se3mpc_shooting_plan_f64(const se3mpc_params* p, int B, int ld, int iters, double step, const double* state, const double* samples_T,
+                                        double* candidates, uint64_t* wave_keys, int32_t* counter, double* out, uint64_t* key_out, void* stream) {
+  return shooting_plan_impl<double>(p, B, ld, iters, step, state, samples_T, false, nullptr, 0, 0.0, candidates, wave_keys, counter, out, key_out, stream);
+}
+extern "C" int se3mpc_shooting_plan_obstacles_f32(const se3mpc_params* p, int B, int ld, int iters, double step, const double* state,
+                                                  const float* samples_T, const double* spheres, int K, double obstacle_weight, float* candidates,
+                                                  uint64_t* wave_keys, int32_t* counter, double* out, uint64_t* key_out, void* stream) {
+  return shooting_plan_impl<float>(p, B, ld, iters, step, state, samples_T, true, spheres, K, obstacle_weight, candidates, wave_keys, counter, out, key_out,
+                                   stream);
+}
+extern "C" int se3mpc_shooting_plan_obstacles_f64(const se3mpc_params* p, int B, int ld, int iters, double step, const double* state,
+                                                  const double* samples_T, const double* spheres, int K, double obstacle_weight, double* candidates,
+                                                  uint64_t* wave_keys, int32_t* counter, double* out, uint64_t* key_out, void* stream) {
+  return shooting_plan_impl<double>(p, B, ld, iters, step, state, samples_T, true, spheres, K, obstacle_weight, candidates, wave_keys, counter, out, key_out,
+                                    stream);
+}
 extern "C" int se3mpc_projected_step_f32(const se3mpc_params* p, int B, int ld, double step, const float* T, const float* gradT, float* T_out,
                                          void* stream) {
   return projected_step_impl<float>(p, B, ld, step, T, gradT, T_out, stream);
diff --git a/dart_planner_amd/ops.py b/dart_planner_amd/ops.py
--- a/dart_planner_amd/ops.py
+++ b/dart_planner_amd/ops.py
@@ -224,6 +224,49 @@
         self.lib.call("shooting_finish", suf, self._B(ld, B), ld, self.be.ptr(T), self.be.ptr(wave_keys), int(np.prod(wave_keys.shape)), int(index_base),
                       self.be.ptr(state), self.be.ptr(spheres if K else None), K, float(obstacle_weight), self.be.ptr(out), self.be.ptr(key_out),
                       self.be.stream(), params=params)
+        return out
+
+    def shooting_plan_work(self, params: Params, samples, B: Optional[int] = None) -> dict:
+        ld = samples.shape[1]
+        nB = self._B(ld, B)
+        suf = self.be.suffix(samples)
+        cols = self.lib.shooting_plan_columns(params.horizon, nB, ld, 4 if suf == "f32" else 8)
+        return dict(candidates=self.be.empty((3 * params.horizon, cols), suf), wave_keys=self.be.empty((2 * ((nB + 63) // 64),), "i64"),
+                    counter=self.be.from_host(np.zeros(1, dtype=np.int32)))
+
+    def shooting_plan(self, params: Params, samples, iters: int, step: float, state, out, key_out=None, spheres=None, obstacle_weight: float = 0.0,
+                      work: Optional[dict] = None, B: Optional[int] = None):
+        N = params.horizon
+        self._lane(samples, 3 * N, "samples")
+        suf = self.be.suffix(samples)
+        for nm, a, n in (("state", state, 9), ("out", out, 19 * N + 3), ("key_out", key_out, 1)):
+            if a is None and nm == "key_out":
+                continue
+            if not (self.be.is_host_mapped(a) or (self.be.check(a, nm) is a)):
+                raise TypeError(f"{nm}: expected a device tensor or a pinned host tensor")
+            if int(np.prod(a.shape)) < n or str(a.dtype).rsplit(".", 1)[-1] != ("int64" if nm == "key_out" else "float64"):
+                raise ValueError(f"{nm}: expected at least {n} {'int64' if nm == 'key_out' else 'float64'} values")
+        ld = samples.shape[1]
+        nB = self._B(ld, B)
+        if work is None:
+            work = self.shooting_plan_work(params, samples, B)
+        cand, wk, counter = work["candidates"], work["wave_keys"], work["counter"]
+        cols = self.lib.shooting_plan_columns(N, nB, ld, 4 if suf == "f32" else 8)
+        for nm, a, n, ty in (("candidates", cand, 3 * N * cols, None), ("wave_keys", wk, 2 * ((nB + 63) // 64), "int64"), ("counter", counter, 1, "int32")):
+            self.be.check(a, nm)
+            if int(np.prod(a.shape)) < n or (ty is not None and str(a.dtype).rsplit(".", 1)[-1] != ty) or (ty is None and self.be.suffix(a) != suf):
+                raise ValueError(f"{nm}: expected at least {n} {ty or suf} values")
+        if spheres is None:
+            self.lib.call("shooting_plan", suf, nB, ld, int(iters), float(step), self.be.ptr(state), self.be.ptr(samples), self.be.ptr(cand),
+                          self.be.ptr(wk), self.be.ptr(counter), self.be.ptr(out), self.be.ptr(key_out), self.be.stream(), params=params)
+            return out
+        self.be.check(spheres, "spheres")
+        if spheres.ndim != 2 or spheres.shape[1] != 4 or spheres.shape[0] > SE3MPC_MAX_SPHERES or str(spheres.dtype).rsplit(".", 1)[-1] != "float64":
+            raise ValueError(f"spheres: expected float64 (K<={SE3MPC_MAX_SPHERES}, 4), got {tuple(spheres.shape)} {spheres.dtype}")
+        K = spheres.shape[0]
+        self.lib.call("shooting_plan_obstacles", suf, nB, ld, int(iters), float(step), self.be.ptr(state), self.be.ptr(samples),
+                      self.be.ptr(spheres if K else None), K, float(obstacle_weight), self.be.ptr(cand), self.be.ptr(wk), self.be.ptr(counter),
+                      self.be.ptr(out), self.be.ptr(key_out), self.be.stream(), params=params)
         return out
 
     def rollout_cost_grad_batched(self, params: Params, p0, v0, goal, T, cost, gradT, wave_keys=None, index_base: int = 0):
diff --git a/dart_planner_amd/planning/se3_mpc_planner.py b/dart_planner_amd/planning/se3_mpc_planner.py
--- a/dart_planner_amd/planning/se3_mpc_planner.py
+++ b/dart_planner_amd/planning/se3_mpc_planner.py
@@ -371,29 +371,17 @@
                 self._shooting_graphs = {}
             dev = ops.be.device
             dt = torch.float32 if precision == "f32" else torch.float64
-            io = dict(h_in=torch.zeros(9, dtype=torch.float64).pin_memory(), d_in=torch.zeros(9, dtype=torch.float64, device=dev),
+            io = dict(h_in=torch.zeros(9 + 4 * K, dtype=torch.float64).pin_memory(), d_in=torch.zeros(9 + 4 * K, dtype=torch.float64, device=dev),
                       h_out=torch.zeros(19 * N + 3, dtype=torch.float64).pin_memory(), h_key=torch.zeros(1, dtype=torch.int64).pin_memory(),
-                      samples=shooting_samples(prm, n_samples, sigma, seed, dev, dt), wk=torch.zeros(((n_samples + 63) // 64,), dtype=torch.int64, device=dev))
-            if K:
-                io.update(h_sph=torch.zeros((K, 4), dtype=torch.float64).pin_memory(), d_sph=torch.zeros((K, 4), dtype=torch.float64, device=dev))
-
-            io["wide"] = torch.empty((3, 3, n_samples), dtype=dt, device=dev)
+                      samples=shooting_samples(prm, n_samples, sigma, seed, dev, dt))
+            io["work"] = ops.shooting_plan_work(prm, io["samples"])
+            io["d_state"], io["d_sph"] = io["d_in"][:9], io["d_in"][9:].view(K, 4)
             io["h_in_np"], io["h_out_np"], io["h_key_np"] = io["h_in"].numpy(), io["h_out"].numpy(), io["h_key"].numpy()
-            if K:
-                io["h_sph_np"] = io["h_sph"].numpy()
 
             def body():
                 io["d_in"].copy_(io["h_in"], non_blocking=True)
-                wide = io["wide"]
-                wide.copy_(io["d_in"].view(3, 3, 1).expand(3, 3, n_samples))
-                sph_d = None
-                if K:
-                    io["d_sph"].copy_(io["h_sph"], non_blocking=True)
-                    sph_d = io["d_sph"].to(dt)
-                out = ops.rollout_iterate(prm, wide[0], wide[1], wide[2], io["samples"], iters, step, want_grad=False, wave_keys=io["wk"], index_base=0,
-                                          spheres=sph_d, obstacle_weight=w_obs, want_penalty=False)
-                ops.shooting_finish(prm, out["T"], io["wk"], io["d_in"], io["h_out"], key_out=io["h_key"], spheres=io["d_sph"] if K else None,
-                                    obstacle_weight=w_obs)
+                ops.shooting_plan(prm, io["samples"], iters, step, io["d_state"], io["h_out"], key_out=io["h_key"], spheres=io["d_sph"] if K else None,
+                                  obstacle_weight=w_obs, work=io["work"])
 
             side = torch.cuda.Stream(device=dev)
             side.wait_stream(torch.cuda.current_stream(dev))
@@ -411,7 +399,7 @@
         hin = io["h_in_np"]
         hin[0:3] = p0; hin[3:6] = v0; hin[6:9] = self.goal_position
         if K:
-            io["h_sph_np"][...] = sph
+            hin[9:] = np.asarray(sph, float).reshape(-1)
         graph.replay()
         torch.cuda.current_stream(ops.be.device).synchronize()
         r = io["h_out_np"]
diff --git a/include/se3mpc.h b/include/se3mpc.h
--- a/include/se3mpc.h
+++ b/include/se3mpc.h
@@ -157,6 +157,18 @@
 int se3mpc_shooting_finish_f64(const se3mpc_params* p, int B, int ld, const double* T, const uint64_t* wave_keys, int n_slots,
                                uint32_t index_base, const double* state, const double* spheres, int K, double obstacle_weight, double* out,
                                uint64_t* key_out, void* stream);
+
+int se3mpc_shooting_plan_columns(int horizon, int B, int ld, int elem_bytes);
+int se3mpc_shooting_plan_f32(const se3mpc_params* p, int B, int ld, int iters, double step, const double* state, const float* samples_T,
+                             float* candidates, uint64_t* wave_keys, int32_t* counter, double* out, uint64_t* key_out, void* stream);
+int se3mpc_shooting_plan_f64(const se3mpc_params* p, int B, int ld, int iters, double step, const double* state, const double* samples_T,
+                             double* candidates, uint64_t* wave_keys, int32_t* counter, double* out, uint64_t* key_out, void* stream);
+int se3mpc_shooting_plan_obstacles_f32(const se3mpc_params* p, int B, int ld, int iters, double step, const double* state,
+                                       const float* samples_T, const double* spheres, int K, double obstacle_weight, float* candidates,
+                                       uint64_t* wave_keys, int32_t* counter, double* out, uint64_t* key_out, void* stream);
+int se3mpc_shooting_plan_obstacles_f64(const se3mpc_params* p, int B, int ld, int iters, double step, const double* state,
+                                       const double* samples_T, const double* spheres, int K, double obstacle_weight, double* candidates,
+                                       uint64_t* wave_keys, int32_t* counter, double* out, uint64_t* key_out, void* stream);
 
 int se3mpc_reduce_keys(const uint64_t* wave_keys, int per_batch, int nbatch, uint64_t* keys_out, void* stream);
 
```

Measured after the change: 7.942 billion. 1.3% lower.
